# automerge/automerge-classic

Measured on AMD Instinct MI355X. Metric: CRDT ops/sec applied (bulk replay), higher is better.
Workload: dtype u32

## Files before the change

### automerge_classic_amd/csrc/am355_api.hip

```cpp
#include "am355_ctx.h"

static bool ctx_init(am355_ctx* c) {
  {
    unsigned hw = std::thread::hardware_concurrency();
    const char* env = getenv("AM355_HOST_THREADS");
    unsigned want = env && atoi(env) > 0 ? (unsigned)atoi(env) : std::min(hw ? hw : 4u, 64u);
    c->pool.reset(new HostPool(want > 1 ? want - 1 : 0));
  }
  int prio_low = 0, prio_high = 0;
  (void)hipDeviceGetStreamPriorityRange(&prio_low, &prio_high);
  auto make_stream = [](Stream& s, int prio) { return hipStreamCreateWithPriority(&s.h, hipStreamNonBlocking, prio) == hipSuccess; };
  if (!make_stream(c->stream, prio_high)) return false;
  {
    const char* env = getenv("AM355_HASH_CUS");
    int want = env ? atoi(env) : 0;
    bool made = false;
    if (want > 0) {
      hipDeviceProp_t prop;
      if (hipGetDeviceProperties(&prop, c->device) == hipSuccess && prop.multiProcessorCount > want) {
        int n_cu = prop.multiProcessorCount;
        std::vector<uint32_t> mask((size_t)(n_cu + 31) / 32, 0u);
        for (int k = 0; k < want; k++) { int cu = n_cu - 1 - k; mask[(size_t)cu / 32] |= 1u << (cu % 32); }
        made = hipExtStreamCreateWithCUMask(&c->stream2.h, (uint32_t)mask.size(), mask.data()) == hipSuccess;
      }
    }
    if (!made && !make_stream(c->stream2, prio_low)) return false;
  }
  if (!make_stream(c->stream3, prio_high) || !make_stream(c->stream4, prio_high)) return false;
  for (Event* e : {&c->ev_fork, &c->ev_join, &c->ev[0], &c->ev[1], &c->ev[2], &c->ev[3], &c->ev[4], &c->ev[5], &c->ev[6], &c->ev[7], &c->ev_parse, &c->ev_b0, &c->ev_b1,
                   &c->ev_counts, &c->ev_runs, &c->ev_s1, &c->ev_plan, &c->ev_tables, &c->ev_fills, &c->ev_sched})
    if (hipEventCreate(&e->h) != hipSuccess) return false;
  if (!c->h_sig.ensure(sizeof(HostSignals))) return false;
  memset(c->h_sig.p, 0, sizeof(HostSignals));
  if (const char* e = getenv("AM355_PHASE_EVENTS")) c->phase_events = strcmp(e, "0") != 0;
  if (const char* e = getenv("AM355_STAGE1_FILLS")) c->inline_fills = strcmp(e, "stream") != 0;
  return true;
}

extern "C" am355_ctx* am355_create(int device) {
  int n = 0;
  if (hipGetDeviceCount(&n) != hipSuccess || n <= 0 || device < 0 || device >= n) return nullptr;
  (void)hipSetDeviceFlags(hipDeviceScheduleSpin);
  if (hipSetDevice(device) != hipSuccess) return nullptr;
  am355_ctx* c = new am355_ctx();
  c->device = device;
  if (!ctx_init(c)) { delete c; return nullptr; }
  return c;
}

am355_ctx::~am355_ctx() {
  (void)hipSetDevice(device);
  if (lane) lane->wait();
  (void)doc_sum.wait();
  for (const Stream* s : {&stream, &stream2, &stream3, &stream4})
    if (s->h) (void)hipStreamSynchronize(s->h);
  if (shard_comm) (void)am355_shard_finalize(this);
}

extern "C" void am355_destroy(am355_ctx* c) {
  delete c;
}

extern "C" const char* am355_last_error(const am355_ctx* c) { return c ? c->err.c_str() : "no context (no GPU?)"; }
extern "C" uint32_t am355_flags(const am355_ctx* c) { return c ? c->flags : 0; }

extern "C" int am355_set_phase_events(am355_ctx* c, int on) {
  if (!c) return AM355_E_ARG;
  c->phase_events = on != 0;
  return AM355_OK;
}

extern "C" int am355_get_stats(const am355_ctx* c, am355_stats* out) {
  if (!c || !out) return AM355_E_ARG;
  *out = c->stats;
  return AM355_OK;
}

extern "C" int am355_get_hashes(const am355_ctx* c, uint8_t* out) {
  if (!c || !out) return AM355_E_ARG;
  if (!c->replayed || !c->h_hashes.p || c->is_document) return AM355_E_STATE;
  memcpy(out, c->h_hashes.p, 32 * (size_t)c->n_changes);
  return AM355_OK;
}

extern "C" int am355_arena_epoch(const am355_ctx* c, uint64_t* epoch) {
  if (!c || !epoch) return AM355_E_ARG;
  *epoch = c->arena_epoch;
  return AM355_OK;
}

extern "C" int am355_get_hashes_range(const am355_ctx* c, uint32_t first, uint32_t count, uint8_t* out) {
  if (!c || (!out && count)) return AM355_E_ARG;
  if (!c->replayed || !c->h_hashes.p || c->is_document) return AM355_E_STATE;
  if (first > c->n_changes || count > c->n_changes - first) return AM355_E_ARG;
  if (count) memcpy(out, (const uint8_t*)c->h_hashes.p + 32 * (size_t)first, 32 * (size_t)count);
  return AM355_OK;
}

extern "C" int am355_applied_in_input_order(const am355_ctx* c, int* yes) {
  if (!c || !yes) return AM355_E_ARG;
  if (!c->replayed || c->is_document) return AM355_E_STATE;
  bool ok = c->pending_change.empty() && c->n_pending == 0 && c->applied_change.size() == c->n_changes;
  for (uint32_t i = 0; ok && i < c->n_changes; i++) ok = c->applied_change[i] == i;
  *yes = ok ? 1 : 0;
  return AM355_OK;
}

extern "C" int am355_resident_counters(const am355_ctx* c, uint64_t out[3]) {
  if (!c || !out) return AM355_E_ARG;
  out[0] = c->n_resident_calls;
  out[1] = c->n_resident_fallbacks;
  out[2] = c->n_resorder_calls;
  return AM355_OK;
}

extern "C" int am355_resident_maps_only_calls(const am355_ctx* c, uint64_t* out) {
  if (!c || !out) return AM355_E_ARG;
  *out = c->n_maps_only_calls;
  return AM355_OK;
}

extern "C" int am355_get_raw(const am355_ctx* c, const uint8_t** arena, const uint64_t** offsets, uint32_t* n) {
  if (!c || !c->staged) return AM355_E_STATE;
  if (arena) *arena = c->raw.data();
  if (offsets) *offsets = c->raw_off.data();
  if (n) *n = c->n_changes;
  return AM355_OK;
}

extern "C" int am355_get_applied(const am355_ctx* c, uint32_t* out, uint32_t* n_applied) {
  if (!c || !n_applied) return AM355_E_ARG;
  if (!c->replayed || c->is_document) return AM355_E_STATE;
  *n_applied = (uint32_t)c->applied_change.size();
  if (out) memcpy(out, c->applied_change.data(), 4 * c->applied_change.size());
  return AM355_OK;
}

extern "C" int am355_test_sort(am355_ctx* c, uint64_t* keys, uint32_t* vals, uint32_t n, int key_bits) {
  if (!c) return AM355_E_ARG;
  (void)hipSetDevice(c->device);
  DevBuf ka, kb, va, vb, ws;
  if (!ka.ensure(8 * (size_t)n + 8) || !kb.ensure(8 * (size_t)n + 8) || !va.ensure(4 * (size_t)n + 4) || !vb.ensure(4 * (size_t)n + 4) || !ws.ensure(sort_workspace_bytes(n)))
    return fail(c, AM355_E_NOMEM, "alloc");
  hipStream_t st = c->stream;
  (void)hipMemcpyAsync(ka.p, keys, 8 * (size_t)n, hipMemcpyHostToDevice, st);
  (void)hipMemcpyAsync(va.p, vals, 4 * (size_t)n, hipMemcpyHostToDevice, st);
  int res = radix_sort_pairs(ka.as<uint64_t>(), va.as<uint32_t>(), kb.as<uint64_t>(), vb.as<uint32_t>(), n, 0, key_bits, ws.p, st);
  (void)hipMemcpyAsync(keys, res ? kb.p : ka.p, 8 * (size_t)n, hipMemcpyDeviceToHost, st);
  (void)hipMemcpyAsync(vals, res ? vb.p : va.p, 4 * (size_t)n, hipMemcpyDeviceToHost, st);
  HIPCHK(c, hipStreamSynchronize(st));
  HIPCHK(c, hipGetLastError());
  return AM355_OK;
}

extern "C" int am355_test_scan(am355_ctx* c, const uint32_t* in, uint32_t* out, uint32_t n, uint32_t* total) {
  if (!c) return AM355_E_ARG;
  (void)hipSetDevice(c->device);
  DevBuf di, dt, ws;
  if (!di.ensure(4 * (size_t)n + 4) || !dt.ensure(4) || !ws.ensure(scan_workspace_bytes(n))) return fail(c, AM355_E_NOMEM, "alloc");
  hipStream_t st = c->stream;
  (void)hipMemcpyAsync(di.p, in, 4 * (size_t)n, hipMemcpyHostToDevice, st);
  exclusive_scan_u32(di.as<uint32_t>(), di.as<uint32_t>(), n, dt.as<uint32_t>(), ws.p, st);
  (void)hipMemcpyAsync(out, di.p, 4 * (size_t)n, hipMemcpyDeviceToHost, st);
  (void)hipMemcpyAsync(total, dt.p, 4, hipMemcpyDeviceToHost, st);
  HIPCHK(c, hipStreamSynchronize(st));
// ... 42 lines not shown
```

### automerge_classic_amd/csrc/am355_ctx.h

```cpp
#pragma once
#include "../../include/am355.h"
#include "am355_decode.h"
#include "am355_merge.h"
#include "am355_bigcol.h"
#include "am355_encode.h"
#include "am355_prims.h"
#include "am355_render.h"
#include "am355_host.h"
#include "am355_pinflate.h"
#include "am355_history.h"
#include "am355_delta.h"
#include "am355_resorder.h"
#include "am355_apply.h"
#include "am355_sync.h"
#include "am355_sched.h"
#include "am355_hist.h"
#include "am355_canary.h"

#include <zlib.h>

#include <algorithm>
#include <atomic>
#include <chrono>
#include <cstdarg>
// ... 236 lines not shown
      if (stop_) return;
    }
  }
  static uint64_t now_us() { return (uint64_t)std::chrono::duration_cast<std::chrono::microseconds>(std::chrono::steady_clock::now().time_since_epoch()).count(); }
  std::function<void()> job_;
  std::atomic<int> state_{0};
  std::atomic<bool> sleeping_{false};
  std::mutex m_;
  std::condition_variable cv_;
  bool stop_ = false;
  std::thread t_;
};

struct Hash32 {
  uint8_t b[32];
  bool operator==(const Hash32& o) const { return memcmp(b, o.b, 32) == 0; }
};
struct Hash32Hasher {
  size_t operator()(const Hash32& h) const { size_t v; memcpy(&v, h.b, sizeof v); return v; }
};

}
using namespace am355_host;

struct am355_ctx {
  ~am355_ctx();
  int device = 0;
  Stream stream;
  Stream stream2;
  Stream stream3;
  Stream stream4;
  Event ev_fork, ev_join;
  Event ev[8];
  Event ev_parse, ev_b0, ev_b1;
  Event ev_counts, ev_runs;
  std::string err;
  uint32_t flags = 0;

  PinnedBytes raw;
  std::unique_ptr<HostPool> pool;
  std::unique_ptr<AsyncLane> lane;
  std::vector<uint64_t> raw_off;
  uint32_t n_changes = 0;
  DevBuf d_plan_totals;
  bool spec_launched = false;
  bool spec_large_launched = false;
  uint32_t spec_cap_ops = 0, spec_cap_preds = 0;
  uint32_t hint_ops = 0, hint_preds = 0, hint_large = 0;
  bool staged = false, replayed = false, ir_fetched = false;
  int ir_copy_enqueued = 0;
  bool prefetch_ir = false;
  bool has_unknown_cols = false;
  bool staging_in_flight = false;
  bool is_document = false;
  ChangeMeta doc_meta{};
  std::vector<uint32_t> doc_actor_rank;
  DevBuf d_arena, d_offsets, d_metas;
  uint64_t arena_epoch = 1;
  CopyRanges pending_up;
  std::vector<uint32_t> breaks_dev;
  void* breaks_dev_ptr = nullptr;
  HostBuf h_breaks_ahead;
  bool offsets_on_device = false;
  HostBuf h_metas, h_offsets, h_sig;
  uint32_t sig_seq = 0;
  Event ev_s1;
  Event ev_fills;
  Event ev_sched;
  Event ev_plan, ev_tables;
  void* counts_zeroed_at = nullptr; size_t counts_zeroed = 0;
  bool phase_events = false;
  bool inline_fills = true;
  DevBuf d_big, d_bigvals, d_ks;
  HostBuf h_biginfo;
  BigColDesc doc_cols{};
  bool doc_serial = false;
  DevBuf d_entries, d_amap_base, d_amap_prov, d_slots, d_first_idx, d_hashes, d_hash_tab, d_min_idx, d_has_dep, d_words, d_slot_rank, d_scan1, d_plan_sums, d_dep_idx, d_self_idx, d_rank_ids;
  HostBuf h_dep_idx, h_self_idx, h_amap, h_amap_base;
  HostBuf h_slots, h_hashes, h_has_dep, h_words, h_stage, h_s1;
  DevBuf d_s1;
  ChangeBrief* hp_briefs = nullptr;
  uint32_t* hp_distinct = nullptr;
  bool have_host_metas = false;
  uint32_t amap_cap = 0, slot_mask = 0, hash_mask = 0;
  bool used_fast_path = false;

  std::vector<ChangePlan> plans;
  std::vector<uint32_t> applied_change, applied_op_base;
  struct DocSum {
    static constexpr size_t PIECE = (size_t)4 << 20;
    std::thread t;
    std::unique_ptr<std::atomic<uint8_t>[]> copied;
    size_t n_pieces = 0;
    bool pending = false, ok = false;
    bool wait() {
      if (t.joinable()) t.join();
      pending = false;
      return ok;
    }
    ~DocSum() { if (t.joinable()) t.join(); }
  } doc_sum;
  std::vector<uint8_t> doc_bytes;
  std::vector<uint8_t> saved;
  HistoryOutput history;
  bool history_ok = false; uint32_t history_flags = 0;
  std::vector<std::vector<uint8_t>> inflate_scratch;
// ... 183 lines not shown
```

### automerge_classic_amd/csrc/am355_decode.h

```cpp
#pragma once
#include "am355_internal.h"

namespace am355 {
struct ParseFills {
  uint32_t* p[5];
  uint64_t n_words[5];
  uint32_t value[5];
  uint32_t n;
};
void parse_changes_host(const uint8_t* arena, const uint64_t* offsets, uint32_t n_changes, ChangeMeta* metas, uint32_t* n_entries);
void launch_parse_changes(const uint8_t* arena, const uint64_t* offsets, uint32_t n_changes, ChangeMeta* metas, uint32_t* n_entries, const ParseFills& fills,
                          hipStream_t st, bool fat = false);
int change_wave_class(const ChangeMeta& m);
void launch_hash_changes(const uint8_t* arena, const uint64_t* offsets, uint32_t n, uint8_t* hashes, uint32_t* min_idx, uint32_t* hash_tab,
                         uint32_t tab_mask, uint32_t* flags, hipStream_t st);
void launch_deps_resolve(const uint8_t* arena, const ChangeMeta* metas, const uint8_t* hashes, uint32_t n, const uint32_t* hash_tab, uint32_t tab_mask,
                         const uint32_t* min_idx, uint8_t* has_dependent, uint32_t* fast_flags, uint32_t* dep_idx, uint32_t* self_idx, hipStream_t st);
void launch_actor_intern(const uint8_t* arena, ChangeMeta* metas, uint32_t n, const uint32_t* amap_base, uint32_t* amap, uint32_t amap_cap,
                         unsigned long long* slots, uint32_t slot_mask, uint32_t* first_idx, uint32_t* flags, uint32_t* fast_flags, uint32_t* distinct,
                         void* rank_ids, ChangeBrief* briefs, uint32_t* slot_rank, unsigned long long* block_sums, uint32_t* plan_words, hipStream_t st,
                         ChangeBrief* host_briefs = nullptr);
size_t rank_ids_bytes();
size_t plan_block_sums_bytes(uint32_t n);
uint32_t distinct_capacity();
void launch_plan(const ChangeBrief* briefs, uint32_t n, const uint32_t* distinct, const uint32_t* slot_rank, uint32_t slot_mask, const unsigned long long* block_sums,
                 ChangePlan* plans, ChangePlan* plans_serial, const uint32_t* words, const uint32_t* plan_words, HostSignals* sig, uint32_t seq, hipStream_t st,
                 PlanTotals* dev_totals = nullptr, uint32_t* host_s1 = nullptr);
void launch_decode_speculative(const uint8_t* arena, const ChangeMeta* metas, const ChangePlan* plans, uint32_t n_changes, const PlanTotals* totals, uint32_t cap_ops,
                               uint32_t cap_preds, uint32_t cap_distinct, const uint32_t* amap, const uint32_t* slot_rank, OpCols cols, uint32_t* flags, hipStream_t st,
                               hipStream_t aux, bool with_large, uint32_t shard_rank = 0, uint32_t shard_world = 1);
void launch_decode_planned(const uint8_t* arena, const ChangeMeta* metas, const ChangePlan* plans, const ChangePlan* plans_serial, uint32_t n_changes,
                           uint32_t n_small, uint32_t n_large, uint32_t n_serial, const uint32_t* amap, const uint32_t* slot_rank, OpCols cols, uint32_t* flags,
                           hipStream_t st, hipStream_t aux, uint32_t shard_rank = 0, uint32_t shard_world = 1);
void launch_decode_columns(const uint8_t* arena, const ChangeMeta* metas, const ChangePlan* plans, uint32_t n_small, uint32_t n_large, uint32_t n_serial,
                           const uint32_t* amap, const uint32_t* slot_rank, OpCols cols, uint32_t* flags, hipStream_t st, hipStream_t aux, uint32_t shard_rank = 0,
                           uint32_t shard_world = 1);
void launch_doc_count(const uint8_t* arena, ChangeMeta* meta, hipStream_t st);
void launch_decode_document(const uint8_t* arena, const ChangeMeta* meta, const ChangePlan* plan, const uint32_t* actor_rank, OpCols cols,
                            uint32_t* flags, hipStream_t st);
void launch_keystr_expand(const uint32_t* run_start, const uint32_t* run_off, const uint32_t* run_len, const uint32_t* n_runs, uint32_t n_rows,
                          uint32_t* key_off, uint32_t* key_len, hipStream_t st);
}
```

### automerge_classic_amd/csrc/am355_decode.hip

```cpp
#include "am355_decode.h"
#include "am355_scan.h"

#include <cstdlib>

namespace am355 {

struct __attribute__((packed)) U8B {
  uint64_t v;
};
__host__ __device__ __forceinline__ uint64_t load_u64_unaligned(const uint8_t* p) { return ((const U8B*)p)->v; }
#ifdef AM355_LDS_IS_DISTINCT
__device__ __forceinline__ uint64_t load_u64_unaligned(LdsBytes p) { return ((const __attribute__((address_space(3))) U8B*)p)->v; }
#endif

template <class P>
struct CurT {
  P p;
  uint32_t off, len;
  uint64_t win;
  uint32_t win_off;
  __host__ __device__ __forceinline__ CurT() {}
  static constexpr uint32_t WIN_EMPTY = 0xffffff00u;
  __host__ __device__ __forceinline__ CurT(P p_, uint32_t off_, uint32_t len_) : p(p_), off(off_), len(len_), win(0), win_off(WIN_EMPTY) {}
  __host__ __device__ __forceinline__ uint32_t byte_at(uint32_t o) {
// ... 866 lines not shown
  if (wide) {
    p0 = load_u64_unaligned(p);
    p1 = load_u64_unaligned(p + 8);
    h = (p0 ^ (p1 * 0x9e3779b97f4a7c15ull)) * 0xff51afd7ed558ccdull;
    h ^= h >> 29;
  } else {
    for (uint32_t k = 0; k < len; k++) h = (h ^ p[k]) * 0x100000001b3ull;
    h = (h ^ h >> 33) * 0xff51afd7ed558ccdull;
  }
  uint32_t i = (uint32_t)(h >> 20) & mask;
  unsigned long long mine = ((unsigned long long)off + 1) << 16 | len;
  for (uint32_t probes = 0; probes <= mask; probes++) {
    unsigned long long v = slots[i];
    if (v == 0) {
      v = atomicCAS(&slots[i], 0ull, mine);
      if (v == 0) {
        uint32_t k = atomicAdd(&distinct[0], 1u);
        if (k < DISTINCT_CAP) {
          distinct[1 + k] = i;
          ((unsigned long long*)(distinct + 2 + DISTINCT_CAP))[k] = mine;
        }
        if (k < PLAN_RANK_MAX) {
          RankId r;
          for (uint32_t wd = 0; wd < PLAN_ID_MAX / 8; wd++) r.w[wd] = 0;
          r.len = len;
          r.pad = 0;
          if (wide) {
            r.w[0] = __builtin_bswap64(p0);
            r.w[1] = __builtin_bswap64(p1);
          } else if (len <= PLAN_ID_MAX) {
            for (uint32_t b = 0; b < len; b++) r.w[b >> 3] |= (unsigned long long)p[b] << (56 - 8 * (b & 7));
          }
          rank_ids[k] = r;
        }
        return i;
      }
    }
    if ((uint32_t)(v & 0xffff) == len) {
      const uint8_t* q = arena + ((v >> 16) - 1);
      bool eq = true;
      if (wide) eq = load_u64_unaligned(q) == p0 && load_u64_unaligned(q + 8) == p1;
      else for (uint32_t k = 0; k < len && eq; k++) eq = p[k] == q[k];
      if (eq) return i;
    }
    i = (i + 1) & mask;
  }
  return NONE32;
}

__global__ __launch_bounds__(WAVE) void k_actor_intern(const uint8_t* __restrict__ arena, ChangeMeta* __restrict__ metas, uint32_t n,
                                                        const uint32_t* __restrict__ amap_base, uint32_t* __restrict__ amap, uint32_t amap_cap,
                                                        unsigned long long* __restrict__ slots, uint32_t mask, uint32_t* __restrict__ first_idx,
                                                        uint32_t* __restrict__ flags, uint32_t* __restrict__ fast_flags, uint32_t* __restrict__ distinct,
                                                        RankId* __restrict__ rank_ids) {
  __shared__ uint32_t s_off[WAVE], s_len[WAVE];
  wave_priority_high();
  uint32_t c = blockIdx.x, lane = threadIdx.x;
  if (c >= n) return;
  ChangeMeta* m = &metas[c];
  if (m->flags) return;
  uint32_t base = amap_base[c];
  if ((uint64_t)base + m->n_entries > amap_cap) {
    if (lane == 0) atomicOr(fast_flags, (uint32_t)FF_CAPACITY);
    return;
  }
  const uint8_t* p = arena + m->base;
  uint32_t abs0 = (uint32_t)m->base;
  uint32_t n_other = m->n_other;
  if (lane == 0) {
    uint32_t s = actor_find_or_insert(arena, slots, mask, abs0 + m->actor_off, m->actor_len, distinct, rank_ids);
    if (s == NONE32) { atomicOr(flags, (uint32_t)F_UNSUPPORTED); s = 0; }
    amap[base] = s;
    m->author_slot = s;
    atomicMin(&first_idx[s], c);
  }
  if (n_other && n_other <= WAVE) {
    const uint32_t l0 = p[m->others_off], stride = l0 + 1;
    bool fits = l0 < 0x80 && (uint64_t)m->others_off + (uint64_t)stride * n_other <= m->len;
    bool mine_ok = !fits || lane >= n_other || p[m->others_off + stride * lane] == l0;
    if (fits && __ballot(!mine_ok) == 0) {
      if (lane < n_other) {
        uint32_t t = actor_find_or_insert(arena, slots, mask, abs0 + m->others_off + stride * lane + 1, l0, distinct, rank_ids);
        if (t == NONE32) { atomicOr(flags, (uint32_t)F_UNSUPPORTED); t = 0; }
        amap[base + 1 + lane] = t;
      }
      return;
    }
  }
  Cur cur(p, m->others_off, m->len);
  for (uint32_t k0 = 0; k0 < n_other; k0 += WAVE) {
    uint32_t cnt = n_other - k0 < WAVE ? n_other - k0 : WAVE;
    if (lane == 0) {
      for (uint32_t j = 0; j < cnt; j++) {
        uint64_t l = 0;
        read_uleb(cur, l);
        s_off[j] = abs0 + cur.off;
        s_len[j] = l < 65536 ? (uint32_t)l : NONE32;
        skip_bytes(cur, l);
      }
    }
    __syncthreads();
    if (lane < cnt) {
      uint32_t t = s_len[lane] != NONE32 ? actor_find_or_insert(arena, slots, mask, s_off[lane], s_len[lane], distinct, rank_ids) : NONE32;
      if (t == NONE32) { atomicOr(flags, (uint32_t)F_UNSUPPORTED); t = 0; }
      amap[base + 1 + k0 + lane] = t;
    }
    __syncthreads();
  }
}

// ... 25 lines not shown
  t[0] = ta; t[1] = tb; t[2] = tc;
}

__device__ void rank_actors(const uint32_t* __restrict__ distinct, const RankId* __restrict__ rank_ids, uint32_t* __restrict__ slot_rank,
                            uint32_t* __restrict__ plan_words) {
  __shared__ unsigned long long s_id[PLAN_RANK_MAX][PLAN_ID_MAX / 8];
  __shared__ uint32_t s_len[PLAN_RANK_MAX];
  __shared__ uint32_t s_fallback;
  static_assert(PLAN_RANK_MAX % BLOCK == 0 && PLAN_RANK_MAX <= DISTINCT_CAP, "rank_actors: records per thread");
  constexpr uint32_t PER = PLAN_RANK_MAX / BLOCK;
  const uint32_t t = threadIdx.x;
  RankId rec[PER];
  uint32_t slot_of[PER];
#pragma unroll
  for (uint32_t k = 0; k < PER; k++) {
    rec[k] = rank_ids[t + k * BLOCK];
    slot_of[k] = distinct[1 + t + k * BLOCK];
  }
  const uint32_t nd = distinct[0];
  if (t == 0) s_fallback = nd > PLAN_RANK_MAX ? 1u : 0u;
  __syncthreads();
  if (nd <= PLAN_RANK_MAX) {
#pragma unroll
    for (uint32_t k = 0; k < PER; k++) {
      const uint32_t a = t + k * BLOCK;
      if (a < nd) {
        s_len[a] = rec[k].len;
        if (rec[k].len > PLAN_ID_MAX) s_fallback = 1;
        for (uint32_t wd = 0; wd < PLAN_ID_MAX / 8; wd++) s_id[a][wd] = rec[k].w[wd];
      }
    }
  }
  __syncthreads();
  if (s_fallback) { if (t == 0) plan_words[0] = 1; return; }
#pragma unroll
  for (uint32_t k = 0; k < PER; k++) {
    const uint32_t a = t + k * BLOCK;
    if (a >= nd) break;
    uint32_t rank = 0;
    const uint32_t my_len = rec[k].len;
    static_assert(PLAN_ID_MAX == 32, "rank_actors compares four 64-bit words");
    const unsigned long long m0 = rec[k].w[0], m1 = rec[k].w[1], m2 = rec[k].w[2], m3 = rec[k].w[3];
    for (uint32_t j = 0; j < nd; j++) {
      const unsigned long long x0 = s_id[j][0], x1 = s_id[j][1], x2 = s_id[j][2], x3 = s_id[j][3];
      const bool less = x0 != m0 ? x0 < m0 : x1 != m1 ? x1 < m1 : x2 != m2 ? x2 < m2 : x3 != m3 ? x3 < m3 : s_len[j] < my_len;
      rank += less ? 1u : 0u;
    }
    slot_rank[slot_of[k]] = rank;
  }
}

__global__ __launch_bounds__(WAVE) void k_actor_first(ChangeMeta* __restrict__ metas, uint32_t n, const uint32_t* __restrict__ amap_base,
                                                       const uint32_t* __restrict__ amap, uint32_t amap_cap, const uint32_t* __restrict__ first_idx,
                                                       uint32_t* __restrict__ fast_flags) {
  wave_priority_high();
  uint32_t c = blockIdx.x, lane = threadIdx.x;
  if (c >= n) return;
  ChangeMeta* m = &metas[c];
  if (m->flags) return;
  uint32_t base = amap_base[c], ne = m->n_entries;
  if ((uint64_t)base + ne > amap_cap) return;
  uint32_t mx = 0;
  for (uint32_t k = lane; k < ne; k += WAVE) {
    uint32_t f = first_idx[amap[base + k]];
    mx = f > mx ? f : mx;
  }
  for (int d = WAVE / 2; d >= 1; d >>= 1) {
    uint32_t o = __shfl_xor(mx, d);
    mx = o > mx ? o : mx;
  }
  if (lane == 0) {
    m->max_first = mx;
    if (mx > c) atomicOr(fast_flags, (uint32_t)FF_LATE_ACTOR);
  }
}

__global__ __launch_bounds__(BLOCK) void k_actor_check(const uint8_t* __restrict__ arena, ChangeMeta* __restrict__ metas, uint32_t n,
                                                       const uint32_t* __restrict__ amap_base, const uint32_t* __restrict__ amap, uint32_t amap_cap,
                                                       const uint32_t* __restrict__ first_idx, uint32_t* __restrict__ flags, uint32_t* __restrict__ fast_flags,
                                                       ChangeBrief* __restrict__ briefs, const uint32_t* __restrict__ distinct, const RankId* __restrict__ rank_ids,
                                                       uint32_t* __restrict__ slot_rank, unsigned long long* __restrict__ block_sums, uint32_t* __restrict__ plan_words,
                                                       ChangeBrief* __restrict__ host_briefs) {
  wave_priority_high();
  __shared__ unsigned long long s_scan[BLOCK / WAVE][3];
  if (blockIdx.x + 1 == gridDim.x) {
    rank_actors(distinct, rank_ids, slot_rank, plan_words);
    return;
  }
  uint32_t c = gtid();
  const bool in_range = c < n;
  ChangeBrief br{};
  if (in_range) {
    ChangeMeta* m = &metas[c];
    br.seq = m->seq;
    br.start_op = (uint32_t)m->start_op;
    br.n_ops = m->n_ops;
    br.n_preds = m->n_preds;
    br.n_entries = m->n_entries;
    br.author_slot = m->author_slot;
    br.flags_fits = m->flags;
    if (!m->flags) {
      int wc = wave_class_of(*m);
      if (wc >= 1) br.flags_fits |= 0x80000000u;
      if (wc == 2) br.flags_fits |= 0x40000000u;
      if (m->pad & 1) br.flags_fits |= 0x20000000u;
    }
    briefs[c] = br;
    if (host_briefs) host_briefs[c] = br;
  }
  const bool valid = in_range && !(br.flags_fits & 0x1fffffffu);
  const bool has = valid && br.n_ops != 0;
  const bool small = has && (br.flags_fits & 0x40000000u), large = has && !small && (br.flags_fits & 0x80000000u), serial = has && !small && !large;
  unsigned long long ex[3], t1[3], t2[3];
  block_scan3(valid ? br.n_ops : 0u, valid ? br.n_preds : 0u, valid ? br.n_entries : 0u, s_scan, ex, t1);
  block_scan3(small ? 1u : 0u, large ? 1u : 0u, serial ? 1u : 0u, s_scan, ex, t2);
  uint32_t mx_op = has ? br.start_op + br.n_ops - 1 : 0u, bad = in_range ? (br.flags_fits & 0x1fffffffu) : 0u, unknown = in_range ? (br.flags_fits & 0x20000000u) : 0u;
  for (int d = WAVE / 2; d >= 1; d >>= 1) {
    uint32_t o = __shfl_xor(mx_op, d), ob = __shfl_xor(bad, d), ou = __shfl_xor(unknown, d);
    mx_op = o > mx_op ? o : mx_op;
    bad |= ob;
    unknown |= ou;
  }
  if ((threadIdx.x & (WAVE - 1)) == 0) {
    if (mx_op) atomicMax(&plan_words[1], mx_op);
    if (bad) atomicOr(&plan_words[2], bad);
    if (unknown) atomicOr(&plan_words[3], 1u);
  }
  if (threadIdx.x == 0) {
    unsigned long long* out = block_sums + (size_t)blockIdx.x * PLAN_SUMS;
    out[0] = t1[0]; out[1] = t1[1]; out[2] = t1[2]; out[3] = t2[0]; out[4] = t2[1]; out[5] = t2[2];
  }
}

__global__ __launch_bounds__(BLOCK) void k_plan_apply(const ChangeBrief* __restrict__ briefs, uint32_t n, const uint32_t* __restrict__ slot_rank, uint32_t slot_mask,
                                                      const unsigned long long* __restrict__ block_sums, ChangePlan* __restrict__ plans,
                                                      ChangePlan* __restrict__ plans_serial, const uint32_t* __restrict__ words, const uint32_t* __restrict__ plan_words,
                                                      const uint32_t* __restrict__ distinct, HostSignals* sig, uint32_t seq, PlanTotals* __restrict__ dev_totals,
                                                      uint32_t* __restrict__ host_s1) {
  wave_priority_high();
  __shared__ unsigned long long s_scan[BLOCK / WAVE][3];
  __shared__ unsigned long long s_base[6];
  {
    unsigned long long p0 = 0, p1 = 0, p2 = 0, p3 = 0, p4 = 0, p5 = 0;
    for (uint32_t j = threadIdx.x; j < blockIdx.x; j += BLOCK) {
      const unsigned long long* q = block_sums + (size_t)j * PLAN_SUMS;
      p0 += q[0]; p1 += q[1]; p2 += q[2]; p3 += q[3]; p4 += q[4]; p5 += q[5];
    }
    unsigned long long ex[3], t1[3], t2[3];
    block_scan3(p0, p1, p2, s_scan, ex, t1);
    block_scan3(p3, p4, p5, s_scan, ex, t2);
    if (threadIdx.x == 0) { s_base[0] = t1[0]; s_base[1] = t1[1]; s_base[2] = t1[2]; s_base[3] = t2[0]; s_base[4] = t2[1]; s_base[5] = t2[2]; }
    __syncthreads();
  }
  const uint32_t c = gtid();
  const bool in_range = c < n;
  ChangeBrief br{};
  if (in_range) br = briefs[c];
  const bool valid = in_range && !(br.flags_fits & 0x1fffffffu);
  const bool has = valid && br.n_ops != 0;
  const bool small = has && (br.flags_fits & 0x40000000u), large = has && !small && (br.flags_fits & 0x80000000u), serial = has && !small && !large;
  unsigned long long e1[3], e2[3], t1[3], t2[3];
  block_scan3(valid ? br.n_ops : 0u, valid ? br.n_preds : 0u, valid ? br.n_entries : 0u, s_scan, e1, t1);
  block_scan3(small ? 1u : 0u, large ? 1u : 0u, serial ? 1u : 0u, s_scan, e2, t2);
  if (has) {
    ChangePlan pl{c, (uint32_t)(s_base[0] + e1[0]), (uint32_t)(s_base[1] + e1[1]), (uint32_t)(s_base[2] + e1[2]),
                  br.author_slot <= slot_mask ? slot_rank[br.author_slot] : 0u, br.n_entries};
    if (small) plans[(uint32_t)(s_base[3] + e2[0])] = pl;
    else if (large) plans[n - 1 - (uint32_t)(s_base[4] + e2[1])] = pl;
    else plans_serial[(uint32_t)(s_base[5] + e2[2])] = pl;
  }
  if (blockIdx.x + 1 == gridDim.x && host_s1) {
    const uint32_t nd = distinct[0] < DISTINCT_CAP ? distinct[0] : DISTINCT_CAP;
    const uint32_t* src = words;
    for (uint32_t i = threadIdx.x; i < 16; i += BLOCK) host_s1[i] = src[i];
    uint32_t* hd = host_s1 + 16;
    for (uint32_t i = threadIdx.x; i < 1 + nd; i += BLOCK) hd[i] = distinct[i];
    const unsigned long long* ids = (const unsigned long long*)(distinct + 2 + DISTINCT_CAP);
    unsigned long long* hids = (unsigned long long*)(hd + 2 + DISTINCT_CAP);
    for (uint32_t i = threadIdx.x; i < nd; i += BLOCK) hids[i] = ids[i];
    __threadfence_system();
    __syncthreads();
  }
  if (blockIdx.x + 1 == gridDim.x && threadIdx.x == 0) {
    unsigned long long ops = s_base[0] + t1[0], preds = s_base[1] + t1[1], ent = s_base[2] + t1[2];
    PlanTotals z{};
    z.n_ops = (uint32_t)ops; z.n_preds = (uint32_t)preds; z.n_entries = (uint32_t)ent;
    z.n_small = (uint32_t)(s_base[3] + t2[0]); z.n_large = (uint32_t)(s_base[4] + t2[1]); z.n_serial = (uint32_t)(s_base[5] + t2[2]);
    z.max_op = plan_words[1];
    z.fallback = (plan_words[0] || ops >= 0x7ffffff0ull || preds >= 0xfffffff0ull || ent >= 0xfffffff0ull) ? 1u : 0u;
    z.flags_a = words[0] | plan_words[2]; z.fast_a = words[1]; z.total_entries = words[2]; z.n_distinct = distinct[0];
    z.reserved[0] = plan_words[3];
    if (dev_totals) *dev_totals = z;
    signal_host((uint32_t*)&sig->plan, (const uint32_t*)&z, sizeof(PlanTotals) / 4, &sig->plan_seq, seq);
  }
}

struct Rle {
  Cur c;
  int state;
  int64_t count;
  bool have_last, last_null;
  int64_t last;
  uint32_t last_off, last_len;
};

__device__ __forceinline__ void rle_init(Rle& r, const uint8_t* p, uint32_t len) {
  r.c = Cur(p, 0, len);
  r.state = 0;
  r.count = 0;
  r.have_last = false;
  r.last_null = true;
  r.last = 0;
  r.last_off = r.last_len = 0;
}

enum { RT_UINT = 0, RT_INT = 1, RT_UTF8 = 2 };

struct RVal {
  bool is_null;
  int64_t i;
  uint32_t off, len;
};

template <int TYPE>
__device__ __forceinline__ bool rle_raw(Rle& r, RVal& v) {
  v.is_null = false;
  if (TYPE == RT_UINT) {
    uint64_t u;
    if (!read_uleb(r.c, u)) return false;
    v.i = (int64_t)u;
  } else if (TYPE == RT_INT) {
    if (!read_sleb(r.c, v.i)) return false;
  } else {
    uint64_t n;
    if (!read_uleb(r.c, n)) return false;
    v.off = r.c.off;
    v.len = (uint32_t)n;
    if (!skip_bytes(r.c, n)) return false;
  }
  return true;
}

template <int TYPE>
__device__ __forceinline__ bool rle_same(const Rle& r, const RVal& v) {
  if (!r.have_last || r.last_null) return false;
  if (TYPE == RT_UTF8) {
// ... 639 lines not shown
        L.run_tok[nr] = 0;
        L.aux[nr] = 0;
        nr++;
        rows = n;
      }
      L.run_start[nr] = (uint32_t)(rows - rows_done);
      L.n_runs = nr;
      L.total_rows = (uint32_t)(rows - rows_done);
      L.err = e;
    }
    __syncthreads();
    err |= L.err;
    uint32_t batch = L.total_rows, nr = L.n_runs;
    for (uint32_t r = lane; r < nr; r += WAVE) {
      uint32_t k = L.run_kind[r], pk = r ? L.run_kind[r - 1] : prev_kind;
      if (k == RK_NUL || pk == RK_NUL) continue;
      uint32_t off = L.run_tok[r] - col_abs, len = L.aux[r];
      uint32_t poff = r ? L.run_tok[r - 1] - col_abs : prev_off, plen = r ? L.aux[r - 1] : prev_len;
      if (len == plen && bytes_equal(keycol, poff, off, len, key_len)) err |= F_BAD_RLE;
    }
    if (lane == 0 && nr) { prev_kind = L.run_kind[nr - 1]; prev_off = L.run_tok[nr - 1] - col_abs; prev_len = L.aux[nr - 1]; }
    for (uint32_t i = lane; i < batch; i += WAVE) {
      uint32_t lo = 0, hi = nr;
      while (hi - lo > 1) {
        uint32_t mid = (lo + hi) >> 1;
        if (L.run_start[mid] <= i) lo = mid; else hi = mid;
      }
      bool nul = L.run_kind[lo] == RK_NUL;
      o.key_off[base + rows_done + i] = nul ? 0 : L.run_tok[lo];
      o.key_len[base + rows_done + i] = nul ? NONE32 : L.aux[lo];
    }
    rows_done += batch;
    __syncthreads();
    if (rows_done >= n || batch == 0) break;
  }
  return err;
}

enum : uint32_t { DG_ROWS = 1 , DG_KEY_ID = 2 , DG_KEY_STR = 4, DG_PRED = 8, DG_ALL = 15 };

template <class WL>
__global__ __launch_bounds__(WAVE) AM355_WAVES_PER_EU(WL::COLMAX <= 256 ? 6 : 1) void k_decode_wave(const uint8_t* __restrict__ arena, const ChangeMeta* __restrict__ metas,
                                                       const ChangePlan* __restrict__ plans, uint32_t n_plans, ActorXlate x, OpCols o,
                                                       uint32_t* __restrict__ flags, DecodeGate gate) {
  __shared__ WL L;
  wave_priority_high();
  uint32_t pi = blockIdx.x, lane = threadIdx.x;
  const uint32_t groups = gridDim.y > 1 ? (1u << blockIdx.y) : (uint32_t)DG_ALL;
  if (gate.totals) {
    const PlanTotals t = *gate.totals;
    if (!decode_gate_open(t, gate.cap_ops, gate.cap_preds, gate.cap_distinct)) return;
    n_plans = gate.large ? t.n_large : t.n_small;
    if (gate.large) plans += gate.n_changes - t.n_large;
  }
  if (pi >= n_plans) return;
  const ChangePlan pl = plans[pi];
  const ChangeMeta* m = &metas[pl.change];
  const uint8_t* p = arena + m->base;
  const uint32_t n = m->n_ops, base = pl.op_base, abs0 = (uint32_t)m->base, n_preds_cap = m->n_preds;
  const uint32_t start_op = (uint32_t)m->start_op;
  uint32_t col_off[C_NUM], col_len[C_NUM];
  for (int k = 0; k < C_NUM; k++) { col_off[k] = m->col_off[k]; col_len[k] = m->col_len[k]; }
  uint32_t err = 0;
  for (uint32_t k = lane; k < pl.n_actors; k += WAVE) {
    uint32_t v = x.amap[pl.amap_base + k];
    L.rank[k] = x.slot_rank ? x.slot_rank[v] : v;
  }
  uint32_t reg_lo = 0xffffffffu, reg_hi = 0;
  for (int k = 0; k < C_NUM; k++)
    if (col_len[k]) {
      reg_lo = col_off[k] < reg_lo ? col_off[k] : reg_lo;
      reg_hi = col_off[k] + col_len[k] > reg_hi ? col_off[k] + col_len[k] : reg_hi;
    }
  const bool staged = reg_hi > reg_lo && reg_hi - reg_lo <= WL::REGION;
  if (staged) stage_to_lds(L.region, p + reg_lo, reg_hi - reg_lo, lane);
  auto load_col = [&](int k) {
    if (staged && col_len[k]) wv_load_column(L, (LdsBytes)(L.region + (col_off[k] - reg_lo)), col_len[k], lane);
    else wv_load_column(L, p + col_off[k], col_len[k], lane);
  };

  if (groups & DG_ROWS) {
  load_col(C_ACTION);
  err |= L.err;
  for (uint32_t i = lane; i < n; i += WAVE) {
    bool nul; int64_t v;
    wv_row_value<false>(L, i, nul, v, err);
    if (nul) err |= F_UNSUPPORTED;
    if ((uint64_t)v >= NONE32) err |= F_OVERFLOW;
    o.action[base + i] = (uint32_t)v;
    o.id_ctr[base + i] = start_op + i;
    o.id_actor[base + i] = pl.author;
  }
  {
    __syncthreads();
    uint32_t len = col_len[C_INSERT];
    if (staged && len) {
      LdsBytes col = (LdsBytes)(L.region + (col_off[C_INSERT] - reg_lo));
      for (uint32_t i = lane; i < len; i += WAVE) L.bytes[i] = col[i];
    } else {
      const uint8_t* col = p + col_off[C_INSERT];
      for (uint32_t i = lane; i < len; i += WAVE) L.bytes[i] = col[i];
    }
    __syncthreads();
    uint32_t tok_base = 0, carry_start = 0;
    for (uint32_t chunk = 0; chunk < len; chunk += WAVE) {
      uint32_t pos = chunk + lane;
// ... 166 lines not shown
    uint32_t r = 0;
    if (nul) err |= F_UNSUPPORTED;
    else if ((uint64_t)v >= pl.n_actors) err |= F_BAD_ROW;
    else r = L.rank[v];
    o.pred_actor[pl.pred_base + j] = r;
  }
  load_col(C_PRED_CTR);
  err |= L.err;
  {
    int64_t carry = 0;
    for (uint32_t j0 = 0; j0 < total_preds; j0 += WAVE) {
      uint32_t j = j0 + lane;
      bool nul = true; int64_t d = 0;
      if (j < total_preds) wv_row_value<true>(L, j, nul, d, err);
      int64_t abs = carry + wave_incl_scan_i64(nul ? 0 : d, lane);
      carry = __shfl(abs, WAVE - 1);
      if (j < total_preds) {
        if (nul) err |= F_UNSUPPORTED;
        else if (abs < 0 || (uint64_t)abs >= NONE32) err |= F_OVERFLOW;
        o.pred_ctr[pl.pred_base + j] = (uint32_t)abs;
      }
    }
  }
  }
  if (err) atomicOr(flags, err);
}

int change_wave_class(const ChangeMeta& m) { return wave_class_of(m); }

void launch_parse_changes(const uint8_t* arena, const uint64_t* offsets, uint32_t n_changes, ChangeMeta* metas, uint32_t* n_entries, const ParseFills& fills,
                          hipStream_t st, bool fat) {
  if (!n_changes && !fills.n) return;
  if (fat) hipLaunchKernelGGL(k_parse_changes<true>, dim3(n_changes ? n_changes : 64), dim3(WAVE), 0, st, arena, offsets, n_changes, metas, n_entries, fills);
  else hipLaunchKernelGGL(k_parse_changes<false>, dim3(n_changes ? n_changes : 64), dim3(WAVE), 0, st, arena, offsets, n_changes, metas, n_entries, fills);
}

void launch_hash_changes(const uint8_t* arena, const uint64_t* offsets, uint32_t n, uint8_t* hashes, uint32_t* min_idx, uint32_t* hash_tab,
                         uint32_t tab_mask, uint32_t* flags, hipStream_t st) {
  if (!n) return;
  hipLaunchKernelGGL(k_hash_changes, dim3((n + HASH_LANES - 1) / HASH_LANES), dim3(2 * HASH_LANES), 0, st, arena, offsets, n, hashes, min_idx, flags);
  AM355_LAUNCH_INDEPENDENT(k_hash_insert, dim3((n + BLOCK - 1) / BLOCK), dim3(BLOCK), st, (const uint8_t*)hashes, n, hash_tab, tab_mask, min_idx);
}

void launch_deps_resolve(const uint8_t* arena, const ChangeMeta* metas, const uint8_t* hashes, uint32_t n, const uint32_t* hash_tab, uint32_t tab_mask,
                         const uint32_t* min_idx, uint8_t* has_dependent, uint32_t* fast_flags, uint32_t* dep_idx, uint32_t* self_idx, hipStream_t st) {
  if (!n) return;
  AM355_LAUNCH_INDEPENDENT(k_deps_resolve, dim3(n), dim3(WAVE), st, arena, metas, hashes, n, hash_tab, tab_mask, min_idx, has_dependent, fast_flags, dep_idx,
                           self_idx);
}

void launch_actor_intern(const uint8_t* arena, ChangeMeta* metas, uint32_t n, const uint32_t* amap_base, uint32_t* amap, uint32_t amap_cap,
                         unsigned long long* slots, uint32_t slot_mask, uint32_t* first_idx, uint32_t* flags, uint32_t* fast_flags, uint32_t* distinct,
                         void* rank_ids, ChangeBrief* briefs, uint32_t* slot_rank, unsigned long long* block_sums, uint32_t* plan_words, hipStream_t st,
                         ChangeBrief* host_briefs) {
  if (n)
    hipLaunchKernelGGL(k_actor_intern, dim3(n), dim3(WAVE), 0, st, arena, metas, n, amap_base, amap, amap_cap, slots, slot_mask, first_idx, flags,
                       fast_flags, distinct, (RankId*)rank_ids);
  if (n) hipLaunchKernelGGL(k_actor_first, dim3(n), dim3(WAVE), 0, st, metas, n, amap_base, (const uint32_t*)amap, amap_cap, (const uint32_t*)first_idx, fast_flags);
  hipLaunchKernelGGL(k_actor_check, dim3((n + BLOCK - 1) / BLOCK + 1), dim3(BLOCK), 0, st, arena, metas, n, amap_base, (const uint32_t*)amap, amap_cap,
                     (const uint32_t*)first_idx, flags, fast_flags, briefs, (const uint32_t*)distinct, (const RankId*)rank_ids, slot_rank, block_sums, plan_words,
                     host_briefs);
}

size_t rank_ids_bytes() { return sizeof(RankId) * PLAN_RANK_MAX; }

size_t plan_block_sums_bytes(uint32_t n) { return sizeof(unsigned long long) * PLAN_SUMS * ((size_t)(n + BLOCK - 1) / BLOCK + 1); }

void launch_plan(const ChangeBrief* briefs, uint32_t n, const uint32_t* distinct, const uint32_t* slot_rank, uint32_t slot_mask, const unsigned long long* block_sums,
                 ChangePlan* plans, ChangePlan* plans_serial, const uint32_t* words, const uint32_t* plan_words, HostSignals* sig, uint32_t seq, hipStream_t st,
                 PlanTotals* dev_totals, uint32_t* host_s1) {
  uint32_t nb = (n + BLOCK - 1) / BLOCK;
  hipLaunchKernelGGL(k_plan_apply, dim3(nb ? nb : 1), dim3(BLOCK), 0, st, briefs, n, slot_rank, slot_mask, block_sums, plans, plans_serial, words, plan_words,
                     distinct, sig, seq, dev_totals, host_s1);
}

uint32_t distinct_capacity() { return DISTINCT_CAP; }

__global__ __launch_bounds__(WAVE) void k_doc_count(const uint8_t* __restrict__ arena, ChangeMeta* __restrict__ meta) {
  uint32_t lane = threadIdx.x;
  if (lane > 1) return;
  int slot = lane == 0 ? C_ACTION : C_PRED_NUM;
  uint64_t cnt, sum;
  bool ok = rle_count_sum(arena + meta->base + meta->col_off[slot], meta->col_len[slot], cnt, sum);
  if (!ok) { atomicOr(&meta->flags, (uint32_t)F_BAD_RLE); return; }
  if (lane == 0) meta->n_ops = (uint32_t)cnt; else meta->n_preds = (uint32_t)sum;
}

void launch_doc_count(const uint8_t* arena, ChangeMeta* meta, hipStream_t st) {
  AM355_LAUNCH_INDEPENDENT(k_doc_count, dim3(1), dim3(WAVE), st, arena, meta);
}

__global__ __launch_bounds__(BLOCK) void k_keystr_expand(const uint32_t* __restrict__ run_start, const uint32_t* __restrict__ run_off,
                                                          const uint32_t* __restrict__ run_len, const uint32_t* __restrict__ n_runs_p, uint32_t n_rows,
                                                          uint32_t* __restrict__ key_off, uint32_t* __restrict__ key_len) {
  uint32_t row = gtid();
  if (row >= n_rows) return;
  uint32_t nr = *n_runs_p;
  uint32_t off = 0, len = NONE32;
  if (nr && row < run_start[nr]) {
    uint32_t lo = 0, hi = nr;
    while (hi - lo > 1) {
      uint32_t mid = (lo + hi) >> 1;
      if (run_start[mid] <= row) lo = mid; else hi = mid;
    }
    off = run_off[lo];
    len = run_len[lo];
  }
  key_off[row] = off;
  key_len[row] = len;
}

void launch_keystr_expand(const uint32_t* run_start, const uint32_t* run_off, const uint32_t* run_len, const uint32_t* n_runs, uint32_t n_rows,
                          uint32_t* key_off, uint32_t* key_len, hipStream_t st) {
  if (!n_rows) return;
  AM355_LAUNCH_INDEPENDENT(k_keystr_expand, dim3((n_rows + BLOCK - 1) / BLOCK), dim3(BLOCK), st, run_start, run_off, run_len, n_runs, n_rows, key_off, key_len);
}

void launch_decode_document(const uint8_t* arena, const ChangeMeta* meta, const ChangePlan* plan, const uint32_t* actor_rank, OpCols cols,
                            uint32_t* flags, hipStream_t st) {
  ActorXlate x{actor_rank, nullptr, 0, 1};
  AM355_LAUNCH_INDEPENDENT(k_decode_columns, dim3(1, T_NUM_DOC), dim3(WAVE), st, arena, meta, plan, 1u, x, cols, flags, 0);
}

static uint32_t decode_group_split(uint32_t n_waves, uint32_t shard_world, bool large_class = false) {
  static const uint32_t split_max = []() { const char* e = getenv("AM355_DECODE_SPLIT_MAX"); return e && atol(e) > 0 ? (uint32_t)atol(e) : 1536u; }();
  return (shard_world <= 1 && n_waves <= (large_class ? 512u : split_max)) ? 4u : 1u;
}

void launch_decode_columns(const uint8_t* arena, const ChangeMeta* metas, const ChangePlan* plans, uint32_t n_small, uint32_t n_large, uint32_t n_serial,
                           const uint32_t* amap, const uint32_t* slot_rank, OpCols cols, uint32_t* flags, hipStream_t st, hipStream_t aux, uint32_t shard_rank,
                           uint32_t shard_world) {
  ActorXlate x{amap, slot_rank, shard_rank, shard_world};
  if (n_large && n_small + n_large <= 1024) { n_large += n_small; n_small = 0; }
  hipStream_t s2 = (n_small && aux) ? aux : st;
  if (n_small) hipLaunchKernelGGL(k_decode_wave<WaveLdsSmall>, dim3(n_small, decode_group_split(n_small, shard_world)), dim3(WAVE), 0, st, arena, metas, plans, n_small, x, cols, flags, DecodeGate{});
  if (n_large) hipLaunchKernelGGL(k_decode_wave<WaveLdsLarge>, dim3(n_large, decode_group_split(n_large, shard_world, true)), dim3(WAVE), 0, s2, arena, metas, plans + n_small, n_large, x, cols, flags, DecodeGate{});
  if (n_serial)
    AM355_LAUNCH_INDEPENDENT(k_decode_columns, dim3((n_serial + WAVE - 1) / WAVE, T_NUM), dim3(WAVE), s2, arena, metas, plans + n_small + n_large, n_serial,
                             x, cols, flags, 0);
}

void launch_decode_planned(const uint8_t* arena, const ChangeMeta* metas, const ChangePlan* plans, const ChangePlan* plans_serial, uint32_t n_changes,
                           uint32_t n_small, uint32_t n_large, uint32_t n_serial, const uint32_t* amap, const uint32_t* slot_rank, OpCols cols, uint32_t* flags,
                           hipStream_t st, hipStream_t aux, uint32_t shard_rank, uint32_t shard_world) {
  ActorXlate x{amap, slot_rank, shard_rank, shard_world};
  hipStream_t s2 = (n_small && aux) ? aux : st;
  if (n_small) hipLaunchKernelGGL(k_decode_wave<WaveLdsSmall>, dim3(n_small, decode_group_split(n_small, shard_world)), dim3(WAVE), 0, st, arena, metas, plans, n_small, x, cols, flags, DecodeGate{});
  if (n_large) hipLaunchKernelGGL(k_decode_wave<WaveLdsLarge>, dim3(n_large, decode_group_split(n_large, shard_world, true)), dim3(WAVE), 0, s2, arena, metas, plans + (n_changes - n_large), n_large, x, cols, flags, DecodeGate{});
  if (n_serial)
    AM355_LAUNCH_INDEPENDENT(k_decode_columns, dim3((n_serial + WAVE - 1) / WAVE, T_NUM), dim3(WAVE), s2, arena, metas, plans_serial, n_serial, x, cols, flags, 0);
}

void launch_decode_speculative(const uint8_t* arena, const ChangeMeta* metas, const ChangePlan* plans, uint32_t n_changes, const PlanTotals* totals, uint32_t cap_ops,
                               uint32_t cap_preds, uint32_t cap_distinct, const uint32_t* amap, const uint32_t* slot_rank, OpCols cols, uint32_t* flags, hipStream_t st,
                               hipStream_t aux, bool with_large, uint32_t shard_rank, uint32_t shard_world) {
  if (!n_changes) return;
  ActorXlate x{amap, slot_rank, shard_rank, shard_world};
  hipLaunchKernelGGL(k_decode_wave<WaveLdsSmall>, dim3(n_changes, decode_group_split(n_changes, shard_world)), dim3(WAVE), 0, st, arena, metas, plans, 0u, x, cols, flags,
                     DecodeGate{totals, cap_ops, cap_preds, cap_distinct, n_changes, 0u});
  if (with_large)
    hipLaunchKernelGGL(k_decode_wave<WaveLdsLarge>, dim3(n_changes, decode_group_split(n_changes, shard_world, true)), dim3(WAVE), 0, aux, arena, metas, plans, 0u, x, cols, flags,
                       DecodeGate{totals, cap_ops, cap_preds, cap_distinct, n_changes, 1u});
}

}
```

### automerge_classic_amd/csrc/am355_internal.h

```cpp
#pragma once
#include "am355_device.h"

namespace am355 {

enum ColSlot { C_OBJ_ACTOR, C_OBJ_CTR, C_KEY_ACTOR, C_KEY_CTR, C_KEY_STR, C_INSERT, C_ACTION, C_VAL_LEN, C_VAL_RAW, C_PRED_NUM, C_PRED_ACTOR, C_PRED_CTR,
               C_ID_ACTOR, C_ID_CTR, C_NUM };

struct ChangeMeta {
  uint64_t base;
  uint32_t len;
  uint32_t flags;
  uint64_t seq, start_op;
  uint32_t n_entries;
  uint32_t author_slot;
  uint32_t max_first;
  uint32_t pad;
  uint32_t n_deps, deps_off;
  uint32_t actor_off, actor_len;
  uint32_t n_other, others_off;
  uint32_t col_off[C_NUM], col_len[C_NUM];
  uint32_t n_ops, n_preds;
};

struct ChangeBrief {
  uint64_t seq;
  uint32_t start_op, n_ops, n_preds, n_entries, author_slot;
  uint32_t flags_fits;
};

enum FastFlag : uint32_t {
  FF_DUP_HASH = 1u << 0,
  FF_MISSING_DEP = 1u << 1,
  FF_LATE_DEP = 1u << 2,
  FF_LATE_ACTOR = 1u << 3,
  FF_CAPACITY = 1u << 4
};

struct ChangePlan {
  uint32_t change;
  uint32_t op_base;
  uint32_t pred_base;
  uint32_t amap_base;
  uint32_t author;
  uint32_t n_actors;
};

struct PlanTotals {
  uint32_t n_ops, n_preds, n_entries;
  uint32_t n_small, n_large, n_serial;
  uint32_t max_op;
  uint32_t fallback;
  uint32_t flags_a, fast_a, total_entries, n_distinct;
  uint32_t reserved[4];
};

__host__ __device__ inline bool decode_gate_open(const PlanTotals& t, uint32_t cap_ops, uint32_t cap_preds, uint32_t cap_distinct) {
  return !t.fallback && !t.flags_a && !t.fast_a && t.n_ops <= cap_ops && t.n_preds <= cap_preds && t.n_distinct <= cap_distinct;
}
struct DecodeGate {
  const PlanTotals* totals = nullptr;
  uint32_t cap_ops = 0, cap_preds = 0, cap_distinct = 0, n_changes = 0, large = 0;
};

struct HostSignals {
  volatile uint32_t plan_seq;    uint32_t pad0[15];
  PlanTotals plan;
  volatile uint32_t counts_seq;  uint32_t pad1[15];
  uint32_t counts[32];
  volatile uint32_t runs_seq;    uint32_t pad2[15];
  uint32_t runs[16];
  volatile uint32_t final_seq;   uint32_t pad3[15];
  uint32_t final_counts[16];
  volatile uint32_t resorder_seq;  uint32_t pad4[15];
  uint32_t resorder[16];
  volatile uint32_t delta_mid_seq; uint32_t pad5[15];
  uint32_t delta_mid[16];
  volatile uint32_t delta_end_seq; uint32_t pad6[15];
  uint32_t delta_end[16];
};

struct ActorSpan {
  uint32_t start_op, n_ops, op_base;
};

struct OpCols {
  uint32_t *obj_actor, *obj_ctr;
  uint32_t *key_actor, *key_ctr;
  uint32_t *key_off, *key_len;
  uint32_t *action, *val_tl, *val_off;
  uint32_t *pred_first, *pred_num;
  uint32_t *id_ctr, *id_actor;
  uint8_t* insert;
  uint32_t *pred_actor, *pred_ctr;
};

__host__ __device__ __forceinline__ uint32_t shard_owner(uint32_t obj_actor, uint32_t obj_ctr, uint32_t world) {
  return obj_actor == NONE32 ? 0u : (obj_ctr + obj_actor) % world;
}

}
```

### automerge_classic_amd/csrc/am355_prims.h

```cpp
#pragma once
#include "am355_device.h"
#include "am355_canary.h"
#include <stddef.h>

namespace am355 {
constexpr uint32_t LAUNCH_RANGES = 8;
struct FillRanges {
  uint32_t* p[LAUNCH_RANGES];
  uint32_t n_words[LAUNCH_RANGES];
  uint32_t value[LAUNCH_RANGES];
  uint32_t n = 0;
  bool add(void* q, size_t bytes, uint32_t v) {
    if (n == LAUNCH_RANGES) return false;
    p[n] = (uint32_t*)q; n_words[n] = (uint32_t)((bytes + 3) / 4); value[n] = v; n++;
    return true;
  }
};
void launch_fill_ranges(const FillRanges& f, hipStream_t st);
struct CopyRanges {
  void* dst[LAUNCH_RANGES];
  const void* src[LAUNCH_RANGES];
  uint32_t bytes[LAUNCH_RANGES];
  uint32_t n = 0;
  bool add(void* d, const void* s, size_t b) {
    if (n == LAUNCH_RANGES) return false;
    dst[n] = d; src[n] = s; bytes[n] = (uint32_t)b; n++;
    return true;
  }
};
void launch_copy_ranges(const CopyRanges& r, hipStream_t st);
void launch_signal_words(const uint32_t* src_a, uint32_t n_a, const uint32_t* src_b, uint32_t n_b, uint32_t* host_words, volatile uint32_t* host_seq, uint32_t seq,
                         hipStream_t st);
size_t scan_workspace_bytes(uint32_t n);
void exclusive_scan_u32(const uint32_t* in, uint32_t* out, uint32_t n, uint32_t* d_total, void* ws, hipStream_t st);
void exclusive_scan_terminators(const uint8_t* bytes, uint32_t L, uint32_t* out, uint32_t* d_total, void* ws, hipStream_t st);
void exclusive_scan2_u32(const uint32_t* in_a, uint32_t* out_a, uint32_t* d_total_a, const uint32_t* in_b, uint32_t* out_b, uint32_t* d_total_b, uint32_t n,
                         void* ws, hipStream_t st);
void max_u32(const uint32_t* v, uint32_t n, uint32_t* d_out, hipStream_t st);
size_t sort_workspace_bytes(uint32_t n);
int radix_sort_pairs(uint64_t* keys_a, uint32_t* vals_a, uint64_t* keys_b, uint32_t* vals_b, uint32_t n, int begin_bit, int end_bit,
                     void* ws, hipStream_t st, bool first_hist_done = false);
constexpr uint32_t SORT_TILE_ELEMS = 2048;
uint32_t sort_tiles(uint32_t n);
bool sort_is_fused(uint32_t n);
uint32_t* sort_first_table(void* ws);
size_t chain_work_bytes(uint32_t n);
void chain_mark(const uint32_t* next, uint32_t n, uint32_t* mark, void* work, hipStream_t st);
}
```

### automerge_classic_amd/csrc/am355_prims.hip

```cpp
#include "am355_prims.h"
#include <algorithm>
#include "am355_scan.h"
#include "am355_canary.h"
#include <mutex>
#include <string>
#include <vector>

namespace am355 {

constexpr int SCAN_ITEMS = 8;
constexpr int SCAN_TILE = BLOCK * SCAN_ITEMS;
constexpr uint32_t SCAN_SINGLE = 4 * SCAN_TILE;
constexpr uint32_t SCAN_TWO_LAUNCH_TILES = 1024;

__global__ __launch_bounds__(BLOCK) void k_scan_tile_sums(const uint32_t* __restrict__ in, uint32_t* __restrict__ tile_sums, uint32_t n) {
  __shared__ uint32_t s[BLOCK / WAVE];
  uint32_t base = blockIdx.x * SCAN_TILE;
  uint32_t v[SCAN_ITEMS];
#pragma unroll
  for (int j = 0; j < SCAN_ITEMS; j++) {
    uint32_t i = base + j * BLOCK + threadIdx.x;
    v[j] = i < n ? in[i] : 0u;
  }
  uint32_t sum = 0;
#pragma unroll
  for (int j = 0; j < SCAN_ITEMS; j++) sum += v[j];
  uint32_t total = block_sum_u32(sum, s);
  if (threadIdx.x == 0) tile_sums[blockIdx.x] = total;
}

__global__ __launch_bounds__(BLOCK) void k_scan_sums(uint32_t* __restrict__ sums, uint32_t n_tiles, uint32_t* __restrict__ grand_total) {
  __shared__ uint32_t s[BLOCK / WAVE];
  uint32_t carry = 0;
  constexpr uint32_t SUMS_PER = 4;
  for (uint32_t base = 0; base < n_tiles; base += BLOCK * SUMS_PER) {
    const uint32_t i0 = base + threadIdx.x * SUMS_PER;
    uint32_t v[SUMS_PER], mine = 0;
#pragma unroll
    for (uint32_t k = 0; k < SUMS_PER; k++) {
      v[k] = i0 + k < n_tiles ? sums[i0 + k] : 0u;
      mine += v[k];
    }
    uint32_t total;
    uint32_t ex = block_exclusive_scan_u32(mine, s, &total) + carry;
#pragma unroll
    for (uint32_t k = 0; k < SUMS_PER; k++) {
      if (i0 + k < n_tiles) sums[i0 + k] = ex;
      ex += v[k];
    }
    carry += total;
  }
  if (threadIdx.x == 0 && grand_total) *grand_total = carry;
}

template <bool PREFIXED>
__global__ __launch_bounds__(BLOCK) void k_scan_apply(const uint32_t* __restrict__ in, uint32_t* __restrict__ out,
                                                      const uint32_t* __restrict__ tile_sums, uint32_t n, uint32_t* __restrict__ grand_total) {
  __shared__ uint32_t s[BLOCK / WAVE];
  uint32_t before;
  if (PREFIXED) before = tile_sums[blockIdx.x];
  else {
    uint32_t part = 0;
    for (uint32_t k = threadIdx.x; k < blockIdx.x; k += BLOCK) part += tile_sums[k];
    before = block_sum_u32(part, s);
  }
  static_assert(SCAN_ITEMS == 8, "k_scan_apply moves a thread's stretch as two uint4");
  uint32_t base = blockIdx.x * SCAN_TILE + threadIdx.x * SCAN_ITEMS;
  const bool wide = ((((uintptr_t)in | (uintptr_t)out) & 15) == 0) && base + SCAN_ITEMS <= n;
  uint32_t v[SCAN_ITEMS];
  if (wide) {
    const uint4 a = *(const uint4*)(in + base), b4 = *(const uint4*)(in + base + 4);
    v[0] = a.x; v[1] = a.y; v[2] = a.z; v[3] = a.w; v[4] = b4.x; v[5] = b4.y; v[6] = b4.z; v[7] = b4.w;
  } else {
#pragma unroll
    for (int j = 0; j < SCAN_ITEMS; j++) {
      uint32_t i = base + j;
      v[j] = i < n ? in[i] : 0;
    }
  }
  uint32_t sum = 0;
#pragma unroll
  for (int j = 0; j < SCAN_ITEMS; j++) sum += v[j];
  uint32_t total;
  uint32_t ex = block_exclusive_scan_u32(sum, s, &total) + before;
  if (!PREFIXED && grand_total && blockIdx.x == gridDim.x - 1 && threadIdx.x == 0) *grand_total = before + total;
  uint32_t o[SCAN_ITEMS];
#pragma unroll
  for (int j = 0; j < SCAN_ITEMS; j++) {
    o[j] = ex;
    ex += v[j];
  }
  if (wide) {
    *(uint4*)(out + base) = uint4{o[0], o[1], o[2], o[3]};
    *(uint4*)(out + base + 4) = uint4{o[4], o[5], o[6], o[7]};
  } else {
#pragma unroll
    for (int j = 0; j < SCAN_ITEMS; j++) {
      uint32_t i = base + j;
      if (i < n) out[i] = o[j];
    }
  }
}

constexpr unsigned long long LB_SUM = 1ull << 32, LB_PREFIX = 2ull << 32;
__device__ __forceinline__ unsigned long long lb_load(const unsigned long long* p) {
#if defined(__HIP_DEVICE_COMPILE__)
  return __hip_atomic_load(p, __ATOMIC_RELAXED, __HIP_MEMORY_SCOPE_AGENT);
#else
  return *(const volatile unsigned long long*)p;
#endif
}
__device__ __forceinline__ void lb_store(unsigned long long* p, unsigned long long v) {
#if defined(__HIP_DEVICE_COMPILE__)
  __hip_atomic_store(p, v, __ATOMIC_RELAXED, __HIP_MEMORY_SCOPE_AGENT);
#else
  *(volatile unsigned long long*)p = v;
#endif
// ... 24 lines not shown
#pragma unroll
  for (int j = 0; j < SCAN_ITEMS; j++) sum += v[j];
  uint32_t total;
  uint32_t ex = block_exclusive_scan_u32(sum, s, &total);
  if (threadIdx.x == 0) {
    lb_store(&state[tile], (tile ? LB_SUM : LB_PREFIX) | total);
    s_before = 0;
  }
  if (tile && threadIdx.x < WAVE) {
    const uint32_t lane = threadIdx.x;
    uint32_t before = 0;
    int look = (int)tile - 1;
    for (;;) {
      const int idx = look - (int)lane;
      const unsigned long long w = idx >= 0 ? lb_load(&state[idx]) : LB_PREFIX;
      const uint32_t st = (uint32_t)(w >> 32);
      const unsigned long long pending = __ballot(st == 0), prefix = __ballot(st == 2);
      const uint32_t first = prefix ? (uint32_t)__ffsll((long long)prefix) - 1 : WAVE;
      const unsigned long long needed = first >= WAVE - 1 ? ~0ull : ((2ull << first) - 1);
      if (pending & needed) continue;
      uint32_t part = lane <= first ? (uint32_t)w : 0u;
      for (int d = WAVE / 2; d; d >>= 1) part += __shfl_xor(part, d);
      before += part;
      if (prefix) break;
      look -= WAVE;
    }
    if (lane == 0) {
      s_before = before;
      lb_store(&state[tile], LB_PREFIX | (before + total));
    }
  }
  __syncthreads();
  const uint32_t before = s_before;
  if (grand_total && (size_t)(tile + 1) * SCAN_TILE >= n && threadIdx.x == 0) *grand_total = before + total;
  ex += before;
  uint32_t o[SCAN_ITEMS];
#pragma unroll
  for (int j = 0; j < SCAN_ITEMS; j++) {
    o[j] = ex;
    ex += v[j];
  }
  if (wide) {
    *(uint4*)(out + base) = uint4{o[0], o[1], o[2], o[3]};
    *(uint4*)(out + base + 4) = uint4{o[4], o[5], o[6], o[7]};
  } else {
#pragma unroll
    for (int j = 0; j < SCAN_ITEMS; j++) {
      uint32_t i = base + j;
      if (i < n) out[i] = o[j];
    }
  }
}

__global__ __launch_bounds__(BLOCK) void k_scan_single(const uint32_t* __restrict__ in, uint32_t* __restrict__ out, uint32_t n, uint32_t* __restrict__ grand_total) {
  wave_priority_high();
  __shared__ uint32_t s[BLOCK / WAVE];
  uint32_t carry = 0;
  for (uint32_t tile = 0; tile < n; tile += SCAN_TILE) {
    uint32_t base = tile + threadIdx.x * SCAN_ITEMS;
    uint32_t v[SCAN_ITEMS];
    uint32_t sum = 0;
    for (int j = 0; j < SCAN_ITEMS; j++) {
      uint32_t i = base + j;
      v[j] = i < n ? in[i] : 0;
      sum += v[j];
    }
    uint32_t total;
    uint32_t ex = block_exclusive_scan_u32(sum, s, &total) + carry;
    for (int j = 0; j < SCAN_ITEMS; j++) {
      uint32_t i = base + j;
      if (i < n) out[i] = ex;
      ex += v[j];
    }
    carry += total;
  }
  if (threadIdx.x == 0 && grand_total) *grand_total = carry;
}

__global__ __launch_bounds__(BLOCK) void k_scan2_tile_sums(const uint32_t* __restrict__ in_a, const uint32_t* __restrict__ in_b, uint32_t* __restrict__ sums_a,
                                                          uint32_t* __restrict__ sums_b, uint32_t n) {
  __shared__ uint32_t s[BLOCK / WAVE];
  uint32_t base = blockIdx.x * SCAN_TILE;
  uint32_t sa = 0, sb = 0;
  for (int j = 0; j < SCAN_ITEMS; j++) {
    uint32_t i = base + j * BLOCK + threadIdx.x;
    if (i < n) { sa += in_a[i]; sb += in_b[i]; }
  }
  uint32_t ta = block_sum_u32(sa, s), tb = block_sum_u32(sb, s);
  if (threadIdx.x == 0) { sums_a[blockIdx.x] = ta; sums_b[blockIdx.x] = tb; }
}
__global__ __launch_bounds__(BLOCK) void k_scan2_sums(uint32_t* __restrict__ sums_a, uint32_t* __restrict__ sums_b, uint32_t n_tiles, uint32_t* __restrict__ total_a,
                                                     uint32_t* __restrict__ total_b) {
  __shared__ uint32_t s[BLOCK / WAVE];
  uint32_t ca = 0, cb = 0;
  for (uint32_t base = 0; base < n_tiles; base += BLOCK) {
    uint32_t i = base + threadIdx.x;
    uint32_t va = i < n_tiles ? sums_a[i] : 0, vb = i < n_tiles ? sums_b[i] : 0;
    uint32_t ta, tb;
    uint32_t ea = block_exclusive_scan_u32(va, s, &ta);
    uint32_t eb = block_exclusive_scan_u32(vb, s, &tb);
    if (i < n_tiles) { sums_a[i] = ca + ea; sums_b[i] = cb + eb; }
    ca += ta;
    cb += tb;
  }
  if (threadIdx.x == 0) {
    if (total_a) *total_a = ca;
    if (total_b) *total_b = cb;
  }
}
template <bool PREFIXED>
// ... 58 lines not shown
__device__ __forceinline__ void term_load(const uint8_t* __restrict__ bytes, uint32_t L, uint32_t base, uint32_t (&v)[SCAN_ITEMS]) {
  static_assert(SCAN_ITEMS == 8, "a thread's stretch is one 8-byte load");
  if ((((uintptr_t)(bytes + base)) & 7) == 0 && base + SCAN_ITEMS <= L) {
    const unsigned long long x = *(const unsigned long long*)(bytes + base);
#pragma unroll
    for (int j = 0; j < SCAN_ITEMS; j++) v[j] = (uint32_t)((x >> (8 * j + 7)) & 1ull) ^ 1u;
  } else {
#pragma unroll
    for (int j = 0; j < SCAN_ITEMS; j++) { uint32_t i = base + j; v[j] = i < L ? ((bytes[i] >> 7) ^ 1u) : 0u; }
  }
}
__global__ __launch_bounds__(BLOCK) void k_scan_term_sums(const uint8_t* __restrict__ bytes, uint32_t L, uint32_t* __restrict__ tile_sums) {
  __shared__ uint32_t s[BLOCK / WAVE];
  uint32_t v[SCAN_ITEMS];
  term_load(bytes, L, blockIdx.x * SCAN_TILE + threadIdx.x * SCAN_ITEMS, v);
  uint32_t sum = 0;
#pragma unroll
  for (int j = 0; j < SCAN_ITEMS; j++) sum += v[j];
  uint32_t total = block_sum_u32(sum, s);
  if (threadIdx.x == 0) tile_sums[blockIdx.x] = total;
}
__global__ __launch_bounds__(BLOCK) void k_scan_term_apply(const uint8_t* __restrict__ bytes, uint32_t L, uint32_t* __restrict__ out, const uint32_t* __restrict__ tile_sums) {
  __shared__ uint32_t s[BLOCK / WAVE];
  const uint32_t n = L + 1;
  const uint32_t base = blockIdx.x * SCAN_TILE + threadIdx.x * SCAN_ITEMS;
  uint32_t v[SCAN_ITEMS];
  term_load(bytes, L, base, v);
  uint32_t sum = 0;
#pragma unroll
  for (int j = 0; j < SCAN_ITEMS; j++) sum += v[j];
  uint32_t total;
  uint32_t ex = block_exclusive_scan_u32(sum, s, &total) + tile_sums[blockIdx.x];
  uint32_t o[SCAN_ITEMS];
#pragma unroll
  for (int j = 0; j < SCAN_ITEMS; j++) { o[j] = ex; ex += v[j]; }
  if ((((uintptr_t)(out + base)) & 15) == 0 && base + SCAN_ITEMS <= n) {
    *(uint4*)(out + base) = uint4{o[0], o[1], o[2], o[3]};
    *(uint4*)(out + base + 4) = uint4{o[4], o[5], o[6], o[7]};
  } else {
#pragma unroll
    for (int j = 0; j < SCAN_ITEMS; j++) if (base + j < n) out[base + j] = o[j];
  }
}
void exclusive_scan_terminators(const uint8_t* bytes, uint32_t L, uint32_t* out, uint32_t* d_total, void* ws, hipStream_t st) {
  const uint32_t n = L + 1, n_tiles = (n + SCAN_TILE - 1) / SCAN_TILE;
  uint32_t* sums = (uint32_t*)ws;
  hipLaunchKernelGGL(k_scan_term_sums, dim3(n_tiles), dim3(BLOCK), 0, st, bytes, L, sums);
  hipLaunchKernelGGL(k_scan_sums, dim3(1), dim3(BLOCK), 0, st, sums, n_tiles, d_total);
  hipLaunchKernelGGL(k_scan_term_apply, dim3(n_tiles), dim3(BLOCK), 0, st, bytes, L, out, (const uint32_t*)sums);
}

size_t scan_workspace_bytes(uint32_t n) { return 2 * sizeof(uint32_t) * ((size_t)(n + SCAN_TILE - 1) / SCAN_TILE + 2); }

void exclusive_scan_u32(const uint32_t* in, uint32_t* out, uint32_t n, uint32_t* d_total, void* ws, hipStream_t st) {
  uint32_t n_tiles = (n + SCAN_TILE - 1) / SCAN_TILE;
  uint32_t* sums = (uint32_t*)ws;
  if (n_tiles == 0) {
    if (d_total) (void)hipMemsetAsync(d_total, 0, sizeof(uint32_t), st);
    return;
  }
  if (n <= SCAN_SINGLE) {
    hipLaunchKernelGGL(k_scan_single, dim3(1), dim3(BLOCK), 0, st, in, out, n, d_total);
    return;
  }
  if (n_tiles <= SCAN_TWO_LAUNCH_TILES) {
    hipLaunchKernelGGL(k_scan_tile_sums, dim3(n_tiles), dim3(BLOCK), 0, st, in, sums, n);
    hipLaunchKernelGGL(k_scan_apply<false>, dim3(n_tiles), dim3(BLOCK), 0, st, in, out, (const uint32_t*)sums, n, d_total);
    return;
  }
  const char* lb_env = getenv("AM355_SCAN_LOOKBACK");
  const bool lookback = lb_env && *lb_env == '1';
  if (lookback) {
    unsigned long long* state = (unsigned long long*)ws;
    uint32_t* ticket = (uint32_t*)(state + n_tiles);
    (void)hipMemsetAsync(ws, 0, sizeof(unsigned long long) * n_tiles + 8, st);
    hipLaunchKernelGGL(k_scan_lookback, dim3(n_tiles), dim3(BLOCK), 0, st, in, out, n, state, ticket, d_total);
    return;
  }
  hipLaunchKernelGGL(k_scan_tile_sums, dim3(n_tiles), dim3(BLOCK), 0, st, in, sums, n);
  hipLaunchKernelGGL(k_scan_sums, dim3(1), dim3(BLOCK), 0, st, sums, n_tiles, d_total);
  hipLaunchKernelGGL(k_scan_apply<true>, dim3(n_tiles), dim3(BLOCK), 0, st, in, out, (const uint32_t*)sums, n, (uint32_t*)nullptr);
}

constexpr int SORT_ITEMS = 8;
constexpr int SORT_WAVE_SPAN = WAVE * SORT_ITEMS;
constexpr int SORT_TILE = (BLOCK / WAVE) * SORT_WAVE_SPAN;
constexpr int RADIX = 256;
constexpr uint32_t SORT_FUSED_TILES = 64;

__global__ __launch_bounds__(BLOCK) void k_sort_hist(const uint64_t* __restrict__ keys, uint32_t n, int shift,
                                                      uint32_t* __restrict__ table, uint32_t n_tiles) {
  __shared__ uint32_t hist[RADIX];
  hist[threadIdx.x] = 0;
  __syncthreads();
  uint32_t base = blockIdx.x * SORT_TILE;
  for (int j = 0; j < SORT_TILE / BLOCK; j++) {
    uint32_t i = base + j * BLOCK + threadIdx.x;
    if (i < n) atomicAdd(&hist[(uint32_t)(keys[i] >> shift) & 0xff], 1u);
  }
  __syncthreads();
  table[threadIdx.x * n_tiles + blockIdx.x] = hist[threadIdx.x];
}

template <bool RAW_TABLE>
__global__ __launch_bounds__(BLOCK) void k_sort_scatter(const uint64_t* __restrict__ keys_in, const uint32_t* __restrict__ vals_in,
                                                         uint64_t* __restrict__ keys_out, uint32_t* __restrict__ vals_out, uint32_t n,
                                                         int shift, const uint32_t* __restrict__ table, uint32_t n_tiles) {
  __shared__ uint32_t wave_cnt[BLOCK / WAVE][RADIX];
  __shared__ uint32_t s_red[BLOCK / WAVE];
  uint32_t t = threadIdx.x, w = t / WAVE, lane = t % WAVE;
  for (int k = 0; k < BLOCK / WAVE; k++) wave_cnt[k][t] = 0;
  __syncthreads();

  uint64_t key[SORT_ITEMS];
  uint32_t val[SORT_ITEMS], rank[SORT_ITEMS];
  uint32_t base = blockIdx.x * SORT_TILE + w * SORT_WAVE_SPAN;
  for (int j = 0; j < SORT_ITEMS; j++) {
    uint32_t i = base + j * WAVE + lane;
    bool valid = i < n;
    key[j] = valid ? keys_in[i] : 0;
    val[j] = valid ? vals_in[i] : 0;
    uint32_t d = (uint32_t)(key[j] >> shift) & 0xff;
    unsigned long long peers = __ballot(valid);
    for (int b = 0; b < 8; b++) {
      unsigned long long m = __ballot(valid && ((d >> b) & 1));
      peers &= ((d >> b) & 1) ? m : ~m;
    }
    uint32_t before = (uint32_t)__popcll(peers & ((1ull << lane) - 1));
    uint32_t seen = valid ? wave_cnt[w][d] : 0;
    rank[j] = seen + before;
    __builtin_amdgcn_wave_barrier();
    if (valid && before == 0) wave_cnt[w][d] = seen + (uint32_t)__popcll(peers);
    __builtin_amdgcn_wave_barrier();
  }
// ... 466 lines not shown
```

### automerge_classic_amd/csrc/am355_replay.hip

```cpp
#include "am355_ctx.h"


struct HashSet {
  std::vector<const uint8_t*> slot;
  size_t mask = 0;
  void init(size_t n) {
    size_t cap = 16;
    while (cap < n * 2 + 2) cap <<= 1;
    slot.assign(cap, nullptr);
    mask = cap - 1;
  }
  static uint64_t key(const uint8_t* h) { uint64_t v; memcpy(&v, h, 8); return v * 0x9e3779b97f4a7c15ull; }
  const uint8_t** find(const uint8_t* h) {
    size_t i = (size_t)(key(h) >> 20) & mask;
    while (slot[i]) {
      if (slot[i] != (const uint8_t*)1 && memcmp(slot[i], h, 32) == 0) return &slot[i];
      i = (i + 1) & mask;
    }
    return nullptr;
  }
  bool has(const uint8_t* h) { return find(h) != nullptr; }
  void add(const uint8_t* h) {
    size_t i = (size_t)(key(h) >> 20) & mask;
    while (slot[i] && slot[i] != (const uint8_t*)1) i = (i + 1) & mask;
// ... 567 lines not shown
      d_amap = c->d_amap_prov.as<uint32_t>();
      d_rank = (const uint32_t*)(d_tables + o_x);
    } else {
      if (b_amap) memcpy(h + o_x, c->amap.data(), b_amap);
      d_amap = (const uint32_t*)(d_tables + o_x);
    }
    HIPCHK(c, hipMemcpyAsync(d_tables, h, o_x + std::max(b_rank, b_amap), hipMemcpyHostToDevice, st));
  }

  HIPCHK(c, hipMemsetAsync(c->d_counts.p, 0, c->mb.counts_bytes, st));
  HIPCHK(c, hipEventRecord(c->ev_fork, st));
  HIPCHK(c, hipStreamWaitEvent(c->stream3, c->ev_fork, 0));
  if (!merge_prepare(c->mb, c->stream3)) return fail(c, AM355_E_DEVICE, "merge fills: more ranges than one launch takes");
  HIPCHK(c, hipEventRecord(c->ev[2], st));
  launch_decode_columns(c->d_arena.as<uint8_t>(), c->d_metas.as<ChangeMeta>(), (const ChangePlan*)d_tables, n_small, n_large, (uint32_t)np - n_small - n_large, d_amap,
                        d_rank, c->cols, &c->d_counts.as<Counts>()->flags, st, c->stream3, c->shard_rank, c->shard_world);
  HIPCHK(c, hipEventRecord(c->ev[3], st));
  HIPCHK(c, hipEventRecord(c->ev_join, c->stream3));
  HIPCHK(c, hipStreamWaitEvent(st, c->ev_join, 0));

  Counts* hc = c->h_counts.as<Counts>();
  merge_run(c->mb, c->ir, hc, st, (c->phase_events || !c->mb.sig) ? c->ev_counts.h : nullptr, c->ev_runs);
  HIPCHK(c, hipEventRecord(c->ev[5], st));
  if (hc->flags) return error_for_flags(c, hc->flags, "op set rejected");
  c->counts = *hc;
  c->counts.n_objects += 1;
  return AM355_OK;
}

struct GeneralOrder { const uint32_t* order; const uint32_t* pass; uint32_t n_applied; hipEvent_t ready; };
static int run_device_planned(am355_ctx* c, const PlanTotals& tot, uint32_t n_distinct, float* ms_host_plan, const GeneralOrder* go = nullptr) {
  hipStream_t st = c->stream;
  const bool trace = getenv("AM355_TRACE") != nullptr;
  auto t_begin = std::chrono::steady_clock::now();
  auto lap = [&](const char* what) {
    if (trace) fprintf(stderr, "  planned: %-26s +%8.3f ms\n", what, std::chrono::duration<double, std::milli>(std::chrono::steady_clock::now() - t_begin).count());
  };
  uint32_t n = c->n_changes;
  c->n_ops = tot.n_ops;
  c->n_preds = tot.n_preds;
  c->max_op = tot.max_op;
  auto al = [](size_t b) { return (b + 255) & ~(size_t)255; };
  size_t o_tab = al(sizeof(ActorSpan) * (size_t)n + 16), tables_bytes = o_tab + al(4 * ((size_t)n_distinct + 1) + 16);
  if (!c->d_tables.ensure(tables_bytes) || !c->h_stage.ensure(tables_bytes)) return fail(c, AM355_E_NOMEM, "device allocation failed");
  uint8_t* d_tables = c->d_tables.as<uint8_t>();
  c->p_spans = (ActorSpan*)d_tables;
  c->p_tab_off = (uint32_t*)(d_tables + o_tab);
  c->sig_seq++;
  int rcb = setup_buffers(c, n_distinct);
  if (rcb) return rcb;
  lap("buffers carved");
  const bool spec_done = c->spec_launched && decode_gate_open(tot, c->spec_cap_ops, c->spec_cap_preds, distinct_capacity()) &&
                         c->counts_zeroed_at == c->d_counts.p && c->mb.counts_bytes <= c->counts_zeroed;
  if (trace && c->spec_launched && !spec_done)
    fprintf(stderr, "  planned: speculative decode not usable: ops %u / cap %u, preds %u / cap %u, distinct %u, fast_a %x flags_a %x fallback %u, counts %p/%p %zu/%zu\n", tot.n_ops,
            c->spec_cap_ops, tot.n_preds, c->spec_cap_preds, tot.n_distinct, tot.fast_a, tot.flags_a, tot.fallback, c->counts_zeroed_at, c->d_counts.p, c->mb.counts_bytes, c->counts_zeroed);
  if (c->spec_launched && !spec_done) {
    c->spec_launched = false;
    HIPCHK(c, hipStreamSynchronize(c->stream3));
    HIPCHK(c, hipStreamSynchronize(st));
    int rc2 = setup_buffers(c, n_distinct);
    if (rc2) return rc2;
  }
  if (!spec_done && !(c->counts_zeroed_at == c->d_counts.p && c->mb.counts_bytes <= c->counts_zeroed)) HIPCHK(c, hipMemsetAsync(c->d_counts.p, 0, c->mb.counts_bytes, st));
  c->counts_zeroed_at = nullptr;
  c->hint_large = tot.n_large;
  if (spec_done) {
    c->hint_ops = std::max(c->hint_ops, tot.n_ops);
    c->hint_preds = std::max(c->hint_preds, tot.n_preds);
    const uint32_t host_large = c->spec_large_launched ? 0u : tot.n_large;
    if (tot.n_serial || host_large) {
      if (!c->spec_large_launched) {
        HIPCHK(c, hipEventRecord(c->ev_fork, st));
        HIPCHK(c, hipStreamWaitEvent(c->stream3, c->ev_fork, 0));
      }
      launch_decode_planned(c->d_arena.as<uint8_t>(), c->d_metas.as<ChangeMeta>(), c->d_plans.as<ChangePlan>(), c->d_plans.as<ChangePlan>() + std::max(n, 1u), n, 0,
                            host_large, tot.n_serial, c->d_amap_prov.as<uint32_t>(), c->d_slot_rank.as<uint32_t>(), c->cols, &c->d_counts.as<Counts>()->flags,
                            c->stream3, nullptr, c->shard_rank, c->shard_world);
    }
    lap("decode was launched behind the plan kernel");
  } else {
    c->hint_ops = tot.n_ops;
    c->hint_preds = tot.n_preds;
    if (tot.n_small && (tot.n_large || tot.n_serial)) {
      HIPCHK(c, hipEventRecord(c->ev_fork, st));
      HIPCHK(c, hipStreamWaitEvent(c->stream3, c->ev_fork, 0));
    }
    if (c->phase_events) HIPCHK(c, hipEventRecord(c->ev[2], st));
    launch_decode_planned(c->d_arena.as<uint8_t>(), c->d_metas.as<ChangeMeta>(), c->d_plans.as<ChangePlan>(), c->d_plans.as<ChangePlan>() + std::max(n, 1u), n,
                          tot.n_small, tot.n_large, tot.n_serial, c->d_amap_prov.as<uint32_t>(), c->d_slot_rank.as<uint32_t>(), c->cols,
                          &c->d_counts.as<Counts>()->flags, st, c->stream3, c->shard_rank, c->shard_world);
    lap("decode launched");
    if (c->phase_events) HIPCHK(c, hipEventRecord(c->ev[3], st));
  }
  c->spec_launched = false;
  const bool second_class = tot.n_small && (tot.n_large || tot.n_serial);
  hipStream_t fill_stream = second_class ? c->stream4 : c->stream3;
  if (!merge_prepare(c->mb, fill_stream)) return fail(c, AM355_E_DEVICE, "merge fills: more ranges than one launch takes");
  if (second_class) {
    HIPCHK(c, hipEventRecord(c->ev_join, c->stream3));
    HIPCHK(c, hipStreamWaitEvent(st, c->ev_join, 0));
  }
  lap("fills enqueued");
  if (go) HIPCHK(c, hipEventSynchronize(go->ready));
  auto t0 = std::chrono::steady_clock::now();
  std::vector<uint32_t> slot_rank;
// ... 652 lines not shown
  c->ir_copy_enqueued = 0;
  c->h_tables_current = false;
  c->pos_valid = false;
  c->stats.n_edits = c->counts.n_edits;
  c->stats.ir_bytes = (uint64_t)c->counts.n_objects * sizeof(am355_ir_object) + (uint64_t)c->counts.n_map_emit * sizeof(am355_ir_map) +
                      ((uint64_t)c->counts.n_erecs + 1) * sizeof(am355_ir_edit);
  if (verify) {
    std::vector<uint32_t> now(c->counts.n_list_ins);
    HIPCHK(c, hipMemcpy(now.data(), b.order, 4 * now.size(), hipMemcpyDeviceToHost));
    if (now != kept) return fail(c, AM355_E_DEVICE, "internal: the list order merged in place differs from the order computed from scratch");
  }
  return AM355_OK;
}

int replay_impl(am355_ctx* c) {
  if (!c) return AM355_E_ARG;
  if (!c->staged) return fail(c, AM355_E_STATE, "am355_load_changes must be called first");
  (void)hipSetDevice(c->device);
  c->replayed = c->ir_fetched = false;
  c->ir_copy_enqueued = 0;
  c->dep_graph_ready = false;
  c->flags = 0;
  c->spec_launched = false;
  c->batch_list_only = false;
  c->h_tables_were_current = c->h_tables_current;
  c->h_tables_current = false;
  if (c->is_document) return replay_document(c);
  auto t_begin = std::chrono::steady_clock::now();
  if (c->in_apply && c->keep.want) {
    c->keep.want = false;
    const int rr = replay_resident(c);
    if (rr != RESIDENT_FALLBACK) {
      if (rr != AM355_OK) return rr;
      am355_stats& s = c->stats;
      s.n_changes = c->n_changes; s.n_applied = c->n_applied; s.n_pending = 0; s.n_actors = (uint32_t)c->actors.size(); s.n_objects = c->counts.n_objects;
      s.n_heads = (uint32_t)(c->heads.size() / 32); s.n_ops = c->n_ops; s.max_op = c->max_op; s.raw_bytes = c->raw.size();
      s.n_map_values = c->counts.n_map_emit; s.n_list_elems = c->counts.n_list_ins; s.n_edits = c->counts.n_edits;
      s.ir_bytes = (uint64_t)c->counts.n_objects * sizeof(am355_ir_object) + (uint64_t)c->counts.n_map_emit * sizeof(am355_ir_map) +
                   ((uint64_t)c->counts.n_erecs + 1) * sizeof(am355_ir_edit);
      s.ms_parse = s.ms_decode = s.ms_merge = s.ms_order = s.ms_hash_stream = s.ms_host_schedule = 0;
      s.fast_path = 1;
      s.ms_total = std::chrono::duration<float, std::milli>(std::chrono::steady_clock::now() - t_begin).count();
      c->used_fast_path = true;
      c->device_scheduled = false;
      c->replayed = true;
      c->seed_list_inc = c->counts.n_list_inc;
      resident_mark(c);
      c->resident_valid = true;
      return AM355_OK;
    }
  }
  c->keep.want = false;
  { int orc = flush_uploads(c); if (!orc) orc = upload_offsets(c); if (orc) return orc; }
  const bool trace = getenv("AM355_TRACE") != nullptr;
  auto lap = [&](const char* what) {
    if (trace) fprintf(stderr, "replay: %-28s +%8.3f ms\n", what, std::chrono::duration<double, std::milli>(std::chrono::steady_clock::now() - t_begin).count());
  };
  hipStream_t sa = c->stream, sb = c->stream2;
  uint32_t n = c->n_changes;
  size_t n1 = std::max<size_t>(n, 1);
  c->slot_mask = pow2_at_least(4 * (uint64_t)n + 64) - 1;
  c->hash_mask = pow2_at_least(2 * (uint64_t)n + 64) - 1;
  if (c->amap_cap < 16 * n1 + 1024) c->amap_cap = (uint32_t)(16 * n1 + 1024);
  if (!c->d_entries.ensure(4 * n1) || !c->d_amap_base.ensure(4 * (n1 + 1)) || !c->d_amap_prov.ensure(4 * (size_t)c->amap_cap) ||
      !c->d_slots.ensure(8 * (size_t)(c->slot_mask + 1)) || !c->d_first_idx.ensure(4 * (size_t)(c->slot_mask + 1)) || !c->d_hashes.ensure(32 * n1) ||
      !c->d_hash_tab.ensure(4 * (size_t)(c->hash_mask + 1)) || !c->d_min_idx.ensure(4 * n1) || !c->d_has_dep.ensure(n1) || !c->d_words.ensure(4 * W_NUM) ||
      !c->d_scan1.ensure(scan_workspace_bytes((uint32_t)n1)) || !c->h_slots.ensure(8 * (size_t)(c->slot_mask + 1)) || !c->h_hashes.ensure(32 * n1) ||
      !c->h_has_dep.ensure(n1) || !c->h_words.ensure(4 * W_NUM) || !c->d_plans.ensure(2 * sizeof(ChangePlan) * n1) ||
      !c->d_slot_rank.ensure(4 * (size_t)(c->slot_mask + 1)) || !c->d_plan_sums.ensure(plan_block_sums_bytes(n)) ||
      !c->d_dep_idx.ensure(4 * (c->raw.size() / 32 + 2)) || !c->d_self_idx.ensure(4 * n1) || !c->d_rank_ids.ensure(rank_ids_bytes()))
    return fail(c, AM355_E_NOMEM, "device allocation failed (stage 1)");
  c->have_host_metas = false;
  const size_t s1_distinct = 64, s1_briefs = s1_distinct + ((12 * (size_t)distinct_capacity() + 16 + 63) & ~(size_t)63);
  const size_t s1_bytes = s1_briefs + sizeof(ChangeBrief) * n1;
  if (!c->d_s1.ensure(s1_bytes) || !c->h_s1.ensure(s1_bytes)) return fail(c, AM355_E_NOMEM, "device allocation failed (stage 1)");
  uint32_t* d_wa = c->d_s1.as<uint32_t>();
  uint32_t* d_distinct = (uint32_t*)(c->d_s1.as<uint8_t>() + s1_distinct);
  ChangeBrief* d_briefs = (ChangeBrief*)(c->d_s1.as<uint8_t>() + s1_briefs);
  const uint32_t* h_wa = c->h_s1.as<uint32_t>();
  c->hp_distinct = (uint32_t*)(c->h_s1.as<uint8_t>() + s1_distinct);
  c->hp_briefs = (ChangeBrief*)(c->h_s1.as<uint8_t>() + s1_briefs);
  uint32_t* d_words = c->d_words.as<uint32_t>();
  uint32_t* h_words = c->h_words.as<uint32_t>();
  HostSignals* sig = c->h_sig.as<HostSignals>();
  PlanTotals tot{};
  static const bool hash_after_parse = []() { const char* e = getenv("AM355_HASH_START"); return !(e && !strcmp(e, "intern")); }();

  HIPCHK(c, hipEventRecord(c->ev[0], sa));
  const size_t cb = merge_counts_bytes((uint32_t)std::min<size_t>(c->raw.size(), 0x7ffffff0u));
  c->counts_zeroed_at = nullptr;
  const bool counts_too = c->d_counts.ensure(cb);
  const bool fat_changes = n && c->raw.size() / n > 4096 && !getenv("AM355_PARSE_LEAN");
  if (c->inline_fills) {
    ParseFills f{};
    auto add = [&](void* q, size_t bytes, uint32_t v) { f.p[f.n] = (uint32_t*)q; f.n_words[f.n] = (bytes + 3) / 4; f.value[f.n] = v; f.n++; };
    add(d_words, 4 * W_NUM, 0);
    add(d_wa, s1_distinct + 16, 0);
    add(c->d_slots.p, 8 * (size_t)(c->slot_mask + 1), 0);
    add(c->d_first_idx.p, 4 * (size_t)(c->slot_mask + 1), 0xffffffffu);
    if (counts_too) add(c->d_counts.p, cb, 0);
    launch_parse_changes(c->d_arena.as<uint8_t>(), c->d_offsets.as<uint64_t>(), n, c->d_metas.as<ChangeMeta>(), c->d_entries.as<uint32_t>(), f, sa, fat_changes);
    HIPCHK(c, hipEventRecord(c->ev_parse, sa));
  } else {
    launch_parse_changes(c->d_arena.as<uint8_t>(), c->d_offsets.as<uint64_t>(), n, c->d_metas.as<ChangeMeta>(), c->d_entries.as<uint32_t>(), ParseFills{}, sa, fat_changes);
    HIPCHK(c, hipEventRecord(c->ev_parse, sa));
    HIPCHK(c, hipMemsetAsync(d_words, 0, 4 * W_NUM, c->stream3));
    HIPCHK(c, hipMemsetAsync(d_wa, 0, s1_distinct + 16, c->stream3));
    HIPCHK(c, hipMemsetAsync(c->d_slots.p, 0, 8 * (size_t)(c->slot_mask + 1), c->stream3));
    HIPCHK(c, hipMemsetAsync(c->d_first_idx.p, 0xff, 4 * (size_t)(c->slot_mask + 1), c->stream3));
    if (counts_too) HIPCHK(c, hipMemsetAsync(c->d_counts.p, 0, cb, c->stream3));
    HIPCHK(c, hipEventRecord(c->ev_join, c->stream3));
    HIPCHK(c, hipStreamWaitEvent(sa, c->ev_join, 0));
  }
  if (counts_too) {
    c->counts_zeroed_at = c->d_counts.p;
    c->counts_zeroed = cb;
  }

  auto enqueue_stream_b = [&]() -> int {
    HIPCHK(c, hipStreamWaitEvent(sb, hash_after_parse ? c->ev_parse : c->ev[1], 0));
    if (!c->inline_fills) HIPCHK(c, hipStreamWaitEvent(sb, c->ev_join, 0));
    HIPCHK(c, hipEventRecord(c->ev_b0, sb));
    HIPCHK(c, hipMemsetAsync(c->d_hash_tab.p, 0, 4 * (size_t)(c->hash_mask + 1), sb));
    HIPCHK(c, hipMemsetAsync(c->d_has_dep.p, 0, n1, sb));
    launch_hash_changes(c->d_arena.as<uint8_t>(), c->d_offsets.as<uint64_t>(), n, c->d_hashes.as<uint8_t>(), c->d_min_idx.as<uint32_t>(),
                    c->d_hash_tab.as<uint32_t>(), c->hash_mask, d_words + W_FLAGS_B, sb);
    launch_deps_resolve(c->d_arena.as<uint8_t>(), c->d_metas.as<ChangeMeta>(), c->d_hashes.as<uint8_t>(), n, c->d_hash_tab.as<uint32_t>(), c->hash_mask,
                    c->d_min_idx.as<uint32_t>(), c->d_has_dep.as<uint8_t>(), d_words + W_FAST_B, c->d_dep_idx.as<uint32_t>(), c->d_self_idx.as<uint32_t>(), sb);
    HIPCHK(c, hipMemcpyAsync(c->h_hashes.p, c->d_hashes.p, 32 * (size_t)n, hipMemcpyDeviceToHost, sb));
    HIPCHK(c, hipMemcpyAsync(c->h_has_dep.p, c->d_has_dep.p, n, hipMemcpyDeviceToHost, sb));
    HIPCHK(c, hipMemcpyAsync(h_words + W_FLAGS_B, d_words + W_FLAGS_B, 8, hipMemcpyDeviceToHost, sb));
    HIPCHK(c, hipEventRecord(c->ev_b1, sb));
    return AM355_OK;
  };
  static const bool enqueue_early = []() { const char* e = getenv("AM355_HASH_ENQUEUE"); return e && !strcmp(e, "early"); }();
  static const bool enqueue_thread = AM355_STREAMS_ORDER_ACROSS_THREADS && []() { const char* e = getenv("AM355_HASH_ENQUEUE"); return !e || !strcmp(e, "thread"); }();
  std::atomic<int> lane_rc{AM355_OK};
  struct LaneJoin {
    AsyncLane* l = nullptr;
    ~LaneJoin() { if (l) l->wait(); }
  } lane_join;
  bool b_enqueued = false;
  if (hash_after_parse && enqueue_early) { int rb = enqueue_stream_b(); if (rb) return rb; b_enqueued = true; }
  else if (hash_after_parse && enqueue_thread && n >= 512) {
    if (!c->lane) c->lane.reset(new AsyncLane);
    c->lane->post([&]() { (void)hipSetDevice(c->device); lane_rc.store(enqueue_stream_b()); });
    lane_join.l = c->lane.get();
    b_enqueued = true;
  }
  exclusive_scan_u32(c->d_entries.as<uint32_t>(), c->d_amap_base.as<uint32_t>(), n, d_wa + W_TOTAL_ENTRIES, c->d_scan1.p, sa);
  static const bool spec_env = []() { const char* e = getenv("AM355_SPEC_DECODE"); return !(e && *e == '0'); }();
  const bool spec_possible = spec_env && n && c->inline_fills && counts_too && hash_after_parse && !getenv("AM355_HOST_PLAN") && !(c->in_apply && c->graph_mode != 0) &&
                             c->d_plan_totals.ensure(sizeof(PlanTotals));
  for (int attempt = 0;; attempt++) {
    if (attempt) {
      HIPCHK(c, hipMemsetAsync(c->d_slots.p, 0, 8 * (size_t)(c->slot_mask + 1), sa));
      HIPCHK(c, hipMemsetAsync(c->d_first_idx.p, 0xff, 4 * (size_t)(c->slot_mask + 1), sa));
      HIPCHK(c, hipMemsetAsync(d_distinct, 0, 4, sa));
    }
    launch_actor_intern(c->d_arena.as<uint8_t>(), c->d_metas.as<ChangeMeta>(), n, c->d_amap_base.as<uint32_t>(), c->d_amap_prov.as<uint32_t>(), c->amap_cap,
                        c->d_slots.as<unsigned long long>(), c->slot_mask, c->d_first_idx.as<uint32_t>(), d_wa + W_FLAGS_A, d_wa + W_FAST_A,
                        d_distinct, c->d_rank_ids.p, d_briefs, c->d_slot_rank.as<uint32_t>(), c->d_plan_sums.as<unsigned long long>(), d_wa + 8, sa, c->hp_briefs);
    c->sig_seq++;
    launch_plan(d_briefs, n, d_distinct, c->d_slot_rank.as<uint32_t>(), c->slot_mask, c->d_plan_sums.as<unsigned long long>(), c->d_plans.as<ChangePlan>(),
                c->d_plans.as<ChangePlan>() + n1, d_wa, d_wa + 8, sig, c->sig_seq, sa, spec_possible ? c->d_plan_totals.as<PlanTotals>() : nullptr,
                c->h_s1.as<uint32_t>());
    const bool want_large_spec = spec_possible && attempt == 0 && c->hint_large != 0;
    if (want_large_spec) HIPCHK(c, hipEventRecord(c->ev_plan, sa));
    if (spec_possible && attempt == 0) {
      const uint64_t est = c->raw.size() / 2 + 1024;
      c->spec_cap_ops = (uint32_t)std::min<uint64_t>(std::max<uint64_t>(c->hint_ops, est), 0x7ffffff0u);
      c->spec_cap_preds = (uint32_t)std::min<uint64_t>(std::max<uint64_t>(c->hint_preds, est), 0x7ffffff0u);
      if (trace) fprintf(stderr, "replay: speculative decode: cap %u ops / %u preds (counter block %zu of %zu bytes)\n", c->spec_cap_ops, c->spec_cap_preds, merge_counts_bytes(c->spec_cap_ops), cb);
      if (merge_counts_bytes(c->spec_cap_ops) <= cb && carve_cols(c, c->spec_cap_ops, c->spec_cap_preds, true) == AM355_OK) {
        canary_arm();
        if (c->phase_events) { HIPCHK(c, hipEventRecord(c->ev[1], sa)); HIPCHK(c, hipEventRecord(c->ev[2], sa)); }
        if (want_large_spec) HIPCHK(c, hipStreamWaitEvent(c->stream3, c->ev_plan, 0));
        launch_decode_speculative(c->d_arena.as<uint8_t>(), c->d_metas.as<ChangeMeta>(), c->d_plans.as<ChangePlan>(), n, c->d_plan_totals.as<PlanTotals>(), c->spec_cap_ops,
                                  c->spec_cap_preds, distinct_capacity(), c->d_amap_prov.as<uint32_t>(), c->d_slot_rank.as<uint32_t>(), c->cols,
                                  &c->d_counts.as<Counts>()->flags, sa, c->stream3, want_large_spec, c->shard_rank, c->shard_world);
        c->spec_large_launched = want_large_spec;
        if (c->phase_events) HIPCHK(c, hipEventRecord(c->ev[3], sa));
        c->spec_launched = true;
      }
    }
    if ((c->phase_events && !c->spec_launched) || !hash_after_parse) HIPCHK(c, hipEventRecord(c->ev[1], sa));
    if (attempt == 0 && !b_enqueued) { int rb = enqueue_stream_b(); if (rb) return rb; b_enqueued = true; }
    lap("stage 1 enqueued");
    if (!wait_host_signal(&sig->plan_seq, c->sig_seq, sa)) {
      (void)hipStreamSynchronize(sb);
      (void)hipStreamSynchronize(c->stream3);
      return fail(c, AM355_E_DEVICE, "the device did not report the plan of this replay (%s)", hipGetErrorString(hipGetLastError()));
    }
    memcpy(&tot, (const void*)&sig->plan, sizeof tot);
    lap("stage 1 totals read");
    if (!(tot.fast_a & FF_CAPACITY) || attempt) break;
    c->spec_launched = false;
    c->amap_cap = tot.total_entries + 1024;
    if (!c->d_amap_prov.ensure(4 * (size_t)c->amap_cap)) return fail(c, AM355_E_NOMEM, "device allocation failed (actor tables)");
    HIPCHK(c, hipMemsetAsync(d_wa + W_FAST_A, 0, 4, sa));
    HIPCHK(c, hipMemsetAsync(d_wa + 8, 0, 32, sa));
  }

  auto t_h0 = std::chrono::steady_clock::now();
  float ms_host = 0;
  int rc = AM355_OK;
  if (tot.flags_a) { (void)hipStreamSynchronize(sa); (void)hipStreamSynchronize(sb); return error_for_flags(c, tot.flags_a, "malformed change"); }
  c->has_unknown_cols = tot.reserved[0] != 0;
  bool fast = tot.fast_a == 0;
  const bool lineage_schedule = c->in_apply && c->graph_mode != 0;
  if (lineage_schedule) fast = false;
  if (tot.n_distinct > distinct_capacity()) fast = false;
  const bool planned = !tot.fallback && !getenv("AM355_HOST_PLAN");
  std::vector<uint32_t> slot_rank;
  int opt_rc = AM355_OK;
  uint32_t opt_flags = 0;
  std::string opt_err;
  if (fast && planned) {
    float ms_plan = 0;
    opt_rc = run_device_planned(c, tot, tot.n_distinct, &ms_plan);
    ms_host += ms_plan;
    lap("run_device (device plan) done");
    opt_flags = c->flags;
    opt_err = c->err;
  } else {
    if (tot.fallback) {
      const ChangeBrief* br = c->hp_briefs;
      uint32_t dev_flags = 0;
      c->has_unknown_cols = false;
      for (uint32_t i = 0; i < n; i++) {
        dev_flags |= br[i].flags_fits & 0x1fffffffu;
        if (br[i].flags_fits & 0x20000000u) c->has_unknown_cols = true;
      }
      if (dev_flags) { (void)hipStreamSynchronize(sa); (void)hipStreamSynchronize(sb); return error_for_flags(c, dev_flags, "malformed change"); }
    }
    if (fast) {
      opt_rc = plan_fast(c, slot_rank);
      ms_host += std::chrono::duration<float, std::milli>(std::chrono::steady_clock::now() - t_h0).count();
      lap("plan_fast done");
      if (opt_rc == AM355_OK) opt_rc = run_device(c, &slot_rank);
      lap("run_device done");
      opt_flags = c->flags;
      opt_err = c->err;
    }
  }
  if (lane_join.l) { lane_join.l->wait(); lane_join.l = nullptr; if (lane_rc.load()) return lane_rc.load(); }
  HIPCHK(c, hipEventSynchronize(c->ev_b1));
  lap("hash stream joined");
// ... 144 lines not shown
```

### automerge_classic_amd/csrc/am355_stage.hip

```cpp
#include "am355_ctx.h"
#include "am355_pinflate.h"

bool read_uleb_host(const uint8_t* p, size_t len, size_t& off, uint64_t& out) {
  uint64_t v = 0;
  int shift = 0;
  while (off < len && shift < 64) {
    uint8_t b = p[off++];
    v |= (uint64_t)(b & 0x7f) << shift;
    shift += 7;
    if (!(b & 0x80)) { out = v; return true; }
  }
  return false;
}

constexpr size_t INFLATE_CAP = 0xfff00000ull;

int flush_uploads(am355_ctx* c) {
  if (!c->pending_up.n) return AM355_OK;
  launch_copy_ranges(c->pending_up, c->stream);
  c->pending_up.n = 0;
  HIPCHK(c, hipGetLastError());
  return AM355_OK;
}

int queue_upload(am355_ctx* c, void* dst, const void* src, size_t bytes) {
  if (!bytes) return AM355_OK;
  static const bool off = getenv("AM355_NO_UPLOAD_QUEUE") != nullptr;
  if (off || bytes > ((size_t)256 << 10)) {
    int rc = flush_uploads(c);
    if (rc) return rc;
    HIPCHK(c, hipMemcpyAsync(dst, src, bytes, hipMemcpyHostToDevice, c->stream));
    return AM355_OK;
  }
  if (c->pending_up.n == LAUNCH_RANGES) { int rc = flush_uploads(c); if (rc) return rc; }
  if (!c->pending_up.add(dst, src, bytes)) return fail(c, AM355_E_DEVICE, "upload queue full");
  return AM355_OK;
}

int upload_offsets(am355_ctx* c) {
  if (c->offsets_on_device) return AM355_OK;
  const size_t bytes = sizeof(uint64_t) * ((size_t)c->n_changes + 1);
  if (!c->d_offsets.ensure(bytes) || !c->h_offsets.ensure(bytes)) return fail(c, AM355_E_NOMEM, "device allocation failed");
  memcpy(c->h_offsets.p, c->raw_off.data(), bytes);
  HIPCHK(c, hipMemcpyAsync(c->d_offsets.p, c->h_offsets.p, bytes, hipMemcpyHostToDevice, c->stream));
  c->offsets_on_device = true;
  return AM355_OK;
}

int load_changes_impl(am355_ctx* c, const uint8_t* arena, const uint64_t* offsets, uint32_t n, bool keep_staged) {
  if (!c || (!arena && n) || !offsets) return c ? fail(c, AM355_E_ARG, "null argument") : AM355_E_ARG;
  (void)hipSetDevice(c->device);
  (void)c->doc_sum.wait();
  const uint32_t k0 = keep_staged ? c->n_changes : 0;
  const size_t b0 = keep_staged ? c->raw.size() : 0;
  { int frc = flush_uploads(c); if (frc) return frc; }
  if (c->staging_in_flight) { c->staging_in_flight = false; HIPCHK(c, hipStreamSynchronize(c->stream)); }
  c->staged = c->replayed = c->ir_fetched = false;
  if (!keep_staged) { c->resident_valid = false; c->arena_epoch++; }
  c->apply_ready = false;
  c->state_checked = false;
  c->is_document = false;
  c->flags = 0;
  if (n && offsets[n] - offsets[0] >= ((uint64_t)1 << 20))
    c->pool->prewake(offsets[1] - offsets[0] > 9 && arena[offsets[0] + 8] == 2 ? c->pool->size() : 4);
  for (uint32_t i = 0; i < n; i++)
    if (offsets[i] > offsets[i + 1]) return fail(c, AM355_E_ARG, "change offsets must be ascending (offsets[%u] > offsets[%u])", i, i + 1);
  if (offsets[n] - offsets[0] + b0 >= INFLATE_CAP) { c->flags |= AM355_F_OVERFLOW; return fail(c, AM355_E_UNSUPPORTED, "batch larger than 4 GiB (32-bit arena offsets)"); }
  const size_t in_bytes = (size_t)(offsets[n] - offsets[0]);
  const bool trace = getenv("AM355_TRACE") != nullptr;
  auto t_begin = std::chrono::steady_clock::now();
  auto lap = [&](const char* what) {
    if (trace) fprintf(stderr, "load_changes: %-22s +%8.3f ms\n", what, std::chrono::duration<double, std::milli>(std::chrono::steady_clock::now() - t_begin).count());
  };
  unsigned n_slices = 1;
  const char* slice_env = getenv("AM355_SLICE_BYTES");
  const size_t slice_bytes = slice_env && atol(slice_env) > 0 ? (size_t)atol(slice_env) : (size_t)1 << 21;
  const bool deflated = n && ((offsets[1] - offsets[0] > 9 && arena[offsets[0] + 8] == 2) || (offsets[n / 2 + 1] - offsets[n / 2] > 9 && arena[offsets[n / 2] + 8] == 2));
  const size_t per_slice = deflated && !slice_env ? (size_t)64 << 10 : slice_bytes;
  if (in_bytes >= 2 * per_slice && n >= 16)
    n_slices = (unsigned)std::min<size_t>({(size_t)(c->pool->size() + 1) * (deflated ? 8 : 2), in_bytes / per_slice, (size_t)n / 8});
  if (n_slices < 1) n_slices = 1;
  struct Slice { uint32_t c0 = 0, c1 = 0; size_t out_bytes = 0, base = 0; bool any_deflated = false; int err = 0; uint32_t err_change = 0; std::vector<uint8_t> tmp; std::vector<uint32_t> tmp_len; };
  std::vector<Slice> slices(n_slices);
  {
    uint32_t ci = 0;
    for (unsigned k = 0; k < n_slices; k++) {
      slices[k].c0 = ci;
      uint64_t target = offsets[0] + (uint64_t)in_bytes * (k + 1) / n_slices;
      while (ci < n && (k + 1 == n_slices || offsets[ci + 1] <= target)) ci++;
      slices[k].c1 = ci;
    }
    slices[n_slices - 1].c1 = n;
  }
  auto phase_a = [&](unsigned k) {
    Slice& sl = slices[k];
    for (uint32_t i = sl.c0; i < sl.c1; i++) {
      size_t len = (size_t)(offsets[i + 1] - offsets[i]);
      if (len > 9 && arena[offsets[i] + 8] == 2) { sl.any_deflated = true; break; }
    }
    if (!sl.any_deflated) { sl.out_bytes = (size_t)(offsets[sl.c1] - offsets[sl.c0]); return; }
    sl.tmp_len.resize(sl.c1 - sl.c0);
    std::vector<uint8_t> out;
    for (uint32_t i = sl.c0; i < sl.c1 && !sl.err; i++) {
      const uint8_t* p = arena + offsets[i];
      size_t len = (size_t)(offsets[i + 1] - offsets[i]);
      size_t before = sl.tmp.size();
      if (len > 9 && p[8] == 2) {
        size_t off = 9;
        uint64_t clen;
        if (!read_uleb_host(p, len, off, clen) || clen > len - off) { sl.err = 10; sl.err_change = i; break; }
        int irc = inflate_raw(p + off, (size_t)clen, out, INFLATE_CAP);
        if (irc) { sl.err = irc; sl.err_change = i; break; }
        sl.tmp.insert(sl.tmp.end(), p, p + 8);
        sl.tmp.push_back(1);
        uint64_t v = out.size();
// ... 2 lines not shown
      } else {
        sl.tmp.insert(sl.tmp.end(), p, p + len);
      }
      if (sl.tmp.size() >= INFLATE_CAP) { sl.err = 2; sl.err_change = i; break; }
      sl.tmp_len[i - sl.c0] = (uint32_t)(sl.tmp.size() - before);
    }
    sl.out_bytes = sl.tmp.size();
  };
  c->pool->run(n_slices, phase_a);
  lap("inflate / sizes");
  size_t total = 0;
  for (Slice& sl : slices) {
    if (sl.err == 10) { c->flags |= AM355_F_BAD_CHUNK; return fail(c, AM355_E_INVALID, "change %u: bad deflate container", sl.err_change); }
    if (sl.err == 3) return fail(c, AM355_E_NOMEM, "inflate: out of memory");
    if (sl.err == 2) { c->flags |= AM355_F_OVERFLOW; return fail(c, AM355_E_UNSUPPORTED, "change %u: inflated size beyond the 4 GiB batch limit", sl.err_change); }
    if (sl.err) { c->flags |= AM355_F_BAD_DEFLATE; return fail(c, AM355_E_INVALID, "change %u: invalid or truncated deflate data", sl.err_change); }
    sl.base = total;
    total += sl.out_bytes;
    if (total + b0 >= INFLATE_CAP) { c->flags |= AM355_F_OVERFLOW; return fail(c, AM355_E_UNSUPPORTED, "batch larger than 4 GiB (32-bit arena offsets)"); }
  }
  const uint32_t n_all = k0 + n;
  c->raw.resize(b0 + total);
  c->raw_off.resize((size_t)n_all + 1);
  c->raw_off[n_all] = b0 + total;
  c->n_changes = n_all;
  if (!(keep_staged ? c->d_arena.ensure_keep(b0 + total + 64, b0) : c->d_arena.ensure(total + 64)) || !c->d_offsets.ensure(sizeof(uint64_t) * ((size_t)n_all + 1)) ||
      !(keep_staged ? c->d_metas.ensure_keep(sizeof(ChangeMeta) * (size_t)std::max(n_all, 1u), sizeof(ChangeMeta) * (size_t)k0)
                    : c->d_metas.ensure(sizeof(ChangeMeta) * (size_t)std::max(n_all, 1u))) || !c->h_metas.ensure(sizeof(ChangeMeta) * (size_t)std::max(n_all, 1u)) ||
      !c->d_counts.ensure(sizeof(Counts)) || !c->h_counts.ensure(2 * sizeof(Counts)) || !c->h_offsets.ensure(sizeof(uint64_t) * ((size_t)n_all + 1)))
    return fail(c, AM355_E_NOMEM, "device allocation failed");
  uint8_t* raw = c->raw.data() + b0;
  uint8_t* d_raw = c->d_arena.as<uint8_t>() + b0;
  uint64_t* roff = c->raw_off.data() + k0;
  std::vector<hipError_t> h2d(n_slices, hipSuccess);
  bool any_deflated = false;
  for (const Slice& sl : slices) any_deflated = any_deflated || sl.any_deflated;
  const char* gather_env = getenv("AM355_GATHER_UNIT");
  if (!any_deflated && (total >= ((size_t)4 << 20) || (gather_env && total > 0))) {
    const size_t unit = gather_env && atol(gather_env) > 0 ? (size_t)atol(gather_env) : (size_t)256 << 10;
    const size_t n_units = (total + unit - 1) / unit;
    std::vector<uint32_t> group_of(n_units);
    std::vector<size_t> group_first;
    for (size_t u = 0, span = 1; u < n_units; span = std::min<size_t>(span * 2, 64)) {
      group_first.push_back(u);
      for (size_t k = 0; k < span && u < n_units; k++, u++) group_of[u] = (uint32_t)group_first.size() - 1;
    }
    const size_t n_groups = group_first.size();
    group_first.push_back(n_units);
    std::vector<std::atomic<uint32_t>> left(n_groups);
    for (size_t g = 0; g < n_groups; g++) left[g].store((uint32_t)(group_first[g + 1] - group_first[g]));
    h2d.assign(n_groups, hipSuccess);
    const uint8_t* src = arena + offsets[0];
    const uint64_t off0 = offsets[0];
    std::atomic<size_t> next_unit{0};
    const unsigned n_helpers = (unsigned)std::min<size_t>(4, std::min<size_t>(n_units > 1 ? n_units - 1 : 0, c->pool->size()));
    lap("  buffers ready");
    c->pool->run(n_helpers + 1, [&](unsigned task) {
      const bool issuer = task == 0;
      size_t next_group = 0;
      auto issue_ready = [&]() {
        while (next_group < n_groups && left[next_group].load(std::memory_order_acquire) == 0) {
          size_t gb = group_first[next_group] * unit, ge = std::min(total, group_first[next_group + 1] * unit);
          h2d[next_group] = hipMemcpyAsync(d_raw + gb, raw + gb, ge - gb, hipMemcpyHostToDevice, c->stream);
          if (trace) fprintf(stderr, "load_changes:   group %zu (%zu KiB) enqueued +%8.3f ms\n", next_group, (ge - gb) >> 10, std::chrono::duration<double, std::milli>(std::chrono::steady_clock::now() - t_begin).count());
          next_group++;
        }
      };
      if (issuer) (void)hipSetDevice(c->device);
      for (;;) {
        size_t u = next_unit.fetch_add(1, std::memory_order_relaxed);
        if (u >= n_units) break;
        size_t b = u * unit, e = std::min(total, b + unit);
        memcpy(raw + b, src + b, e - b);
        left[group_of[u]].fetch_sub(1, std::memory_order_acq_rel);
        if (issuer) issue_ready();
      }
      if (issuer) {
        while (next_group < n_groups) {
          issue_ready();
#if defined(__x86_64__)
          __builtin_ia32_pause();
#endif
        }
      }
    });
    for (uint32_t i = 0; i < n; i++) roff[i] = b0 + (offsets[i] - off0);
  } else {
    std::vector<uint32_t> group_of(n_slices);
    std::vector<size_t> group_begin{0};
    {
      size_t acc = 0;
      for (unsigned k = 0; k < n_slices; k++) {
        group_of[k] = (uint32_t)group_begin.size() - 1;
        acc += slices[k].out_bytes;
        if (acc >= ((size_t)2 << 20) && k + 1 < n_slices) { group_begin.push_back(slices[k + 1].base); acc = 0; }
      }
      group_begin.push_back(total);
    }
    const size_t n_groups = group_begin.size() - 1;
    std::vector<std::atomic<uint32_t>> left(n_groups);
    for (auto& x : left) x.store(0);
    for (unsigned k = 0; k < n_slices; k++) left[group_of[k]].fetch_add(1);
    h2d.assign(n_groups, hipSuccess);
    if (n_slices == 1) {
      Slice& sl = slices[0];
      if (sl.any_deflated) {
        if (sl.out_bytes) memcpy(raw, sl.tmp.data(), sl.out_bytes);
        size_t o = b0;
        for (uint32_t i = 0; i < n; i++) { roff[i] = o; o += sl.tmp_len[i]; }
      } else {
        if (sl.out_bytes) memcpy(raw, arena + offsets[0], sl.out_bytes);
        for (uint32_t i = 0; i < n; i++) roff[i] = b0 + (offsets[i] - offsets[0]);
      }
      if (total) {
        if (keep_staged) { int qrc = queue_upload(c, d_raw, raw, total); if (qrc) return qrc; }
        else h2d[0] = hipMemcpyAsync(d_raw, raw, total, hipMemcpyHostToDevice, c->stream);
      }
    } else
    c->pool->run(n_slices + 1, [&](unsigned task) {
      if (task == 0) {
        (void)hipSetDevice(c->device);
        for (size_t g = 0; g < n_groups; g++) {
          while (left[g].load(std::memory_order_acquire) != 0) {
#if defined(__x86_64__)
            __builtin_ia32_pause();
#endif
          }
          size_t gb = group_begin[g], ge = group_begin[g + 1];
          if (ge > gb) h2d[g] = hipMemcpyAsync(d_raw + gb, raw + gb, ge - gb, hipMemcpyHostToDevice, c->stream);
        }
        return;
      }
      Slice& sl = slices[task - 1];
      if (sl.any_deflated) {
        if (sl.out_bytes) memcpy(raw + sl.base, sl.tmp.data(), sl.out_bytes);
        size_t o = b0 + sl.base;
        for (uint32_t i = sl.c0; i < sl.c1; i++) { roff[i] = o; o += sl.tmp_len[i - sl.c0]; }
      } else {
        if (sl.out_bytes) memcpy(raw + sl.base, arena + offsets[sl.c0], sl.out_bytes);
        for (uint32_t i = sl.c0; i < sl.c1; i++) roff[i] = b0 + sl.base + (offsets[i] - offsets[sl.c0]);
      }
      left[group_of[task - 1]].fetch_sub(1, std::memory_order_acq_rel);
    });
  }
  lap("gathered, H2D enqueued");
  for (hipError_t e : h2d)
    if (e != hipSuccess) return fail(c, AM355_E_DEVICE, "hipMemcpyAsync (arena): %s", hipGetErrorString(e));
  c->offsets_on_device = false;
  if (!keep_staged) { int orc = upload_offsets(c); if (orc) return orc; }
  c->staging_in_flight = true;
  static const bool stage_sync = getenv("AM355_STAGE_SYNC") != nullptr;
  if (trace || stage_sync) { c->staging_in_flight = false; HIPCHK(c, hipStreamSynchronize(c->stream)); lap("H2D done"); }
  c->staged = true;
  c->stats = am355_stats{};
  c->stats.n_changes = n_all;
  c->stats.raw_bytes = c->raw.size();
  return AM355_OK;
}

namespace {
struct HostRle {
  const uint8_t* p; size_t len, off = 0; int64_t count = 0; int state = 0; int64_t last = 0; bool last_null = true; bool is_signed;
  HostRle(const uint8_t* p_, size_t l, bool sg) : p(p_), len(l), is_signed(sg) {}
  bool done() const { return count == 0 && off >= len; }
  bool leb(bool sg, int64_t& out) {
    uint64_t v = 0; int shift = 0;
    while (off < len && shift < 64) {
      uint8_t b = p[off++];
      v |= (uint64_t)(b & 0x7f) << shift; shift += 7;
      if (!(b & 0x80)) { if (sg && (b & 0x40) && shift < 64) v |= ~0ull << shift; out = (int64_t)v; return true; }
    }
    return false;
  }
  bool next(bool& is_null, int64_t& v) {
    if (done()) { is_null = true; v = 0; return true; }
    if (count == 0) {
      int64_t n;
      if (!leb(true, n)) return false;
      if (n > 1) { if (!leb(is_signed, last)) return false; last_null = false; state = 1; count = n; }
      else if (n == 1) return false;
      else if (n < 0) { state = 2; count = -n; }
      else { int64_t z; if (!leb(false, z) || z <= 0) return false; state = 3; count = z; last_null = true; }
    }
    count--;
    if (state == 2) { if (!leb(is_signed, last)) return false; last_null = false; }
    is_null = last_null; v = last;
    return true;
  }
};
}

int load_document_impl(am355_ctx* c, const uint8_t* doc, size_t len, bool defer_checksum) {
  if (!c || !doc) return c ? fail(c, AM355_E_ARG, "null argument") : AM355_E_ARG;
  (void)hipSetDevice(c->device);
  (void)c->doc_sum.wait();
  c->resident_valid = false;
  if (c->staging_in_flight) { c->staging_in_flight = false; HIPCHK(c, hipStreamSynchronize(c->stream)); }
  c->doc_graph_known = false;
  c->staged = c->replayed = c->ir_fetched = false;
  c->history_ok = false;
  c->is_document = true;
  c->flags = 0;
  const bool trace = getenv("AM355_TRACE") != nullptr;
  auto t_begin = std::chrono::steady_clock::now();
  auto lap = [&](const char* what) {
    if (trace) fprintf(stderr, "load_document: %-30s +%8.3f ms\n", what, std::chrono::duration<double, std::milli>(std::chrono::steady_clock::now() - t_begin).count());
  };
  auto bad0 = [&](uint32_t flag, const char* msg) { c->flags |= flag; return fail(c, AM355_E_INVALID, "%s", msg); };
  if (len < 10 || doc[0] != 0x85 || doc[1] != 0x6f || doc[2] != 0x4a || doc[3] != 0x83) return bad0(AM355_F_BAD_MAGIC, "Data does not begin with magic bytes 85 6f 4a 83");
  size_t off = 9;
  uint64_t clen;
  if (!read_uleb_host(doc, len, off, clen) || clen != len - off) return bad0(AM355_F_BAD_CHUNK, "Encoded document has trailing data or is truncated");
  if (doc[8] != 0) return bad0(AM355_F_BAD_CHUNK, "Unexpected chunk type");
  c->doc_bytes.resize(len);
  {
    am355_ctx::DocSum& ds = c->doc_sum;
    ds.n_pieces = (len + am355_ctx::DocSum::PIECE - 1) / am355_ctx::DocSum::PIECE;
    ds.copied.reset(new std::atomic<uint8_t>[ds.n_pieces]);
    for (size_t k = 0; k < ds.n_pieces; k++) ds.copied[k].store(0, std::memory_order_relaxed);
    ds.ok = false;
    ds.pending = true;
    const uint8_t* bytes = c->doc_bytes.data();
    const uint8_t want[4] = {doc[4], doc[5], doc[6], doc[7]};
    ds.t = std::thread([&ds, bytes, len, want0 = want[0], want1 = want[1], want2 = want[2], want3 = want[3]]() {
      uint32_t hs[8];
      sha256_initial(hs);
      size_t pos = 8;
      for (size_t k = 0; k < ds.n_pieces; k++) {
        while (!ds.copied[k].load(std::memory_order_acquire)) std::this_thread::yield();
        const size_t end = std::min(len, (k + 1) * am355_ctx::DocSum::PIECE);
        const size_t nb = end > pos ? (end - pos) / 64 : 0;
        sha256_blocks(hs, bytes + pos, nb);
        pos += nb * 64;
      }
      uint8_t digest[32];
      sha256_finish(hs, bytes + pos, len - pos, len - 8, digest);
      ds.ok = digest[0] == want0 && digest[1] == want1 && digest[2] == want2 && digest[3] == want3;
    });
  }
  auto copy_piece = [&](size_t k) {
    const size_t b = k * am355_ctx::DocSum::PIECE, e = std::min(len, b + am355_ctx::DocSum::PIECE);
    memcpy(c->doc_bytes.data() + b, doc + b, e - b);
    c->doc_sum.copied[k].store(1, std::memory_order_release);
  };
  bool copy_done = false;
  auto sum_verdict = [&]() {
    if (!copy_done) {
      for (size_t k = 0; k < c->doc_sum.n_pieces; k++)
        if (!c->doc_sum.copied[k].load(std::memory_order_acquire)) copy_piece(k);
      copy_done = true;
    }
    return c->doc_sum.wait();
  };
  auto bad = [&](uint32_t flag, const char* msg) {
    if (!sum_verdict()) { flag = AM355_F_BAD_CHECKSUM; msg = "checksum does not match data"; }
// ... 304 lines not shown
```

### automerge_classic_amd/engine.py

```python
import ctypes
import os

import numpy as np

_HERE = os.path.dirname(os.path.abspath(__file__))
DEFAULT_LIB = os.path.join(_HERE, "csrc", "libam355.so")

AM355_OK = 0
AM355_E_DEVICE, AM355_E_ARG, AM355_E_INVALID, AM355_E_UNSUPPORTED, AM355_E_STATE, AM355_E_NOMEM = -1, -2, -3, -4, -5, -6

FLAG_NAMES = {
    1 << 0: "BAD_MAGIC", 1 << 1: "BAD_CHECKSUM", 1 << 2: "BAD_CHUNK", 1 << 3: "BAD_COLUMNS", 1 << 4: "BAD_LEB", 1 << 5: "BAD_RLE",
    1 << 6: "BAD_ROW", 1 << 7: "UNKNOWN_OBJECT", 1 << 8: "BAD_ELEM", 1 << 9: "BAD_PRED", 1 << 10: "DUP_OPID", 1 << 11: "BAD_COUNTER",
    1 << 12: "UNSUPPORTED", 1 << 13: "OVERFLOW", 1 << 16: "BAD_SEQ", 1 << 17: "UNKNOWN_ACTOR", 1 << 18: "BAD_DEFLATE",
}


class Stats(ctypes.Structure):
    _fields_ = [
        ("n_changes", ctypes.c_uint32), ("n_applied", ctypes.c_uint32), ("n_pending", ctypes.c_uint32),
        ("n_actors", ctypes.c_uint32), ("n_objects", ctypes.c_uint32), ("n_heads", ctypes.c_uint32),
        ("n_ops", ctypes.c_uint64), ("max_op", ctypes.c_uint64), ("raw_bytes", ctypes.c_uint64),
        ("n_map_values", ctypes.c_uint64), ("n_list_elems", ctypes.c_uint64), ("n_edits", ctypes.c_uint64),
        ("ir_bytes", ctypes.c_uint64),
# ... 15 lines not shown
        self.flag_names = names


class InvalidChanges(EngineError):
    """The reference would throw on this input (the JS host re-runs it on the JS path to raise the exact error)."""


class UnsupportedChanges(EngineError):
    """Legal input outside the GPU-served subset (documented in DESIGN.md); the JS host uses the JS path."""


def _bind(path):
    if not os.path.exists(path):
        raise RuntimeError(f"HIP engine library not found: {path}. Build it with `python -c 'import __graft_entry__ as g; g.build()'` "
                           "(hipcc --offload-arch=gfx950). There is no CPU fallback.")
    L = ctypes.CDLL(path)
    vp, u32, u64p = ctypes.c_void_p, ctypes.c_uint32, ctypes.c_void_p
    L.am355_create.restype = vp
    L.am355_create.argtypes = [ctypes.c_int]
    L.am355_destroy.argtypes = [vp]
    L.am355_last_error.restype = ctypes.c_char_p
    L.am355_last_error.argtypes = [vp]
    L.am355_flags.restype = u32
    L.am355_flags.argtypes = [vp]
    L.am355_load_changes.argtypes = [vp, vp, u64p, u32]
    L.am355_load_document.argtypes = [vp, vp, ctypes.c_size_t]
    if hasattr(L, "am355_backend_load"):
        L.am355_backend_load.argtypes = [vp, vp, ctypes.c_size_t]
        L.am355_backend_load.restype = ctypes.c_int
    L.am355_replay.argtypes = [vp]
    L.am355_patch_json.argtypes = [vp, ctypes.POINTER(ctypes.c_char_p), ctypes.POINTER(ctypes.c_size_t)]
    L.am355_get_stats.argtypes = [vp, ctypes.POINTER(Stats)]
    L.am355_get_hashes.argtypes = [vp, vp]
    L.am355_test_sort.argtypes = [vp, vp, vp, u32, ctypes.c_int]
    L.am355_test_scan.argtypes = [vp, vp, vp, u32, vp]
    L.am355_get_rows.argtypes = [vp] * 15
    L.am355_save.argtypes = [vp, u32, ctypes.POINTER(ctypes.c_void_p), ctypes.POINTER(ctypes.c_size_t)]
    L.am355_get_applied.argtypes = [vp, vp, ctypes.POINTER(u32)]
    L.am355_fetch_ir.argtypes = [vp, vp]
    L.am355_set_shard.argtypes = [vp, u32, u32]
    L.am355_fragment_size.argtypes = [vp, ctypes.POINTER(ctypes.c_size_t)]
    L.am355_export_fragment.argtypes = [vp, vp, ctypes.c_size_t, ctypes.c_int, ctypes.POINTER(ctypes.c_size_t)]
    L.am355_import_fragments.argtypes = [vp, vp, vp, u32]
    L.am355_shard_unique_id.argtypes = [vp]
    L.am355_shard_init.argtypes = [vp, vp, u32, u32]
    L.am355_sharded_replay.argtypes = [vp, ctypes.c_int]
    L.am355_shard_fragment_bytes.argtypes = [vp, vp, u32]
    L.am355_shard_finalize.argtypes = [vp]
    for f in ("am355_shard_unique_id", "am355_shard_init", "am355_sharded_replay", "am355_shard_fragment_bytes", "am355_shard_finalize"):
        getattr(L, f).restype = ctypes.c_int
    if hasattr(L, "am355_resident_counters"):
        L.am355_resident_counters.argtypes = [vp, vp]
        L.am355_resident_counters.restype = ctypes.c_int
    if hasattr(L, "am355_resident_maps_only_calls"):
        L.am355_resident_maps_only_calls.argtypes = [vp, ctypes.POINTER(ctypes.c_uint64)]
        L.am355_resident_maps_only_calls.restype = ctypes.c_int
    L.am355_get_raw.argtypes = [vp, ctypes.POINTER(ctypes.c_void_p), ctypes.POINTER(ctypes.c_void_p), ctypes.POINTER(u32)]
    L.am355_doc_changes.argtypes = [vp, u32, ctypes.POINTER(ctypes.c_void_p), ctypes.POINTER(ctypes.c_void_p), ctypes.POINTER(u32), ctypes.POINTER(ctypes.c_void_p)]
    L.am355_apply_changes.argtypes = [vp, vp, u64p, u32]
    L.am355_apply_patch_json.argtypes = [vp, ctypes.POINTER(ctypes.c_char_p), ctypes.POINTER(ctypes.c_size_t)]
    L.am355_fetch_apply_ir.argtypes = [vp, vp]
    L.am355_reset.argtypes = [vp]
    L.am355_get_dep_graph.argtypes = [vp, ctypes.POINTER(ctypes.c_void_p), ctypes.POINTER(ctypes.c_void_p), ctypes.POINTER(u32)]
    L.am355_sync_bloom_build.argtypes = [vp, vp, u32, vp, ctypes.c_size_t]
    L.am355_sync_bloom_probe.argtypes = [vp, vp, u32, u32, u32, u32, vp, ctypes.c_size_t, vp]
    L.am355_get_pending.argtypes = [vp, vp, ctypes.POINTER(u32)]
    L.am355_forget_call_history.argtypes = [vp, ctypes.c_int]
    L.am355_hash_graph_known.argtypes = [vp, ctypes.c_int, ctypes.POINTER(ctypes.c_int)]
    L.am355_set_phase_events.argtypes = [vp, ctypes.c_int]
    for f in ("am355_load_changes", "am355_load_document", "am355_replay", "am355_patch_json", "am355_get_stats", "am355_get_hashes", "am355_test_sort",
              "am355_test_scan", "am355_get_rows", "am355_save", "am355_get_applied", "am355_fetch_ir", "am355_get_raw", "am355_set_shard", "am355_fragment_size", "am355_export_fragment",
              "am355_import_fragments", "am355_doc_changes", "am355_apply_changes", "am355_apply_patch_json", "am355_fetch_apply_ir", "am355_reset", "am355_get_pending", "am355_forget_call_history", "am355_hash_graph_known", "am355_set_phase_events", "am355_get_dep_graph", "am355_sync_bloom_build", "am355_sync_bloom_probe"):
        getattr(L, f).restype = ctypes.c_int
    return L


_libs = {}


def load_library(path=DEFAULT_LIB):
    if path not in _libs:
        _libs[path] = _bind(path)
    return _libs[path]


class Engine:

    def __init__(self, device=0, lib_path=DEFAULT_LIB):
        self._L = load_library(lib_path)
        self.device = device
        self.lib_path = lib_path
        self._h = self._L.am355_create(device)
        if not self._h:
            raise RuntimeError("am355_create failed: no usable MI355X / HIP device (the engine has no CPU fallback)")
        self._n_changes = 0

    def set_phase_events(self, on):
        self._check(self._L.am355_set_phase_events(self._h, 1 if on else 0))

    def close(self):
        if getattr(self, "_h", None):
            self._L.am355_destroy(self._h)
            self._h = None

    def __del__(self):
        try:
# ... 103 lines not shown
        out = np.zeros(n.value, dtype=np.uint32)
        self._check(self._L.am355_get_applied(self._h, out.ctypes.data if n.value else None, ctypes.byref(n)))
        return out

    def stats(self):
        s = Stats()
        self._check(self._L.am355_get_stats(self._h, ctypes.byref(s)))
        return s

    def set_shard(self, rank, world):
        self._check(self._L.am355_set_shard(self._h, rank, world))

    def fragment_size(self):
        n = ctypes.c_size_t()
        self._check(self._L.am355_fragment_size(self._h, ctypes.byref(n)))
        return n.value

    def export_fragment(self, ptr, capacity, device):
        n = ctypes.c_size_t()
        self._check(self._L.am355_export_fragment(self._h, ctypes.c_void_p(ptr), capacity, 1 if device else 0, ctypes.byref(n)))
        return n.value

    def import_fragments(self, frags, offsets):
        f = np.ascontiguousarray(frags, dtype=np.uint8)
        o = np.ascontiguousarray(offsets, dtype=np.uint64)
        self._check(self._L.am355_import_fragments(self._h, f.ctypes.data, o.ctypes.data, o.size - 1))

    def shard_unique_id(self):
        buf = (ctypes.c_uint8 * 128)()
        if self._L.am355_shard_unique_id(buf) != AM355_OK:
            raise EngineError(AM355_E_DEVICE, "RCCL is not available (librccl.so.1, or AM355_RCCL_LIB)")
        return bytes(buf)

    def shard_init(self, unique_id, rank, world):
        assert len(unique_id) == 128
        self._check(self._L.am355_shard_init(self._h, ctypes.c_char_p(bytes(unique_id)), rank, world))

    def sharded_replay(self, stitch_on_all_ranks=False):
        self._check(self._L.am355_sharded_replay(self._h, 1 if stitch_on_all_ranks else 0))

    def shard_fragment_bytes(self, world):
        out = np.zeros(world, dtype=np.uint64)
        self._check(self._L.am355_shard_fragment_bytes(self._h, out.ctypes.data, world))
        return out

    def shard_finalize(self):
        self._check(self._L.am355_shard_finalize(self._h))

    def resident_counters(self):
        out = (ctypes.c_uint64 * 3)()
        self._check(self._L.am355_resident_counters(self._h, out))
        return int(out[0]), int(out[1]), int(out[2])

    def resident_maps_only_calls(self):
        out = ctypes.c_uint64()
        self._check(self._L.am355_resident_maps_only_calls(self._h, ctypes.byref(out)))
        return int(out.value)

    def raw(self):
        a, o, n = ctypes.c_void_p(), ctypes.c_void_p(), ctypes.c_uint32()
        self._check(self._L.am355_get_raw(self._h, ctypes.byref(a), ctypes.byref(o), ctypes.byref(n)))
        offs = np.ctypeslib.as_array(ctypes.cast(o, ctypes.POINTER(ctypes.c_uint64)), shape=(n.value + 1,)).copy()
        size = int(offs[-1])
        arena = np.ctypeslib.as_array(ctypes.cast(a, ctypes.POINTER(ctypes.c_uint8)), shape=(size,)).copy() if size else np.zeros(0, dtype=np.uint8)
        return arena, offs

    def doc_changes(self, deflate=True):
        a, o, n, h = ctypes.c_void_p(), ctypes.c_void_p(), ctypes.c_uint32(), ctypes.c_void_p()
        self._check(self._L.am355_doc_changes(self._h, 1 if deflate else 0, ctypes.byref(a), ctypes.byref(o), ctypes.byref(n), ctypes.byref(h)))
        offs = np.ctypeslib.as_array(ctypes.cast(o, ctypes.POINTER(ctypes.c_uint64)), shape=(n.value + 1,)).copy()
        size = int(offs[-1])
        arena = np.ctypeslib.as_array(ctypes.cast(a, ctypes.POINTER(ctypes.c_uint8)), shape=(size,)).copy() if size else np.zeros(0, dtype=np.uint8)
        hashes = np.ctypeslib.as_array(ctypes.cast(h, ctypes.POINTER(ctypes.c_uint8)), shape=(n.value, 32)).copy() if n.value else np.zeros((0, 32), dtype=np.uint8)
        return arena, offs, hashes

    def hashes(self):
        out = np.zeros((self._n_changes, 32), dtype=np.uint8)
        self._check(self._L.am355_get_hashes(self._h, out.ctypes.data))
        return out

    def test_sort(self, keys, vals, key_bits=64):
        k = np.ascontiguousarray(keys, dtype=np.uint64).copy()
        v = np.ascontiguousarray(vals, dtype=np.uint32).copy()
        self._check(self._L.am355_test_sort(self._h, k.ctypes.data, v.ctypes.data, k.size, key_bits))
        return k, v

    def test_scan(self, values):
        a = np.ascontiguousarray(values, dtype=np.uint32)
        out = np.zeros_like(a)
        total = np.zeros(1, dtype=np.uint32)
        self._check(self._L.am355_test_scan(self._h, a.ctypes.data, out.ctypes.data, a.size, total.ctypes.data))
        return out, int(total[0])

    def rows(self):
        n = int(self.stats().n_ops)
        names = ["obj_actor", "obj_ctr", "key_actor", "key_ctr", "key_off", "key_len", "action", "val_tl", "val_off", "pred_num",
                 "id_ctr", "id_actor", "insert", "succ_cnt"]
        arrs = {k: np.zeros(n, dtype=np.uint8 if k == "insert" else np.uint32) for k in names}
        self._check(self._L.am355_get_rows(self._h, *[arrs[k].ctypes.data for k in names]))
        return arrs


def replay_patch_json(log, device=0, lib_path=DEFAULT_LIB):
    eng = Engine(device, lib_path)
    try:
        eng.load_changes(log)
# ... 5 lines not shown
```

### include/am355.h

```cpp
#ifndef AM355_H
#define AM355_H
#include <stddef.h>
#include <stdint.h>

#ifdef __cplusplus
extern "C" {
#endif

typedef struct am355_ctx am355_ctx;

enum {
  AM355_OK = 0,
  AM355_E_DEVICE = -1,
  AM355_E_ARG = -2,
  AM355_E_INVALID = -3,
  AM355_E_UNSUPPORTED = -4,
  AM355_E_STATE = -5,
  AM355_E_NOMEM = -6
};

enum {
  AM355_F_BAD_MAGIC = 1u << 0, AM355_F_BAD_CHECKSUM = 1u << 1, AM355_F_BAD_CHUNK = 1u << 2, AM355_F_BAD_COLUMNS = 1u << 3,
  AM355_F_BAD_LEB = 1u << 4, AM355_F_BAD_RLE = 1u << 5, AM355_F_BAD_ROW = 1u << 6, AM355_F_UNKNOWN_OBJECT = 1u << 7,
  AM355_F_BAD_ELEM = 1u << 8, AM355_F_BAD_PRED = 1u << 9, AM355_F_DUP_OPID = 1u << 10, AM355_F_BAD_COUNTER = 1u << 11,
// ... 73 lines not shown
  uint32_t val_tl;
  uint32_t val_off;
  uint32_t pad;
} am355_ir_edit;

typedef struct {
  uint32_t n_objects, n_map, n_edits, n_values;
  const am355_ir_object *objects;
  const am355_ir_map *map;
  const am355_ir_edit *edits;
  uint64_t max_op;
  uint32_t n_actors;
  const uint32_t *actor_off;
  const uint8_t *actor_bytes;
  uint32_t n_clock;
  const uint32_t *clock_actor;
  const uint64_t *clock_seq;
  uint32_t n_heads;
  const uint8_t *heads;
  uint32_t pending;
  const uint8_t *arena;
  uint64_t arena_len;
} am355_patch_ir;
int am355_fetch_ir(am355_ctx *ctx, am355_patch_ir *out);

int am355_apply_changes(am355_ctx *ctx, const uint8_t *arena, const uint64_t *offsets, uint32_t n_changes);
int am355_reset(am355_ctx *ctx);
int am355_forget_call_history(am355_ctx *ctx, int from_document);
int am355_hash_graph_known(am355_ctx *ctx, int set, int *known);

int am355_get_pending(const am355_ctx *ctx, uint32_t *out, uint32_t *n_pending);
int am355_apply_patch_json(am355_ctx *ctx, const char **json, size_t *len);
int am355_fetch_apply_ir(am355_ctx *ctx, am355_patch_ir *out);

int am355_get_dep_graph(am355_ctx *ctx, const uint32_t **dep_first, const uint32_t **dep_index, uint32_t *n_changes);
int am355_sync_bloom_build(am355_ctx *ctx, const uint32_t *idx, uint32_t n, uint8_t *bits, size_t capacity);
int am355_sync_bloom_probe(am355_ctx *ctx, const uint32_t *idx, uint32_t n, uint32_t num_entries, uint32_t bits_per_entry, uint32_t num_probes,
                           const uint8_t *bits, size_t n_bytes, uint8_t *contains);

int am355_set_shard(am355_ctx *ctx, uint32_t rank, uint32_t world);
int am355_fragment_size(am355_ctx *ctx, size_t *bytes);
int am355_export_fragment(am355_ctx *ctx, void *dst, size_t capacity, int dst_is_device, size_t *len);
int am355_import_fragments(am355_ctx *ctx, const uint8_t *frags, const uint64_t *offsets, uint32_t world);

#define AM355_SHARD_ID_BYTES 128
int am355_shard_unique_id(uint8_t id[AM355_SHARD_ID_BYTES]);
int am355_shard_init(am355_ctx *ctx, const uint8_t id[AM355_SHARD_ID_BYTES], uint32_t rank, uint32_t world);
int am355_sharded_replay(am355_ctx *ctx, int stitch_on_all_ranks);
int am355_shard_fragment_bytes(am355_ctx *ctx, uint64_t *bytes, uint32_t capacity);
int am355_shard_finalize(am355_ctx *ctx);

int am355_resident_counters(const am355_ctx *ctx, uint64_t out[3]);
int am355_resident_maps_only_calls(const am355_ctx *ctx, uint64_t *out);

int am355_arena_epoch(const am355_ctx *ctx, uint64_t *epoch);
int am355_get_hashes_range(const am355_ctx *ctx, uint32_t first, uint32_t count, uint8_t *out);
int am355_applied_in_input_order(const am355_ctx *ctx, int *yes);

int am355_test_sort(am355_ctx *ctx, uint64_t *keys, uint32_t *vals, uint32_t n, int key_bits);
int am355_test_scan(am355_ctx *ctx, const uint32_t *in, uint32_t *out, uint32_t n, uint32_t *total);
int am355_get_rows(am355_ctx *ctx, uint32_t *obj_actor, uint32_t *obj_ctr, uint32_t *key_actor, uint32_t *key_ctr, uint32_t *key_off,
                   uint32_t *key_len, uint32_t *action, uint32_t *val_tl, uint32_t *val_off, uint32_t *pred_num, uint32_t *id_ctr,
                   uint32_t *id_actor, uint8_t *insert, uint32_t *succ_cnt);

#ifdef __cplusplus
}
#endif
#endif
```

Baseline: 1.220 billion.

## Split replay at last H2D group to decode head while tail uploads

Staging records an event once all but the last upload group are enqueued and computes a split change index. Replay then runs actor interning, planning and speculative decode on the head changes while the tail is still being copied, then reranks head plans and decodes the remainder. The aim is to overlap host-to-device transfer with early decode work. In exchange it adds range-parameterised kernels, a rerank pass, extra events and a discard path when capacity gates fail, which adds complexity and some risk of wasted work.

```diff
diff --git a/automerge_classic_amd/csrc/am355_api.hip b/automerge_classic_amd/csrc/am355_api.hip
--- a/automerge_classic_amd/csrc/am355_api.hip
+++ b/automerge_classic_amd/csrc/am355_api.hip
@@ -28,7 +28,7 @@
   }
   if (!make_stream(c->stream3, prio_high) || !make_stream(c->stream4, prio_high)) return false;
   for (Event* e : {&c->ev_fork, &c->ev_join, &c->ev[0], &c->ev[1], &c->ev[2], &c->ev[3], &c->ev[4], &c->ev[5], &c->ev[6], &c->ev[7], &c->ev_parse, &c->ev_b0, &c->ev_b1,
-                   &c->ev_counts, &c->ev_runs, &c->ev_s1, &c->ev_plan, &c->ev_tables, &c->ev_fills, &c->ev_sched})
+                   &c->ev_counts, &c->ev_runs, &c->ev_s1, &c->ev_plan, &c->ev_tables, &c->ev_fills, &c->ev_sched, &c->ev_head_ready, &c->ev_head_done, &c->ev_rewrite})
     if (hipEventCreate(&e->h) != hipSuccess) return false;
   if (!c->h_sig.ensure(sizeof(HostSignals))) return false;
   memset(c->h_sig.p, 0, sizeof(HostSignals));
@@ -111,6 +111,14 @@
   out[0] = c->n_resident_calls;
   out[1] = c->n_resident_fallbacks;
   out[2] = c->n_resorder_calls;
+  return AM355_OK;
+}
+
+extern "C" int am355_split_counters(const am355_ctx* c, uint64_t out[3]) {
+  if (!c || !out) return AM355_E_ARG;
+  out[0] = c->n_split_kept;
+  out[1] = c->n_split_discarded;
+  out[2] = c->n_split_untaken;
   return AM355_OK;
 }
 
diff --git a/automerge_classic_amd/csrc/am355_ctx.h b/automerge_classic_amd/csrc/am355_ctx.h
--- a/automerge_classic_amd/csrc/am355_ctx.h
+++ b/automerge_classic_amd/csrc/am355_ctx.h
@@ -312,6 +312,11 @@
   bool prefetch_ir = false;
   bool has_unknown_cols = false;
   bool staging_in_flight = false;
+  uint32_t split_change = 0;
+  bool split_fresh = false;
+  bool split_taken = false;
+  Event ev_head_ready, ev_head_done, ev_rewrite;
+  uint64_t n_split_kept = 0, n_split_discarded = 0, n_split_untaken = 0;
   bool is_document = false;
   ChangeMeta doc_meta{};
   std::vector<uint32_t> doc_actor_rank;
diff --git a/automerge_classic_amd/csrc/am355_decode.h b/automerge_classic_amd/csrc/am355_decode.h
--- a/automerge_classic_amd/csrc/am355_decode.h
+++ b/automerge_classic_amd/csrc/am355_decode.h
@@ -19,16 +19,22 @@
 void launch_actor_intern(const uint8_t* arena, ChangeMeta* metas, uint32_t n, const uint32_t* amap_base, uint32_t* amap, uint32_t amap_cap,
                          unsigned long long* slots, uint32_t slot_mask, uint32_t* first_idx, uint32_t* flags, uint32_t* fast_flags, uint32_t* distinct,
                          void* rank_ids, ChangeBrief* briefs, uint32_t* slot_rank, unsigned long long* block_sums, uint32_t* plan_words, hipStream_t st,
-                         ChangeBrief* host_briefs = nullptr);
+                         ChangeBrief* host_briefs = nullptr, PlanRange r = PlanRange{});
+uint32_t plan_range_blocks(uint32_t n_changes);
 size_t rank_ids_bytes();
 size_t plan_block_sums_bytes(uint32_t n);
 uint32_t distinct_capacity();
 void launch_plan(const ChangeBrief* briefs, uint32_t n, const uint32_t* distinct, const uint32_t* slot_rank, uint32_t slot_mask, const unsigned long long* block_sums,
                  ChangePlan* plans, ChangePlan* plans_serial, const uint32_t* words, const uint32_t* plan_words, HostSignals* sig, uint32_t seq, hipStream_t st,
-                 PlanTotals* dev_totals = nullptr, uint32_t* host_s1 = nullptr);
+                 PlanTotals* dev_totals = nullptr, uint32_t* host_s1 = nullptr, PlanRange r = PlanRange{}, uint32_t n_all = 0);
 void launch_decode_speculative(const uint8_t* arena, const ChangeMeta* metas, const ChangePlan* plans, uint32_t n_changes, const PlanTotals* totals, uint32_t cap_ops,
                                uint32_t cap_preds, uint32_t cap_distinct, const uint32_t* amap, const uint32_t* slot_rank, OpCols cols, uint32_t* flags, hipStream_t st,
-                               hipStream_t aux, bool with_large, uint32_t shard_rank = 0, uint32_t shard_world = 1);
+                               hipStream_t aux, bool with_large, uint32_t shard_rank = 0, uint32_t shard_world = 1, const PlanTotals* head_totals = nullptr,
+                               uint32_t n_head = 0, bool with_small = true);
+void launch_decode_head(const uint8_t* arena, const ChangeMeta* metas, const ChangePlan* plans, uint32_t n_head, uint32_t n_changes, const PlanTotals* head_totals,
+                        uint32_t cap_ops, uint32_t cap_preds, uint32_t cap_distinct, const uint32_t* amap, OpCols cols, uint32_t* flags, hipStream_t st);
+void launch_head_rerank(OpCols cols, ChangePlan* plans, ChangePlan* plans_serial, uint32_t n_changes, const PlanTotals* head_totals, const PlanTotals* totals,
+                        uint32_t cap_ops, uint32_t cap_preds, uint32_t cap_distinct, const uint32_t* slot_rank, uint32_t slot_mask, hipStream_t st);
 void launch_decode_planned(const uint8_t* arena, const ChangeMeta* metas, const ChangePlan* plans, const ChangePlan* plans_serial, uint32_t n_changes,
                            uint32_t n_small, uint32_t n_large, uint32_t n_serial, const uint32_t* amap, const uint32_t* slot_rank, OpCols cols, uint32_t* flags,
                            hipStream_t st, hipStream_t aux, uint32_t shard_rank = 0, uint32_t shard_world = 1);
diff --git a/automerge_classic_amd/csrc/am355_decode.hip b/automerge_classic_amd/csrc/am355_decode.hip
--- a/automerge_classic_amd/csrc/am355_decode.hip
+++ b/automerge_classic_amd/csrc/am355_decode.hip
@@ -942,10 +942,10 @@
                                                         const uint32_t* __restrict__ amap_base, uint32_t* __restrict__ amap, uint32_t amap_cap,
                                                         unsigned long long* __restrict__ slots, uint32_t mask, uint32_t* __restrict__ first_idx,
                                                         uint32_t* __restrict__ flags, uint32_t* __restrict__ fast_flags, uint32_t* __restrict__ distinct,
-                                                        RankId* __restrict__ rank_ids) {
+                                                        RankId* __restrict__ rank_ids, uint32_t c0) {
   __shared__ uint32_t s_off[WAVE], s_len[WAVE];
   wave_priority_high();
-  uint32_t c = blockIdx.x, lane = threadIdx.x;
+  uint32_t c = c0 + blockIdx.x, lane = threadIdx.x;
   if (c >= n) return;
   ChangeMeta* m = &metas[c];
   if (m->flags) return;
@@ -1077,9 +1077,9 @@
 
 __global__ __launch_bounds__(WAVE) void k_actor_first(ChangeMeta* __restrict__ metas, uint32_t n, const uint32_t* __restrict__ amap_base,
                                                        const uint32_t* __restrict__ amap, uint32_t amap_cap, const uint32_t* __restrict__ first_idx,
-                                                       uint32_t* __restrict__ fast_flags) {
+                                                       uint32_t* __restrict__ fast_flags, uint32_t c0) {
   wave_priority_high();
-  uint32_t c = blockIdx.x, lane = threadIdx.x;
+  uint32_t c = c0 + blockIdx.x, lane = threadIdx.x;
   if (c >= n) return;
   ChangeMeta* m = &metas[c];
   if (m->flags) return;
@@ -1105,14 +1105,14 @@
                                                        const uint32_t* __restrict__ first_idx, uint32_t* __restrict__ flags, uint32_t* __restrict__ fast_flags,
                                                        ChangeBrief* __restrict__ briefs, const uint32_t* __restrict__ distinct, const RankId* __restrict__ rank_ids,
                                                        uint32_t* __restrict__ slot_rank, unsigned long long* __restrict__ block_sums, uint32_t* __restrict__ plan_words,
-                                                       ChangeBrief* __restrict__ host_briefs) {
+                                                       ChangeBrief* __restrict__ host_briefs, uint32_t c0, uint32_t bs0, uint32_t with_rank) {
   wave_priority_high();
   __shared__ unsigned long long s_scan[BLOCK / WAVE][3];
-  if (blockIdx.x + 1 == gridDim.x) {
+  if (with_rank && blockIdx.x + 1 == gridDim.x) {
     rank_actors(distinct, rank_ids, slot_rank, plan_words);
     return;
   }
-  uint32_t c = gtid();
+  uint32_t c = c0 + gtid();
   const bool in_range = c < n;
   ChangeBrief br{};
   if (in_range) {
@@ -1152,7 +1152,7 @@
     if (unknown) atomicOr(&plan_words[3], 1u);
   }
   if (threadIdx.x == 0) {
-    unsigned long long* out = block_sums + (size_t)blockIdx.x * PLAN_SUMS;
+    unsigned long long* out = block_sums + (size_t)(bs0 + blockIdx.x) * PLAN_SUMS;
     out[0] = t1[0]; out[1] = t1[1]; out[2] = t1[2]; out[3] = t2[0]; out[4] = t2[1]; out[5] = t2[2];
   }
 }
@@ -1161,13 +1161,13 @@
                                                       const unsigned long long* __restrict__ block_sums, ChangePlan* __restrict__ plans,
                                                       ChangePlan* __restrict__ plans_serial, const uint32_t* __restrict__ words, const uint32_t* __restrict__ plan_words,
                                                       const uint32_t* __restrict__ distinct, HostSignals* sig, uint32_t seq, PlanTotals* __restrict__ dev_totals,
-                                                      uint32_t* __restrict__ host_s1) {
+                                                      uint32_t* __restrict__ host_s1, uint32_t c0, uint32_t bs0, uint32_t n_all) {
   wave_priority_high();
   __shared__ unsigned long long s_scan[BLOCK / WAVE][3];
   __shared__ unsigned long long s_base[6];
   {
     unsigned long long p0 = 0, p1 = 0, p2 = 0, p3 = 0, p4 = 0, p5 = 0;
-    for (uint32_t j = threadIdx.x; j < blockIdx.x; j += BLOCK) {
+    for (uint32_t j = threadIdx.x; j < bs0 + blockIdx.x; j += BLOCK) {
       const unsigned long long* q = block_sums + (size_t)j * PLAN_SUMS;
       p0 += q[0]; p1 += q[1]; p2 += q[2]; p3 += q[3]; p4 += q[4]; p5 += q[5];
     }
@@ -1177,7 +1177,7 @@
     if (threadIdx.x == 0) { s_base[0] = t1[0]; s_base[1] = t1[1]; s_base[2] = t1[2]; s_base[3] = t2[0]; s_base[4] = t2[1]; s_base[5] = t2[2]; }
     __syncthreads();
   }
-  const uint32_t c = gtid();
+  const uint32_t c = c0 + gtid();
   const bool in_range = c < n;
   ChangeBrief br{};
   if (in_range) br = briefs[c];
@@ -1189,9 +1189,9 @@
   block_scan3(small ? 1u : 0u, large ? 1u : 0u, serial ? 1u : 0u, s_scan, e2, t2);
   if (has) {
     ChangePlan pl{c, (uint32_t)(s_base[0] + e1[0]), (uint32_t)(s_base[1] + e1[1]), (uint32_t)(s_base[2] + e1[2]),
-                  br.author_slot <= slot_mask ? slot_rank[br.author_slot] : 0u, br.n_entries};
+                  br.author_slot <= slot_mask ? (slot_rank ? slot_rank[br.author_slot] : br.author_slot) : 0u, br.n_entries};
     if (small) plans[(uint32_t)(s_base[3] + e2[0])] = pl;
-    else if (large) plans[n - 1 - (uint32_t)(s_base[4] + e2[1])] = pl;
+    else if (large) plans[n_all - 1 - (uint32_t)(s_base[4] + e2[1])] = pl;
     else plans_serial[(uint32_t)(s_base[5] + e2[2])] = pl;
   }
   if (blockIdx.x + 1 == gridDim.x && host_s1) {
@@ -1216,7 +1216,7 @@
     z.flags_a = words[0] | plan_words[2]; z.fast_a = words[1]; z.total_entries = words[2]; z.n_distinct = distinct[0];
     z.reserved[0] = plan_words[3];
     if (dev_totals) *dev_totals = z;
-    signal_host((uint32_t*)&sig->plan, (const uint32_t*)&z, sizeof(PlanTotals) / 4, &sig->plan_seq, seq);
+    if (sig) signal_host((uint32_t*)&sig->plan, (const uint32_t*)&z, sizeof(PlanTotals) / 4, &sig->plan_seq, seq);
   }
 }
 
@@ -1962,6 +1962,11 @@
     if (!decode_gate_open(t, gate.cap_ops, gate.cap_preds, gate.cap_distinct)) return;
     n_plans = gate.large ? t.n_large : t.n_small;
     if (gate.large) plans += gate.n_changes - t.n_large;
+    else if (gate.head) {
+      const uint32_t first = gate.head->n_small;
+      plans += first;
+      n_plans -= first;
+    }
   }
   if (pi >= n_plans) return;
   const ChangePlan pl = plans[pi];
@@ -2234,15 +2239,20 @@
 void launch_actor_intern(const uint8_t* arena, ChangeMeta* metas, uint32_t n, const uint32_t* amap_base, uint32_t* amap, uint32_t amap_cap,
                          unsigned long long* slots, uint32_t slot_mask, uint32_t* first_idx, uint32_t* flags, uint32_t* fast_flags, uint32_t* distinct,
                          void* rank_ids, ChangeBrief* briefs, uint32_t* slot_rank, unsigned long long* block_sums, uint32_t* plan_words, hipStream_t st,
-                         ChangeBrief* host_briefs) {
-  if (n)
-    hipLaunchKernelGGL(k_actor_intern, dim3(n), dim3(WAVE), 0, st, arena, metas, n, amap_base, amap, amap_cap, slots, slot_mask, first_idx, flags,
-                       fast_flags, distinct, (RankId*)rank_ids);
-  if (n) hipLaunchKernelGGL(k_actor_first, dim3(n), dim3(WAVE), 0, st, metas, n, amap_base, (const uint32_t*)amap, amap_cap, (const uint32_t*)first_idx, fast_flags);
-  hipLaunchKernelGGL(k_actor_check, dim3((n + BLOCK - 1) / BLOCK + 1), dim3(BLOCK), 0, st, arena, metas, n, amap_base, (const uint32_t*)amap, amap_cap,
-                     (const uint32_t*)first_idx, flags, fast_flags, briefs, (const uint32_t*)distinct, (const RankId*)rank_ids, slot_rank, block_sums, plan_words,
-                     host_briefs);
-}
+                         ChangeBrief* host_briefs, PlanRange r) {
+  const uint32_t m = n - r.c0;
+  if (m)
+    hipLaunchKernelGGL(k_actor_intern, dim3(m), dim3(WAVE), 0, st, arena, metas, n, amap_base, amap, amap_cap, slots, slot_mask, first_idx, flags,
+                       fast_flags, distinct, (RankId*)rank_ids, r.c0);
+  if (m) hipLaunchKernelGGL(k_actor_first, dim3(m), dim3(WAVE), 0, st, metas, n, amap_base, (const uint32_t*)amap, amap_cap, (const uint32_t*)first_idx, fast_flags, r.c0);
+  const uint32_t nb = (m + BLOCK - 1) / BLOCK + (r.with_rank ? 1u : 0u);
+  if (nb)
+    hipLaunchKernelGGL(k_actor_check, dim3(nb), dim3(BLOCK), 0, st, arena, metas, n, amap_base, (const uint32_t*)amap, amap_cap,
+                       (const uint32_t*)first_idx, flags, fast_flags, briefs, (const uint32_t*)distinct, (const RankId*)rank_ids, slot_rank, block_sums, plan_words,
+                       host_briefs, r.c0, r.bs0, r.with_rank ? 1u : 0u);
+}
+
+uint32_t plan_range_blocks(uint32_t n_changes) { return (n_changes + BLOCK - 1) / BLOCK; }
 
 size_t rank_ids_bytes() { return sizeof(RankId) * PLAN_RANK_MAX; }
 
@@ -2250,10 +2260,10 @@
 
 void launch_plan(const ChangeBrief* briefs, uint32_t n, const uint32_t* distinct, const uint32_t* slot_rank, uint32_t slot_mask, const unsigned long long* block_sums,
                  ChangePlan* plans, ChangePlan* plans_serial, const uint32_t* words, const uint32_t* plan_words, HostSignals* sig, uint32_t seq, hipStream_t st,
-                 PlanTotals* dev_totals, uint32_t* host_s1) {
-  uint32_t nb = (n + BLOCK - 1) / BLOCK;
+                 PlanTotals* dev_totals, uint32_t* host_s1, PlanRange r, uint32_t n_all) {
+  uint32_t nb = (n - r.c0 + BLOCK - 1) / BLOCK;
   hipLaunchKernelGGL(k_plan_apply, dim3(nb ? nb : 1), dim3(BLOCK), 0, st, briefs, n, slot_rank, slot_mask, block_sums, plans, plans_serial, words, plan_words,
-                     distinct, sig, seq, dev_totals, host_s1);
+                     distinct, sig, seq, dev_totals, host_s1, r.c0, r.bs0, n_all ? n_all : n);
 }
 
 uint32_t distinct_capacity() { return DISTINCT_CAP; }
@@ -2335,14 +2345,73 @@
 
 void launch_decode_speculative(const uint8_t* arena, const ChangeMeta* metas, const ChangePlan* plans, uint32_t n_changes, const PlanTotals* totals, uint32_t cap_ops,
                                uint32_t cap_preds, uint32_t cap_distinct, const uint32_t* amap, const uint32_t* slot_rank, OpCols cols, uint32_t* flags, hipStream_t st,
-                               hipStream_t aux, bool with_large, uint32_t shard_rank, uint32_t shard_world) {
+                               hipStream_t aux, bool with_large, uint32_t shard_rank, uint32_t shard_world, const PlanTotals* head_totals, uint32_t n_head,
+                               bool with_small) {
   if (!n_changes) return;
   ActorXlate x{amap, slot_rank, shard_rank, shard_world};
-  hipLaunchKernelGGL(k_decode_wave<WaveLdsSmall>, dim3(n_changes, decode_group_split(n_changes, shard_world)), dim3(WAVE), 0, st, arena, metas, plans, 0u, x, cols, flags,
-                     DecodeGate{totals, cap_ops, cap_preds, cap_distinct, n_changes, 0u});
+  const uint32_t n_mine = head_totals ? n_changes - n_head : n_changes;
+  if (with_small)
+  hipLaunchKernelGGL(k_decode_wave<WaveLdsSmall>, dim3(n_mine, decode_group_split(n_mine, shard_world)), dim3(WAVE), 0, st, arena, metas, plans, 0u, x, cols, flags,
+                     DecodeGate{totals, cap_ops, cap_preds, cap_distinct, n_changes, 0u, head_totals});
   if (with_large)
     hipLaunchKernelGGL(k_decode_wave<WaveLdsLarge>, dim3(n_changes, decode_group_split(n_changes, shard_world, true)), dim3(WAVE), 0, aux, arena, metas, plans, 0u, x, cols, flags,
                        DecodeGate{totals, cap_ops, cap_preds, cap_distinct, n_changes, 1u});
 }
 
-}
+
+__device__ __forceinline__ uint32_t slot_to_rank(uint32_t v, const uint32_t* __restrict__ slot_rank, uint32_t slot_mask) {
+  return v <= slot_mask ? slot_rank[v] : v;
+}
+__device__ __forceinline__ uint4 slot_to_rank4(uint4 v, const uint32_t* __restrict__ slot_rank, uint32_t slot_mask) {
+  return uint4{slot_to_rank(v.x, slot_rank, slot_mask), slot_to_rank(v.y, slot_rank, slot_mask), slot_to_rank(v.z, slot_rank, slot_mask),
+               slot_to_rank(v.w, slot_rank, slot_mask)};
+}
+__global__ __launch_bounds__(BLOCK) void k_head_rerank(OpCols o, ChangePlan* __restrict__ plans, ChangePlan* __restrict__ plans_serial, uint32_t n_changes,
+                                                       const PlanTotals* __restrict__ head, const PlanTotals* __restrict__ totals, uint32_t cap_ops,
+                                                       uint32_t cap_preds, uint32_t cap_distinct, const uint32_t* __restrict__ slot_rank, uint32_t slot_mask) {
+  const PlanTotals h = *head, t = *totals;
+  if (t.fallback) return;
+  const uint32_t tid = gtid(), nth = gridDim.x * BLOCK;
+  for (uint32_t i = tid; i < h.n_small && i < n_changes; i += nth) plans[i].author = slot_to_rank(plans[i].author, slot_rank, slot_mask);
+  for (uint32_t i = tid; i < h.n_large && i < n_changes; i += nth) plans[n_changes - 1 - i].author = slot_to_rank(plans[n_changes - 1 - i].author, slot_rank, slot_mask);
+  for (uint32_t i = tid; i < h.n_serial && i < n_changes; i += nth) plans_serial[i].author = slot_to_rank(plans_serial[i].author, slot_rank, slot_mask);
+  if (!decode_gate_open(t, cap_ops, cap_preds, cap_distinct)) return;
+  const uint32_t n_ops = h.n_ops <= cap_ops ? h.n_ops : 0u, n_preds = h.n_preds <= cap_preds ? h.n_preds : 0u;
+  {
+    uint4* a = (uint4*)o.obj_actor; uint4* b = (uint4*)o.key_actor; uint4* c = (uint4*)o.id_actor;
+    const uint32_t n4 = n_ops / 4;
+    for (uint32_t i = tid; i < n4; i += nth) {
+      const uint4 va = a[i], vb = b[i], vc = c[i];
+      a[i] = slot_to_rank4(va, slot_rank, slot_mask);
+      b[i] = slot_to_rank4(vb, slot_rank, slot_mask);
+      c[i] = slot_to_rank4(vc, slot_rank, slot_mask);
+    }
+    for (uint32_t i = 4 * n4 + tid; i < n_ops; i += nth) {
+      o.obj_actor[i] = slot_to_rank(o.obj_actor[i], slot_rank, slot_mask);
+      o.key_actor[i] = slot_to_rank(o.key_actor[i], slot_rank, slot_mask);
+      o.id_actor[i] = slot_to_rank(o.id_actor[i], slot_rank, slot_mask);
+    }
+  }
+  {
+    uint4* a = (uint4*)o.pred_actor;
+    const uint32_t n4 = n_preds / 4;
+    for (uint32_t i = tid; i < n4; i += nth) a[i] = slot_to_rank4(a[i], slot_rank, slot_mask);
+    for (uint32_t i = 4 * n4 + tid; i < n_preds; i += nth) o.pred_actor[i] = slot_to_rank(o.pred_actor[i], slot_rank, slot_mask);
+  }
+}
+
+void launch_decode_head(const uint8_t* arena, const ChangeMeta* metas, const ChangePlan* plans, uint32_t n_head, uint32_t n_changes, const PlanTotals* head_totals,
+                        uint32_t cap_ops, uint32_t cap_preds, uint32_t cap_distinct, const uint32_t* amap, OpCols cols, uint32_t* flags, hipStream_t st) {
+  if (!n_head) return;
+  ActorXlate x{amap, nullptr, 0, 1};
+  hipLaunchKernelGGL(k_decode_wave<WaveLdsSmall>, dim3(n_head, decode_group_split(n_head, 1)), dim3(WAVE), 0, st, arena, metas, plans, 0u, x, cols, flags,
+                     DecodeGate{head_totals, cap_ops, cap_preds, cap_distinct, n_changes, 0u, nullptr});
+}
+
+void launch_head_rerank(OpCols cols, ChangePlan* plans, ChangePlan* plans_serial, uint32_t n_changes, const PlanTotals* head_totals, const PlanTotals* totals,
+                        uint32_t cap_ops, uint32_t cap_preds, uint32_t cap_distinct, const uint32_t* slot_rank, uint32_t slot_mask, hipStream_t st) {
+  hipLaunchKernelGGL(k_head_rerank, dim3(1024), dim3(BLOCK), 0, st, cols, plans, plans_serial, n_changes, head_totals, totals, cap_ops, cap_preds, cap_distinct,
+                     slot_rank, slot_mask);
+}
+
+}
diff --git a/automerge_classic_amd/csrc/am355_internal.h b/automerge_classic_amd/csrc/am355_internal.h
--- a/automerge_classic_amd/csrc/am355_internal.h
+++ b/automerge_classic_amd/csrc/am355_internal.h
@@ -60,6 +60,11 @@
 struct DecodeGate {
   const PlanTotals* totals = nullptr;
   uint32_t cap_ops = 0, cap_preds = 0, cap_distinct = 0, n_changes = 0, large = 0;
+  const PlanTotals* head = nullptr;
+};
+struct PlanRange {
+  uint32_t c0 = 0, bs0 = 0;
+  bool with_rank = true;
 };
 
 struct HostSignals {
diff --git a/automerge_classic_amd/csrc/am355_prims.h b/automerge_classic_amd/csrc/am355_prims.h
--- a/automerge_classic_amd/csrc/am355_prims.h
+++ b/automerge_classic_amd/csrc/am355_prims.h
@@ -32,7 +32,8 @@
 void launch_signal_words(const uint32_t* src_a, uint32_t n_a, const uint32_t* src_b, uint32_t n_b, uint32_t* host_words, volatile uint32_t* host_seq, uint32_t seq,
                          hipStream_t st);
 size_t scan_workspace_bytes(uint32_t n);
-void exclusive_scan_u32(const uint32_t* in, uint32_t* out, uint32_t n, uint32_t* d_total, void* ws, hipStream_t st);
+void exclusive_scan_u32(const uint32_t* in, uint32_t* out, uint32_t n, uint32_t* d_total, void* ws, hipStream_t st, const uint32_t* d_start = nullptr);
+uint32_t scan_start_max();
 void exclusive_scan_terminators(const uint8_t* bytes, uint32_t L, uint32_t* out, uint32_t* d_total, void* ws, hipStream_t st);
 void exclusive_scan2_u32(const uint32_t* in_a, uint32_t* out_a, uint32_t* d_total_a, const uint32_t* in_b, uint32_t* out_b, uint32_t* d_total_b, uint32_t n,
                          void* ws, hipStream_t st);
diff --git a/automerge_classic_amd/csrc/am355_prims.hip b/automerge_classic_amd/csrc/am355_prims.hip
--- a/automerge_classic_amd/csrc/am355_prims.hip
+++ b/automerge_classic_amd/csrc/am355_prims.hip
@@ -55,7 +55,8 @@
 
 template <bool PREFIXED>
 __global__ __launch_bounds__(BLOCK) void k_scan_apply(const uint32_t* __restrict__ in, uint32_t* __restrict__ out,
-                                                      const uint32_t* __restrict__ tile_sums, uint32_t n, uint32_t* __restrict__ grand_total) {
+                                                      const uint32_t* __restrict__ tile_sums, uint32_t n, uint32_t* __restrict__ grand_total,
+                                                      const uint32_t* __restrict__ start) {
   __shared__ uint32_t s[BLOCK / WAVE];
   uint32_t before;
   if (PREFIXED) before = tile_sums[blockIdx.x];
@@ -63,6 +64,7 @@
     uint32_t part = 0;
     for (uint32_t k = threadIdx.x; k < blockIdx.x; k += BLOCK) part += tile_sums[k];
     before = block_sum_u32(part, s);
+    if (start) before += *start;
   }
   static_assert(SCAN_ITEMS == 8, "k_scan_apply moves a thread's stretch as two uint4");
   uint32_t base = blockIdx.x * SCAN_TILE + threadIdx.x * SCAN_ITEMS;
@@ -193,10 +195,11 @@
   }
 }
 
-__global__ __launch_bounds__(BLOCK) void k_scan_single(const uint32_t* __restrict__ in, uint32_t* __restrict__ out, uint32_t n, uint32_t* __restrict__ grand_total) {
+__global__ __launch_bounds__(BLOCK) void k_scan_single(const uint32_t* __restrict__ in, uint32_t* __restrict__ out, uint32_t n, uint32_t* __restrict__ grand_total,
+                                                       const uint32_t* __restrict__ start) {
   wave_priority_high();
   __shared__ uint32_t s[BLOCK / WAVE];
-  uint32_t carry = 0;
+  uint32_t carry = start ? *start : 0u;
   for (uint32_t tile = 0; tile < n; tile += SCAN_TILE) {
     uint32_t base = tile + threadIdx.x * SCAN_ITEMS;
     uint32_t v[SCAN_ITEMS];
@@ -361,7 +364,9 @@
 
 size_t scan_workspace_bytes(uint32_t n) { return 2 * sizeof(uint32_t) * ((size_t)(n + SCAN_TILE - 1) / SCAN_TILE + 2); }
 
-void exclusive_scan_u32(const uint32_t* in, uint32_t* out, uint32_t n, uint32_t* d_total, void* ws, hipStream_t st) {
+uint32_t scan_start_max() { return SCAN_TILE * SCAN_TWO_LAUNCH_TILES; }
+
+void exclusive_scan_u32(const uint32_t* in, uint32_t* out, uint32_t n, uint32_t* d_total, void* ws, hipStream_t st, const uint32_t* d_start) {
   uint32_t n_tiles = (n + SCAN_TILE - 1) / SCAN_TILE;
   uint32_t* sums = (uint32_t*)ws;
   if (n_tiles == 0) {
@@ -369,12 +374,12 @@
     return;
   }
   if (n <= SCAN_SINGLE) {
-    hipLaunchKernelGGL(k_scan_single, dim3(1), dim3(BLOCK), 0, st, in, out, n, d_total);
+    hipLaunchKernelGGL(k_scan_single, dim3(1), dim3(BLOCK), 0, st, in, out, n, d_total, d_start);
     return;
   }
   if (n_tiles <= SCAN_TWO_LAUNCH_TILES) {
     hipLaunchKernelGGL(k_scan_tile_sums, dim3(n_tiles), dim3(BLOCK), 0, st, in, sums, n);
-    hipLaunchKernelGGL(k_scan_apply<false>, dim3(n_tiles), dim3(BLOCK), 0, st, in, out, (const uint32_t*)sums, n, d_total);
+    hipLaunchKernelGGL(k_scan_apply<false>, dim3(n_tiles), dim3(BLOCK), 0, st, in, out, (const uint32_t*)sums, n, d_total, d_start);
     return;
   }
   const char* lb_env = getenv("AM355_SCAN_LOOKBACK");
@@ -388,7 +393,7 @@
   }
   hipLaunchKernelGGL(k_scan_tile_sums, dim3(n_tiles), dim3(BLOCK), 0, st, in, sums, n);
   hipLaunchKernelGGL(k_scan_sums, dim3(1), dim3(BLOCK), 0, st, sums, n_tiles, d_total);
-  hipLaunchKernelGGL(k_scan_apply<true>, dim3(n_tiles), dim3(BLOCK), 0, st, in, out, (const uint32_t*)sums, n, (uint32_t*)nullptr);
+  hipLaunchKernelGGL(k_scan_apply<true>, dim3(n_tiles), dim3(BLOCK), 0, st, in, out, (const uint32_t*)sums, n, (uint32_t*)nullptr, (const uint32_t*)nullptr);
 }
 
 constexpr int SORT_ITEMS = 8;
diff --git a/automerge_classic_amd/csrc/am355_replay.hip b/automerge_classic_amd/csrc/am355_replay.hip
--- a/automerge_classic_amd/csrc/am355_replay.hip
+++ b/automerge_classic_amd/csrc/am355_replay.hip
@@ -643,6 +643,12 @@
   lap("buffers carved");
   const bool spec_done = c->spec_launched && decode_gate_open(tot, c->spec_cap_ops, c->spec_cap_preds, distinct_capacity()) &&
                          c->counts_zeroed_at == c->d_counts.p && c->mb.counts_bytes <= c->counts_zeroed;
+  if (c->split_taken) {
+    HIPCHK(c, hipStreamWaitEvent(c->stream3, c->ev_rewrite, 0));
+    if (spec_done) c->n_split_kept++;
+    else { c->n_split_discarded++; HIPCHK(c, hipStreamSynchronize(c->stream4)); }
+    c->split_taken = false;
+  }
   if (trace && c->spec_launched && !spec_done)
     fprintf(stderr, "  planned: speculative decode not usable: ops %u / cap %u, preds %u / cap %u, distinct %u, fast_a %x flags_a %x fallback %u, counts %p/%p %zu/%zu\n", tot.n_ops,
             c->spec_cap_ops, tot.n_preds, c->spec_cap_preds, tot.n_distinct, tot.fast_a, tot.flags_a, tot.fallback, c->counts_zeroed_at, c->d_counts.p, c->mb.counts_bytes, c->counts_zeroed);
@@ -1401,6 +1407,11 @@
   }
   c->keep.want = false;
   { int orc = flush_uploads(c); if (!orc) orc = upload_offsets(c); if (orc) return orc; }
+  const uint32_t staged_split = c->split_change;
+  const bool split_fresh = c->split_fresh;
+  c->split_change = 0;
+  c->split_fresh = false;
+  c->split_taken = false;
   const bool trace = getenv("AM355_TRACE") != nullptr;
   auto lap = [&](const char* what) {
     if (trace) fprintf(stderr, "replay: %-28s +%8.3f ms\n", what, std::chrono::duration<double, std::milli>(std::chrono::steady_clock::now() - t_begin).count());
@@ -1440,6 +1451,30 @@
   c->counts_zeroed_at = nullptr;
   const bool counts_too = c->d_counts.ensure(cb);
   const bool fat_changes = n && c->raw.size() / n > 4096 && !getenv("AM355_PARSE_LEAN");
+  static const bool spec_env = []() { const char* e = getenv("AM355_SPEC_DECODE"); return !(e && *e == '0'); }();
+  const bool spec_possible = spec_env && n && c->inline_fills && counts_too && hash_after_parse && !getenv("AM355_HOST_PLAN") && !(c->in_apply && c->graph_mode != 0) &&
+                             c->d_plan_totals.ensure(2 * sizeof(PlanTotals));
+  const uint64_t spec_est = c->raw.size() / 2 + 1024;
+  const uint32_t spec_cap_ops = (uint32_t)std::min<uint64_t>(std::max<uint64_t>(c->hint_ops, spec_est), 0x7ffffff0u);
+  const uint32_t spec_cap_preds = (uint32_t)std::min<uint64_t>(std::max<uint64_t>(c->hint_preds, spec_est), 0x7ffffff0u);
+  uint32_t split = 0;
+  bool split_forced = false;
+  {
+    const char* off_env = getenv("AM355_SPLIT");
+    const char* at_env = getenv("AM355_SPLIT_AT");
+    uint32_t want = staged_split;
+    if (at_env && *at_env) { want = (uint32_t)strtoul(at_env, nullptr, 10); split_forced = true; }
+    const bool had_point = split_fresh && (split_forced || staged_split != 0);
+    bool go = had_point && want > 0 && want < n && c->staging_in_flight && spec_possible && c->shard_world == 1 && !c->phase_events &&
+              !(off_env && *off_env == '0') && n - want <= scan_start_max() && want <= scan_start_max();
+    if (go && !(merge_counts_bytes(spec_cap_ops) <= cb && carve_cols(c, spec_cap_ops, spec_cap_preds, true) == AM355_OK)) go = false;
+    if (go) split = want;
+    else if (had_point) c->n_split_untaken++;
+  }
+  hipStream_t sh = c->stream4;
+  uint32_t* d_head_entries = d_wa + 5;
+  PlanTotals* d_head_totals = spec_possible ? c->d_plan_totals.as<PlanTotals>() + 1 : nullptr;
+  const uint32_t head_blocks = plan_range_blocks(split);
   if (c->inline_fills) {
     ParseFills f{};
     auto add = [&](void* q, size_t bytes, uint32_t v) { f.p[f.n] = (uint32_t*)q; f.n_words[f.n] = (bytes + 3) / 4; f.value[f.n] = v; f.n++; };
@@ -1448,6 +1483,28 @@
     add(c->d_slots.p, 8 * (size_t)(c->slot_mask + 1), 0);
     add(c->d_first_idx.p, 4 * (size_t)(c->slot_mask + 1), 0xffffffffu);
     if (counts_too) add(c->d_counts.p, cb, 0);
+    if (split) {
+      if (split_forced) HIPCHK(c, hipEventRecord(c->ev_head_ready, sa));
+      HIPCHK(c, hipStreamWaitEvent(sh, c->ev_head_ready, 0));
+      launch_parse_changes(c->d_arena.as<uint8_t>(), c->d_offsets.as<uint64_t>(), split, c->d_metas.as<ChangeMeta>(), c->d_entries.as<uint32_t>(), f, sh, fat_changes);
+      exclusive_scan_u32(c->d_entries.as<uint32_t>(), c->d_amap_base.as<uint32_t>(), split, d_head_entries, c->d_scan1.p, sh);
+      launch_actor_intern(c->d_arena.as<uint8_t>(), c->d_metas.as<ChangeMeta>(), split, c->d_amap_base.as<uint32_t>(), c->d_amap_prov.as<uint32_t>(), c->amap_cap,
+                          c->d_slots.as<unsigned long long>(), c->slot_mask, c->d_first_idx.as<uint32_t>(), d_wa + W_FLAGS_A, d_wa + W_FAST_A,
+                          d_distinct, c->d_rank_ids.p, d_briefs, c->d_slot_rank.as<uint32_t>(), c->d_plan_sums.as<unsigned long long>(), d_wa + 8, sh, c->hp_briefs,
+                          PlanRange{0, 0, false});
+      launch_plan(d_briefs, split, d_distinct, nullptr, c->slot_mask, c->d_plan_sums.as<unsigned long long>(), c->d_plans.as<ChangePlan>(),
+                  c->d_plans.as<ChangePlan>() + n1, d_wa, d_wa + 8, nullptr, 0, sh, d_head_totals, nullptr, PlanRange{0, 0, false}, n);
+      c->spec_cap_ops = spec_cap_ops;
+      c->spec_cap_preds = spec_cap_preds;
+      canary_arm();
+      launch_decode_head(c->d_arena.as<uint8_t>(), c->d_metas.as<ChangeMeta>(), c->d_plans.as<ChangePlan>(), split, n, d_head_totals, spec_cap_ops, spec_cap_preds,
+                         distinct_capacity(), c->d_amap_prov.as<uint32_t>(), c->cols, &c->d_counts.as<Counts>()->flags, sh);
+      HIPCHK(c, hipEventRecord(c->ev_head_done, sh));
+      HIPCHK(c, hipStreamWaitEvent(sa, c->ev_head_done, 0));
+      launch_parse_changes(c->d_arena.as<uint8_t>(), c->d_offsets.as<uint64_t>() + split, n - split, c->d_metas.as<ChangeMeta>() + split,
+                           c->d_entries.as<uint32_t>() + split, ParseFills{}, sa, fat_changes);
+      c->split_taken = true;
+    } else
     launch_parse_changes(c->d_arena.as<uint8_t>(), c->d_offsets.as<uint64_t>(), n, c->d_metas.as<ChangeMeta>(), c->d_entries.as<uint32_t>(), f, sa, fat_changes);
     HIPCHK(c, hipEventRecord(c->ev_parse, sa));
   } else {
@@ -1497,11 +1554,13 @@
     lane_join.l = c->lane.get();
     b_enqueued = true;
   }
-  exclusive_scan_u32(c->d_entries.as<uint32_t>(), c->d_amap_base.as<uint32_t>(), n, d_wa + W_TOTAL_ENTRIES, c->d_scan1.p, sa);
-  static const bool spec_env = []() { const char* e = getenv("AM355_SPEC_DECODE"); return !(e && *e == '0'); }();
-  const bool spec_possible = spec_env && n && c->inline_fills && counts_too && hash_after_parse && !getenv("AM355_HOST_PLAN") && !(c->in_apply && c->graph_mode != 0) &&
-                             c->d_plan_totals.ensure(sizeof(PlanTotals));
+  if (split)
+    exclusive_scan_u32(c->d_entries.as<uint32_t>() + split, c->d_amap_base.as<uint32_t>() + split, n - split, d_wa + W_TOTAL_ENTRIES, c->d_scan1.p, sa, d_head_entries);
+  else
+    exclusive_scan_u32(c->d_entries.as<uint32_t>(), c->d_amap_base.as<uint32_t>(), n, d_wa + W_TOTAL_ENTRIES, c->d_scan1.p, sa);
   for (int attempt = 0;; attempt++) {
+    const bool split_now = split && attempt == 0;
+    const PlanRange range = split_now ? PlanRange{split, head_blocks, true} : PlanRange{};
     if (attempt) {
       HIPCHK(c, hipMemsetAsync(c->d_slots.p, 0, 8 * (size_t)(c->slot_mask + 1), sa));
       HIPCHK(c, hipMemsetAsync(c->d_first_idx.p, 0xff, 4 * (size_t)(c->slot_mask + 1), sa));
@@ -1509,17 +1568,32 @@
     }
     launch_actor_intern(c->d_arena.as<uint8_t>(), c->d_metas.as<ChangeMeta>(), n, c->d_amap_base.as<uint32_t>(), c->d_amap_prov.as<uint32_t>(), c->amap_cap,
                         c->d_slots.as<unsigned long long>(), c->slot_mask, c->d_first_idx.as<uint32_t>(), d_wa + W_FLAGS_A, d_wa + W_FAST_A,
-                        d_distinct, c->d_rank_ids.p, d_briefs, c->d_slot_rank.as<uint32_t>(), c->d_plan_sums.as<unsigned long long>(), d_wa + 8, sa, c->hp_briefs);
+                        d_distinct, c->d_rank_ids.p, d_briefs, c->d_slot_rank.as<uint32_t>(), c->d_plan_sums.as<unsigned long long>(), d_wa + 8, sa, c->hp_briefs, range);
     c->sig_seq++;
     launch_plan(d_briefs, n, d_distinct, c->d_slot_rank.as<uint32_t>(), c->slot_mask, c->d_plan_sums.as<unsigned long long>(), c->d_plans.as<ChangePlan>(),
                 c->d_plans.as<ChangePlan>() + n1, d_wa, d_wa + 8, sig, c->sig_seq, sa, spec_possible ? c->d_plan_totals.as<PlanTotals>() : nullptr,
-                c->h_s1.as<uint32_t>());
+                c->h_s1.as<uint32_t>(), PlanRange{range.c0, range.bs0, false}, n);
     const bool want_large_spec = spec_possible && attempt == 0 && c->hint_large != 0;
-    if (want_large_spec) HIPCHK(c, hipEventRecord(c->ev_plan, sa));
-    if (spec_possible && attempt == 0) {
-      const uint64_t est = c->raw.size() / 2 + 1024;
-      c->spec_cap_ops = (uint32_t)std::min<uint64_t>(std::max<uint64_t>(c->hint_ops, est), 0x7ffffff0u);
-      c->spec_cap_preds = (uint32_t)std::min<uint64_t>(std::max<uint64_t>(c->hint_preds, est), 0x7ffffff0u);
+    if (want_large_spec || split_now) HIPCHK(c, hipEventRecord(c->ev_plan, sa));
+    if (split_now) {
+      launch_decode_speculative(c->d_arena.as<uint8_t>(), c->d_metas.as<ChangeMeta>(), c->d_plans.as<ChangePlan>(), n, c->d_plan_totals.as<PlanTotals>(), c->spec_cap_ops,
+                                c->spec_cap_preds, distinct_capacity(), c->d_amap_prov.as<uint32_t>(), c->d_slot_rank.as<uint32_t>(), c->cols,
+                                &c->d_counts.as<Counts>()->flags, sa, c->stream3, false, c->shard_rank, c->shard_world, d_head_totals, split);
+      HIPCHK(c, hipStreamWaitEvent(sh, c->ev_plan, 0));
+      launch_head_rerank(c->cols, c->d_plans.as<ChangePlan>(), c->d_plans.as<ChangePlan>() + n1, n, d_head_totals, c->d_plan_totals.as<PlanTotals>(), c->spec_cap_ops,
+                         c->spec_cap_preds, distinct_capacity(), c->d_slot_rank.as<uint32_t>(), c->slot_mask, sh);
+      HIPCHK(c, hipEventRecord(c->ev_rewrite, sh));
+      if (want_large_spec) {
+        HIPCHK(c, hipStreamWaitEvent(c->stream3, c->ev_rewrite, 0));
+        launch_decode_speculative(c->d_arena.as<uint8_t>(), c->d_metas.as<ChangeMeta>(), c->d_plans.as<ChangePlan>(), n, c->d_plan_totals.as<PlanTotals>(), c->spec_cap_ops,
+                                  c->spec_cap_preds, distinct_capacity(), c->d_amap_prov.as<uint32_t>(), c->d_slot_rank.as<uint32_t>(), c->cols,
+                                  &c->d_counts.as<Counts>()->flags, sa, c->stream3, true, c->shard_rank, c->shard_world, nullptr, 0, false);
+      }
+      c->spec_large_launched = want_large_spec;
+      c->spec_launched = true;
+    } else if (spec_possible && attempt == 0) {
+      c->spec_cap_ops = spec_cap_ops;
+      c->spec_cap_preds = spec_cap_preds;
       if (trace) fprintf(stderr, "replay: speculative decode: cap %u ops / %u preds (counter block %zu of %zu bytes)\n", c->spec_cap_ops, c->spec_cap_preds, merge_counts_bytes(c->spec_cap_ops), cb);
       if (merge_counts_bytes(c->spec_cap_ops) <= cb && carve_cols(c, c->spec_cap_ops, c->spec_cap_preds, true) == AM355_OK) {
         canary_arm();
@@ -1543,6 +1617,12 @@
     }
     memcpy(&tot, (const void*)&sig->plan, sizeof tot);
     lap("stage 1 totals read");
+    if (c->split_taken && !decode_gate_open(tot, c->spec_cap_ops, c->spec_cap_preds, distinct_capacity())) {
+      HIPCHK(c, hipStreamWaitEvent(sa, c->ev_rewrite, 0));
+      c->counts_zeroed_at = nullptr;
+      c->split_taken = false;
+      c->n_split_discarded++;
+    }
     if (!(tot.fast_a & FF_CAPACITY) || attempt) break;
     c->spec_launched = false;
     c->amap_cap = tot.total_entries + 1024;
diff --git a/automerge_classic_amd/csrc/am355_stage.hip b/automerge_classic_amd/csrc/am355_stage.hip
--- a/automerge_classic_amd/csrc/am355_stage.hip
+++ b/automerge_classic_amd/csrc/am355_stage.hip
@@ -61,6 +61,8 @@
   c->state_checked = false;
   c->is_document = false;
   c->flags = 0;
+  c->split_change = 0;
+  c->split_fresh = false;
   if (n && offsets[n] - offsets[0] >= ((uint64_t)1 << 20))
     c->pool->prewake(offsets[1] - offsets[0] > 9 && arena[offsets[0] + 8] == 2 ? c->pool->size() : 4);
   for (uint32_t i = 0; i < n; i++)
@@ -169,6 +171,16 @@
     h2d.assign(n_groups, hipSuccess);
     const uint8_t* src = arena + offsets[0];
     const uint64_t off0 = offsets[0];
+    for (uint32_t i = 0; i < n; i++) roff[i] = b0 + (offsets[i] - off0);
+    const bool leave_split = !keep_staged && n_groups >= 2;
+    hipError_t split_err = hipSuccess;
+    if (leave_split) {
+      const uint64_t head_end = off0 + (uint64_t)std::min(total, group_first[n_groups - 1] * unit);
+      c->split_change = (uint32_t)(std::upper_bound(offsets + 1, offsets + n + 1, head_end) - (offsets + 1));
+      c->offsets_on_device = false;
+      int orc = upload_offsets(c);
+      if (orc) return orc;
+    }
     std::atomic<size_t> next_unit{0};
     const unsigned n_helpers = (unsigned)std::min<size_t>(4, std::min<size_t>(n_units > 1 ? n_units - 1 : 0, c->pool->size()));
     lap("  buffers ready");
@@ -179,6 +191,7 @@
         while (next_group < n_groups && left[next_group].load(std::memory_order_acquire) == 0) {
           size_t gb = group_first[next_group] * unit, ge = std::min(total, group_first[next_group + 1] * unit);
           h2d[next_group] = hipMemcpyAsync(d_raw + gb, raw + gb, ge - gb, hipMemcpyHostToDevice, c->stream);
+          if (leave_split && next_group + 2 == n_groups) split_err = hipEventRecord(c->ev_head_ready, c->stream);
           if (trace) fprintf(stderr, "load_changes:   group %zu (%zu KiB) enqueued +%8.3f ms\n", next_group, (ge - gb) >> 10, std::chrono::duration<double, std::milli>(std::chrono::steady_clock::now() - t_begin).count());
           next_group++;
         }
@@ -201,7 +214,7 @@
         }
       }
     });
-    for (uint32_t i = 0; i < n; i++) roff[i] = b0 + (offsets[i] - off0);
+    if (split_err != hipSuccess) return fail(c, AM355_E_DEVICE, "hipEventRecord (split point): %s", hipGetErrorString(split_err));
   } else {
     std::vector<uint32_t> group_of(n_slices);
     std::vector<size_t> group_begin{0};
@@ -263,11 +276,12 @@
   lap("gathered, H2D enqueued");
   for (hipError_t e : h2d)
     if (e != hipSuccess) return fail(c, AM355_E_DEVICE, "hipMemcpyAsync (arena): %s", hipGetErrorString(e));
-  c->offsets_on_device = false;
+  if (!c->split_change) c->offsets_on_device = false;
   if (!keep_staged) { int orc = upload_offsets(c); if (orc) return orc; }
   c->staging_in_flight = true;
   static const bool stage_sync = getenv("AM355_STAGE_SYNC") != nullptr;
   if (trace || stage_sync) { c->staging_in_flight = false; HIPCHK(c, hipStreamSynchronize(c->stream)); lap("H2D done"); }
+  c->split_fresh = !keep_staged;
   c->staged = true;
   c->stats = am355_stats{};
   c->stats.n_changes = n_all;
@@ -318,6 +332,8 @@
   c->history_ok = false;
   c->is_document = true;
   c->flags = 0;
+  c->split_change = 0;
+  c->split_fresh = false;
   const bool trace = getenv("AM355_TRACE") != nullptr;
   auto t_begin = std::chrono::steady_clock::now();
   auto lap = [&](const char* what) {
diff --git a/automerge_classic_amd/engine.py b/automerge_classic_amd/engine.py
--- a/automerge_classic_amd/engine.py
+++ b/automerge_classic_amd/engine.py
@@ -91,6 +91,9 @@
     if hasattr(L, "am355_resident_counters"):
         L.am355_resident_counters.argtypes = [vp, vp]
         L.am355_resident_counters.restype = ctypes.c_int
+    if hasattr(L, "am355_split_counters"):
+        L.am355_split_counters.argtypes = [vp, vp]
+        L.am355_split_counters.restype = ctypes.c_int
     if hasattr(L, "am355_resident_maps_only_calls"):
         L.am355_resident_maps_only_calls.argtypes = [vp, ctypes.POINTER(ctypes.c_uint64)]
         L.am355_resident_maps_only_calls.restype = ctypes.c_int
@@ -300,6 +303,11 @@
         self._check(self._L.am355_resident_counters(self._h, out))
         return int(out[0]), int(out[1]), int(out[2])
 
+    def split_counters(self):
+        out = (ctypes.c_uint64 * 3)()
+        self._check(self._L.am355_split_counters(self._h, out))
+        return int(out[0]), int(out[1]), int(out[2])
+
     def resident_maps_only_calls(self):
         out = ctypes.c_uint64()
         self._check(self._L.am355_resident_maps_only_calls(self._h, ctypes.byref(out)))
diff --git a/include/am355.h b/include/am355.h
--- a/include/am355.h
+++ b/include/am355.h
@@ -149,6 +149,7 @@
 
 int am355_resident_counters(const am355_ctx *ctx, uint64_t out[3]);
 int am355_resident_maps_only_calls(const am355_ctx *ctx, uint64_t *out);
+int am355_split_counters(const am355_ctx *ctx, uint64_t out[3]);
 
 int am355_arena_epoch(const am355_ctx *ctx, uint64_t *epoch);
 int am355_get_hashes_range(const am355_ctx *ctx, uint32_t first, uint32_t count, uint8_t *out);
```

Result: slower. 1.176 billion (-3.6%).
